# etheriqa/amber

Measured on AMD Instinct MI355X. Metric: Mrays/sec + wall-clock, Cornell 1024^2 @1024spp; 1/2/4/8 GPU, higher is better.
Workload: dtype f32

## Files before the change

amber_amd/api.py:

```python
from __future__ import annotations

import ctypes as C
import os
import subprocess
from pathlib import Path

import numpy as np

_ROOT = Path(__file__).resolve().parent
_LIB_PATH = _ROOT / "lib" / os.environ.get("AMBER_AMD_LIB", "libamber_hip.so")
_lib = None


class AmberError(RuntimeError):
    """Raised for every non-zero return code of the C ABI (message = amber_hip_last_error())."""


class FlatObject(C.Structure):
    _fields_ = [("kind", C.c_uint32), ("material", C.c_uint32), ("p", C.c_float * 12)]


class FlatMaterial(C.Structure):
    _fields_ = [("kind", C.c_uint32), ("rho", C.c_float * 3), ("param", C.c_float), ("r0", C.c_float)]


class FlatThinLens(C.Structure):
    _fields_ = [("origin", C.c_float * 3), ("global_", C.c_float * 9), ("local_", C.c_float * 9),
                ("focus_distance", C.c_float), ("sensor_distance", C.c_float), ("p_area", C.c_float),
                ("n_blades", C.c_uint32), ("first_blade_object", C.c_uint32), ("kind", C.c_uint32)]


class FlatLight(C.Structure):
    _fields_ = [("object", C.c_uint32), ("cum_power", C.c_float), ("pdf_area", C.c_float), ("irradiance", C.c_float * 3)]


class FlatSceneC(C.Structure):
    _fields_ = [("objects", C.POINTER(FlatObject)), ("n_objects", C.c_uint32),
                ("materials", C.POINTER(FlatMaterial)), ("n_materials", C.c_uint32), ("lens", FlatThinLens),
                ("lights", C.POINTER(FlatLight)), ("n_lights", C.c_uint32)]


class Splat(C.Structure):
    _fields_ = [("path", C.c_uint32), ("sample", C.c_uint32), ("bounce", C.c_uint32), ("pixel", C.c_uint32),
                ("rgb", C.c_float * 3), ("pad", C.c_uint32)]


class Sensor(C.Structure):
    _fields_ = [("width", C.c_uint32), ("height", C.c_uint32), ("scene_width", C.c_float), ("scene_height", C.c_float)]

    @classmethod
    def default(cls, width: int, height: int) -> "Sensor":
        return cls(width, height, np.float32(0.036), np.float32(0.036 / width * height))


class PtParams(C.Structure):
    _fields_ = [("seed", C.c_uint64), ("max_depth", C.c_uint32), ("device", C.c_int32), ("row_begin", C.c_uint32),
                ("row_end", C.c_uint32), ("stream", C.c_void_p), ("engine", C.c_uint32), ("stripe_rows", C.c_uint32),
                ("stripe_period", C.c_uint32), ("reserved", C.c_uint32)]


class BuildInfo(C.Structure):
    _fields_ = [("where", C.c_uint32), ("fallback_reason", C.c_uint32), ("n_nodes", C.c_uint32), ("n_leaves", C.c_uint32), ("depth", C.c_uint32),
                ("pad", C.c_uint32), ("tree_ms", C.c_double), ("create_ms", C.c_double)]


class UpdateInfo(C.Structure):
    _fields_ = [("mode_used", C.c_uint32), ("fallback_reason", C.c_uint32), ("n_nodes", C.c_uint32), ("depth", C.c_uint32),
                ("area_before", C.c_float), ("area_after", C.c_float), ("update_ms", C.c_double)]


class LtPassInfo(C.Structure):
    _fields_ = [("n_splats", C.c_uint64), ("n_rays", C.c_uint64), ("n_launches", C.c_uint32), ("n_repeats", C.c_uint32),
                ("longest_run", C.c_uint32), ("pad", C.c_uint32)]


class Photon(C.Structure):
    _fields_ = [("pos", C.c_float * 3), ("object", C.c_int32), ("dir_out", C.c_float * 3), ("path", C.c_uint32),
                ("weight", C.c_float * 3), ("sample", C.c_uint32), ("normal", C.c_float * 3), ("bounce", C.c_uint32)]


class PhotonInfo(C.Structure):
    _fields_ = [("n_photons", C.c_uint64), ("n_written", C.c_uint64), ("n_rays", C.c_uint64), ("n_launches", C.c_uint32), ("n_repeats", C.c_uint32)]


class AccumulateInfo(C.Structure):
    _fields_ = [("n_launches", C.c_uint32), ("n_repeats", C.c_uint32), ("rec_count", C.c_uint32), ("flag_words_set", C.c_uint32),
                ("flags_dirty", C.c_uint32)]


LT_SPLAT_CAPACITY0 = 65536
SPLAT_DTYPE = np.dtype([("path", np.uint32), ("sample", np.uint32), ("bounce", np.uint32), ("pixel", np.uint32), ("rgb", np.float32, (3,)), ("pad", np.uint32)])
PHOTON_DIFFUSE, PHOTON_SPECULAR, PHOTON_LIGHT, PHOTON_EYE, PHOTON_ALL = 1, 2, 4, 8, 15
PHOTONS_HOST = 1
PHOTON_CAPACITY0 = 65536
PHOTON_DTYPE = np.dtype([("pos", np.float32, (3,)), ("object", np.int32), ("dir_out", np.float32, (3,)), ("path", np.uint32),
                         ("weight", np.float32, (3,)), ("sample", np.uint32), ("normal", np.float32, (3,)), ("bounce", np.uint32)])


class Ray(C.Structure):
    _fields_ = [("origin", C.c_float * 3), ("t_max", C.c_float), ("dir", C.c_float * 3), ("pad", C.c_uint32)]


class RayHit(C.Structure):
    _fields_ = [("t", C.c_float), ("object", C.c_int32), ("pos", C.c_float * 3), ("normal", C.c_float * 3)]


class PathRay(C.Structure):
    _fields_ = [("origin", C.c_float * 3), ("pad0", C.c_uint32), ("dir", C.c_float * 3), ("pad1", C.c_uint32),
                ("weight", C.c_float * 3), ("pad2", C.c_uint32), ("rng_state", C.c_uint64), ("pad3", C.c_uint64)]


class PathResult(C.Structure):
    _fields_ = [("rgb", C.c_float * 3), ("casts", C.c_uint32), ("rng_state", C.c_uint64), ("pad", C.c_uint32 * 2)]


class AovPixel(C.Structure):
    _fields_ = [("albedo", C.c_float * 3), ("depth", C.c_float), ("normal", C.c_float * 3), ("coverage", C.c_float)]


class DenoiseParams(C.Structure):
    _fields_ = [("levels", C.c_uint32), ("k_normal", C.c_float), ("k_albedo", C.c_float), ("k_depth", C.c_float), ("k_color", C.c_float),
                ("reserved", C.c_uint32 * 3)]


class MomentsPixel(C.Structure):
    _fields_ = [("m1", C.c_float), ("m2", C.c_float), ("batches", C.c_float), ("pad", C.c_float)]


class DenoiseVarianceParams(C.Structure):
    _fields_ = [("levels", C.c_uint32), ("k_normal", C.c_float), ("k_albedo", C.c_float), ("k_depth", C.c_float), ("k_lum", C.c_float),
                ("var_radius", C.c_uint32), ("reserved", C.c_uint32 * 2)]


class TemporalParams(C.Structure):
    _fields_ = [("levels", C.c_uint32), ("max_history", C.c_uint32), ("k_normal", C.c_float), ("k_albedo", C.c_float), ("k_depth", C.c_float),
                ("k_color", C.c_float), ("reserved", C.c_uint32 * 2)]


class HistoryPixel(C.Structure):
    _fields_ = [("color", C.c_float * 3), ("length", C.c_float), ("m1", C.c_float), ("m2", C.c_float), ("pad", C.c_float * 2)]


class BvhDumpInfo(C.Structure):
    _fields_ = [("n_nodes", C.c_uint32), ("n_prims", C.c_uint32), ("root", C.c_int32), ("depth", C.c_uint32),
                ("gmin", C.c_float * 3), ("step", C.c_float * 3), ("reach", C.c_float * 3)]


class HostStats(C.Structure):
    _fields_ = [("rays", C.c_uint64), ("passes", C.c_uint64), ("launches", C.c_uint32), ("pad", C.c_uint32), ("kernel_ms", C.c_double)]


PRIM_TRIANGLE, PRIM_SPHERE, PRIM_DISK, PRIM_CYLINDER = 0, 1, 2, 3
_RECORD = np.dtype([("kind", np.uint32), ("material", np.uint32), ("p", np.float32, (12,))])
MAT_LAMBERTIAN, MAT_PHONG, MAT_SPECULAR, MAT_REFRACTION, MAT_DIFFUSE_LIGHT, MAT_EYE = 0, 1, 2, 3, 4, 5
ENGINE_AUTO, ENGINE_LIST, ENGINE_TWO_PHASE, ENGINE_BVH, ENGINE_WAVEFRONT = 0, 1, 2, 3, 4
ENGINE_REFERENCE_BVH = 6
PT_FLAG_NULL_STREAM, PT_FLAG_BVH_POOL, PT_FLAG_BVH_ITEMS = 1, 2, 4
PT_FLAG_DEVICE_BUILD = 8
BUILD_NONE, BUILD_HOST, BUILD_DEVICE, BUILD_HOST_FALLBACK = 0, 1, 2, 3
BUILD_REASON_NONE, BUILD_REASON_DEPTH, BUILD_REASON_WIDE, BUILD_REASON_BOUNDS = 0, 1, 2, 3
RAYS_HOST = 1
_RAY = np.dtype([("origin", np.float32, (3,)), ("t_max", np.float32), ("dir", np.float32, (3,)), ("pad", np.uint32)])
_RAY_HIT = np.dtype([("t", np.float32), ("object", np.int32), ("pos", np.float32, (3,)), ("normal", np.float32, (3,))])
_PATH_RAY = np.dtype([("origin", np.float32, (3,)), ("pad0", np.uint32), ("dir", np.float32, (3,)), ("pad1", np.uint32),
                      ("weight", np.float32, (3,)), ("pad2", np.uint32), ("rng_state", np.uint64), ("pad3", np.uint64)])
_PATH_RESULT = np.dtype([("rgb", np.float32, (3,)), ("casts", np.uint32), ("rng_state", np.uint64), ("pad", np.uint32, (2,))])
RESOLVE_MEAN_F32, RESOLVE_RGB8, RESOLVE_RGBA8 = 0, 1, 2
RESOLVE_HOST, RESOLVE_MIRROR_X = 1, 2
UPDATE_REFIT, UPDATE_REBUILD = 0, 1

ABI_SYMBOLS = [
    "amber_hip_pt_create", "amber_hip_pt_render_pass", "amber_hip_pt_clear", "amber_hip_pt_sync",
    "amber_hip_pt_download", "amber_hip_pt_device_framebuffer", "amber_hip_pt_stream", "amber_hip_pt_local_rows", "amber_hip_pt_kernel_time", "amber_hip_pt_build_info", "amber_hip_pt_update_objects", "amber_hip_pt_update_lens",
    "amber_hip_pt_cast_rays", "amber_hip_pt_occluded", "amber_hip_pt_resolve", "amber_hip_pt_destroy",
    "amber_hip_pt_trace_paths", "amber_hip_sampler_state",
    "amber_hip_pt_aov_pass", "amber_hip_pt_aov_clear", "amber_hip_pt_aov_download", "amber_hip_pt_device_aov", "amber_hip_pt_denoise",
    "amber_hip_pt_render_batch", "amber_hip_pt_moments_clear", "amber_hip_pt_moments_download", "amber_hip_pt_device_moments", "amber_hip_pt_denoise_variance",
    "amber_hip_pt_temporal", "amber_hip_pt_temporal_reset", "amber_hip_pt_history_download", "amber_hip_pt_device_history",
    "amber_hip_last_error", "amber_hip_abi_version", "amber_hip_math_mode", "amber_hip_device_count", "amber_hip_lt_trace", "amber_hip_lt_trace_range", "amber_hip_lt_render_pass",
    "amber_hip_lt_trace_photons",
    "amber_host_cornell_box", "amber_host_scene_import", "amber_host_scene_create", "amber_host_scene_destroy", "amber_host_scene_flatten",
    "amber_host_pt_create", "amber_host_render", "amber_host_render_devices", "amber_host_last_error", "amber_host_tonemap", "amber_host_export",
]
LAB_SYMBOLS = [
    "amber_hip_kat_cast", "amber_hip_kat_sample", "amber_hip_kat_eye", "amber_hip_kat_trace", "amber_hip_kat_math", "amber_hip_kat_signatures", "amber_hip_pt_signatures",
    "amber_hip_kat_traversal_rate", "amber_hip_kat_pixel_masks", "amber_hip_kat_bvh_dump", "amber_hip_kat_division",
    "amber_hip_kat_sqrt", "amber_hip_kat_sqrt_sweep", "amber_hip_kat_lt_accumulate", "amber_hip_kat_lt_stage_ms",
    "amber_hip_kat_photon_stage_ms",
    "amber_hip_kat_light_ray", "amber_hip_kat_lens_response", "amber_hip_kat_radiance", "amber_host_kat_scene_lights",
    "amber_hip_kat_accumulate",
]
PRODUCT_LIB, LAB_LIB = "libamber_hip.so", "libamber_hip_lab.so"


def library_path() -> Path:
    return _LIB_PATH


def build_library(force: bool = False) -> Path:
    import shutil
    if shutil.which(os.environ.get("HIPCC", "hipcc")) or not _LIB_PATH.exists():
        subprocess.run(["make", "-C", str(_ROOT / "csrc")] + (["-B"] if force else []), check=True)
    return _LIB_PATH


def is_lab() -> bool:
    return hasattr(load_library(), "amber_hip_kat_cast")


def load_library() -> C.CDLL:
    global _lib
    if _lib is not None:
        return _lib
    if not _LIB_PATH.exists():
        raise AmberError(f"{_LIB_PATH} is missing: build it with `make -C amber_amd/csrc` "
                         "(or __graft_entry__.build()); amber_amd has no CPU fallback")
    lib = C.CDLL(str(_LIB_PATH))
    vp, u32, u64, i32 = C.c_void_p, C.c_uint32, C.c_uint64, C.c_int32
    lib.amber_hip_last_error.restype = C.c_char_p
    lib.amber_host_last_error.restype = C.c_char_p
    lib.amber_hip_pt_create.argtypes = [C.POINTER(FlatSceneC), C.POINTER(Sensor), C.POINTER(PtParams), C.POINTER(vp)]
    lib.amber_hip_pt_render_pass.argtypes = [vp, u32, u32]
    lib.amber_hip_pt_clear.argtypes = [vp]
    lib.amber_hip_pt_sync.argtypes = [vp]
    lib.amber_hip_pt_download.argtypes = [vp, vp, C.POINTER(u64)]
    lib.amber_hip_pt_device_framebuffer.argtypes = [vp, C.POINTER(vp), C.POINTER(u64)]
    lib.amber_hip_pt_local_rows.argtypes = [vp, C.POINTER(u32)]
    lib.amber_hip_pt_stream.argtypes = [vp, C.POINTER(vp)]
    lib.amber_hip_pt_kernel_time.argtypes = [vp, C.POINTER(u32), C.POINTER(C.c_double)]
    lib.amber_hip_pt_destroy.argtypes = [vp]
    lib.amber_hip_pt_destroy.restype = None
    if hasattr(lib, "amber_hip_pt_build_info"):
        lib.amber_hip_pt_build_info.argtypes = [vp, C.POINTER(BuildInfo)]
    if hasattr(lib, "amber_hip_pt_update_objects"):
        lib.amber_hip_pt_update_objects.argtypes = [vp, u32, u32, vp, u32, C.POINTER(UpdateInfo)]
    if hasattr(lib, "amber_hip_pt_update_lens"):
        lib.amber_hip_pt_update_lens.argtypes = [vp, C.POINTER(FlatThinLens), vp, u32, C.POINTER(UpdateInfo)]
    if hasattr(lib, "amber_hip_pt_cast_rays"):
        lib.amber_hip_pt_cast_rays.argtypes = [vp, u64, vp, vp, u32]
        lib.amber_hip_pt_occluded.argtypes = [vp, u64, vp, vp, u32]
    if hasattr(lib, "amber_hip_pt_trace_paths"):
        lib.amber_hip_pt_trace_paths.argtypes = [vp, u64, vp, vp, u32, u32, u32]
        lib.amber_hip_sampler_state.argtypes = [u64, u32, u32]
        lib.amber_hip_sampler_state.restype = u64
    if hasattr(lib, "amber_hip_pt_resolve"):
        lib.amber_hip_pt_resolve.argtypes = [vp, u32, u32, vp, u64, u32]
    if hasattr(lib, "amber_hip_pt_aov_pass"):
        lib.amber_hip_pt_aov_pass.argtypes = [vp, u32, u32]
        lib.amber_hip_pt_aov_clear.argtypes = [vp]
        lib.amber_hip_pt_aov_download.argtypes = [vp, vp]
        lib.amber_hip_pt_device_aov.argtypes = [vp, C.POINTER(vp), C.POINTER(u64)]
    if hasattr(lib, "amber_hip_pt_denoise"):
        lib.amber_hip_pt_denoise.argtypes = [vp, u32, C.POINTER(DenoiseParams), u32, vp, u64, u32]
    if hasattr(lib, "amber_hip_pt_render_batch"):
        lib.amber_hip_pt_render_batch.argtypes = [vp, u32, u32]
        lib.amber_hip_pt_moments_clear.argtypes = [vp]
        lib.amber_hip_pt_moments_download.argtypes = [vp, vp]
        lib.amber_hip_pt_device_moments.argtypes = [vp, C.POINTER(vp), C.POINTER(u64)]
        lib.amber_hip_pt_denoise_variance.argtypes = [vp, u32, C.POINTER(DenoiseVarianceParams), u32, vp, u64, u32]
    if hasattr(lib, "amber_hip_pt_temporal"):
        lib.amber_hip_pt_temporal.argtypes = [vp, u32, C.POINTER(TemporalParams), u32, vp, u64, u32]
        lib.amber_hip_pt_temporal_reset.argtypes = [vp]
        lib.amber_hip_pt_history_download.argtypes = [vp, vp]
        lib.amber_hip_pt_device_history.argtypes = [vp, C.POINTER(vp), C.POINTER(u64)]
    if hasattr(lib, "amber_hip_lt_trace"):
        lib.amber_hip_lt_trace.argtypes = [vp, u32, u32, vp, u32, C.POINTER(u32), C.POINTER(u64)]
    if hasattr(lib, "amber_hip_lt_trace_range"):
        lib.amber_hip_lt_trace_range.argtypes = [vp, u32, u32, u32, u32, vp, u32, C.POINTER(u32), C.POINTER(u64)]
    if hasattr(lib, "amber_hip_lt_render_pass"):
        lib.amber_hip_lt_render_pass.argtypes = [vp, u32, u32, C.POINTER(LtPassInfo)]
        if hasattr(lib, "amber_hip_lt_trace_photons"):
            lib.amber_hip_lt_trace_photons.argtypes = [vp, u32, u32, u32, u32, u32, vp, u64, C.POINTER(PhotonInfo), u32]
        if hasattr(lib, "amber_hip_kat_photon_stage_ms"):
            lib.amber_hip_kat_photon_stage_ms.argtypes = [vp, C.POINTER(C.c_double), C.POINTER(C.c_double), C.POINTER(C.c_double)]
    if hasattr(lib, "amber_hip_kat_cast"):
        lib.amber_hip_kat_cast.argtypes = [vp, u32, vp, vp, vp, vp, vp, vp]
        lib.amber_hip_kat_sample.argtypes = [vp, u32, vp, vp, vp, vp, vp, vp]
        lib.amber_hip_kat_eye.argtypes = [vp, u32, vp, vp, vp]
        lib.amber_hip_kat_trace.argtypes = [vp, u32, vp, vp, u32, vp, vp]
        lib.amber_hip_kat_math.argtypes = [i32, i32, u32, vp, vp]
        lib.amber_hip_kat_signatures.argtypes = [vp, u32, u32, vp]
        lib.amber_hip_kat_pixel_masks.argtypes = [vp, vp, vp, C.POINTER(C.c_uint32), C.POINTER(C.c_double)]
        lib.amber_hip_kat_traversal_rate.argtypes = [vp, u32, vp, vp, u32, u32, u32, vp, vp, C.POINTER(C.c_double), vp]
        lib.amber_hip_pt_signatures.argtypes = [vp, u32, u32, vp]
        lib.amber_hip_kat_bvh_dump.argtypes = [vp, vp, u32, vp, u32, C.POINTER(BvhDumpInfo)]
        if hasattr(lib, "amber_hip_kat_division"):
            lib.amber_hip_kat_division.argtypes = [i32, i32, u32, vp, vp]
        if hasattr(lib, "amber_hip_kat_sqrt"):
            lib.amber_hip_kat_sqrt.argtypes = [i32, i32, u32, vp, vp]
            lib.amber_hip_kat_sqrt_sweep.argtypes = [i32, u32, u64, C.POINTER(SqrtSweep)]
        if hasattr(lib, "amber_hip_kat_lt_accumulate"):
            lib.amber_hip_kat_lt_accumulate.argtypes = [vp, vp, u32]
            lib.amber_hip_kat_lt_stage_ms.argtypes = [vp, C.POINTER(C.c_double), C.POINTER(C.c_double)]
        if hasattr(lib, "amber_hip_kat_light_ray"):
            lib.amber_hip_kat_light_ray.argtypes = [vp, u32, vp, vp, vp, vp, vp]
            lib.amber_hip_kat_lens_response.argtypes = [vp, u32, vp, vp, vp, vp, vp]
            lib.amber_hip_kat_radiance.argtypes = [vp, u32, vp, vp, vp, vp]
            lib.amber_host_kat_scene_lights.argtypes = [vp, C.POINTER(FlatLight), C.POINTER(u32)]
        if hasattr(lib, "amber_hip_kat_accumulate"):
            lib.amber_hip_kat_accumulate.argtypes = [vp, u32, vp, vp, u32, u32, u32, u64, C.POINTER(AccumulateInfo)]
    lib.amber_host_cornell_box.restype = vp
    lib.amber_host_cornell_box.argtypes = [C.c_float, C.c_float, u32]
    lib.amber_host_scene_import.restype = vp
    lib.amber_host_scene_import.argtypes = [C.c_char_p]
    lib.amber_host_scene_create.restype = vp
    lib.amber_host_scene_create.argtypes = [C.POINTER(FlatObject), u32, C.POINTER(FlatMaterial), u32, C.POINTER(C.c_float),
                                            C.c_float, C.c_float, C.c_float, u32, C.c_int]
    lib.amber_host_scene_destroy.argtypes = [vp]
    lib.amber_host_scene_destroy.restype = None
    lib.amber_host_scene_flatten.argtypes = [vp, C.POINTER(FlatObject), C.POINTER(u32), C.POINTER(FlatMaterial), C.POINTER(u32),
                                             C.POINTER(FlatThinLens)]
    lib.amber_host_pt_create.argtypes = [vp, C.POINTER(Sensor), C.POINTER(PtParams), C.POINTER(vp)]
    lib.amber_host_render.argtypes = [vp, C.c_char_p, C.POINTER(Sensor), u32, u64, u32, C.c_int, u32, vp, C.POINTER(HostStats)]
    lib.amber_host_render_devices.argtypes = [vp, C.c_char_p, C.POINTER(Sensor), u32, u64, u32, C.POINTER(C.c_int), u32, u32, vp, C.POINTER(HostStats)]
    lib.amber_host_tonemap.argtypes = [vp, u32, u32, vp]
    lib.amber_host_export.argtypes = [vp, u32, u32, C.c_char_p, C.c_char_p]
    _lib = lib
    return lib


def _check(rc: int, host: bool = False) -> None:
    if rc != 0:
        lib = load_library()
        msg = (lib.amber_host_last_error() if host else lib.amber_hip_last_error()) or b""
        if host and not msg:
            msg = lib.amber_hip_last_error() or b""
        raise AmberError(f"amber error {rc}: {msg.decode(errors='replace')}")


def device_count() -> int:
    return int(load_library().amber_hip_device_count())


def _f32(a) -> np.ndarray:
    return np.ascontiguousarray(a, dtype=np.float32)


class HostScene:

    def __init__(self, handle):
        if not handle:
            raise AmberError("scene creation failed: " + (load_library().amber_host_last_error() or b"").decode())
        self._h = C.c_void_p(handle)

    @classmethod
    def cornell_box(cls, focal_length: float = 0.050, aperture_radius: float = 0.050, n_blades: int = 6) -> "HostScene":
        return cls(load_library().amber_host_cornell_box(focal_length, aperture_radius, n_blades))

    @classmethod
    def import_file(cls, filename) -> "HostScene":
        return cls(load_library().amber_host_scene_import(str(filename).encode()))

    @classmethod
    def create(cls, objects, materials, transform, focal_length, focus_distance, radius, n_blades, accel: int = 0) -> "HostScene":
        objs = (FlatObject * max(1, len(objects)))()
        for i, (kind, mat, params) in enumerate(objects):
            objs[i].kind, objs[i].material = kind, mat
            for j, v in enumerate(params):
                objs[i].p[j] = v
        mats = (FlatMaterial * max(1, len(materials)))()
        for i, (kind, rho, param) in enumerate(materials):
            mats[i].kind, mats[i].param = kind, param
            for j in range(3):
                mats[i].rho[j] = rho[j]
        t = (C.c_float * 16)(*[float(x) for x in transform])
        return cls(load_library().amber_host_scene_create(objs, len(objects), mats, len(materials), t, focal_length,
                                                          focus_distance, radius, n_blades, accel))

    @classmethod
    def create_arrays(cls, kinds, material_index, params, materials, transform, focal_length, focus_distance, radius, n_blades,
                      accel: int = 0) -> "HostScene":
        n = len(kinds)
        dt = np.dtype([("kind", np.uint32), ("material", np.uint32), ("p", np.float32, (12,))])
        arr = np.zeros(n, dt)
        arr["kind"], arr["material"] = kinds, material_index
        arr["p"][:, : np.asarray(params).shape[1]] = params
        assert arr.itemsize == C.sizeof(FlatObject)
        mats = (FlatMaterial * max(1, len(materials)))()
        for i, (kind, rho, param) in enumerate(materials):
            mats[i].kind, mats[i].param = kind, param
            for j in range(3):
                mats[i].rho[j] = rho[j]
        t = (C.c_float * 16)(*[float(x) for x in transform])
        return cls(load_library().amber_host_scene_create(arr.ctypes.data_as(C.POINTER(FlatObject)), n, mats, len(materials), t,
                                                          focal_length, focus_distance, radius, n_blades, accel))

    def flatten(self):
        lib = load_library()
        no, nm = C.c_uint32(0), C.c_uint32(0)
        _check(lib.amber_host_scene_flatten(self._h, None, C.byref(no), None, C.byref(nm), None), host=True)
        objs, mats, lens = (FlatObject * no.value)(), (FlatMaterial * nm.value)(), FlatThinLens()
        _check(lib.amber_host_scene_flatten(self._h, objs, C.byref(no), mats, C.byref(nm), C.byref(lens)), host=True)
        return objs, mats, lens

    def lights(self):
        lib = load_library()
        n = C.c_uint32(0)
        _check(lib.amber_host_kat_scene_lights(self._h, None, C.byref(n)), host=True)
        out = (FlatLight * max(1, n.value))()
        _check(lib.amber_host_kat_scene_lights(self._h, out, C.byref(n)), host=True)
        return list(out[:n.value])

    def render(self, sensor: Sensor, spp: int, seed: int = 12345, max_depth: int = 0, device: int = 0,
               samples_per_launch: int = 0, algorithm: str = "pt", devices=None):
        out = np.empty((sensor.height, sensor.width, 3), np.float32)
        st = HostStats()
        devs = list(devices) if devices else [device]
        arr = (C.c_int * len(devs))(*devs)
        _check(load_library().amber_host_render_devices(self._h, algorithm.encode(), C.byref(sensor), spp, seed, max_depth, arr, len(devs),
                                                        samples_per_launch, out.ctypes.data, C.byref(st)), host=True)
        return out, {"rays": st.rays, "passes": st.passes, "launches": st.launches, "kernel_ms": st.kernel_ms}

    def close(self):
        if self._h:
            load_library().amber_host_scene_destroy(self._h)
            self._h = None

    def __del__(self):
        try:
            self.close()
        except Exception:
            pass


def sampler_state(seed: int, pixel: int, sample: int) -> int:
    return int(load_library().amber_hip_sampler_state(seed & 0xffffffffffffffff, pixel, sample))


def _splitmix64(z):
    with np.errstate(over="ignore"):
        z = z + np.uint64(0x9E3779B97F4A7C15)
        z = (z ^ (z >> np.uint64(30))) * np.uint64(0xBF58476D1CE4E5B9)
        z = (z ^ (z >> np.uint64(27))) * np.uint64(0x94D049BB133111EB)
        return z ^ (z >> np.uint64(31))


def sampler_states(seed: int, pixels, samples) -> np.ndarray:
    pixels, samples = np.asarray(pixels, np.uint64), np.asarray(samples, np.uint64)
    hashed = _splitmix64(np.array([seed & 0xffffffffffffffff], np.uint64))[0]
    s = _splitmix64(hashed ^ ((pixels << np.uint64(32)) | samples))
    return np.where(s == 0, np.uint64(0x9E3779B97F4A7C15), s).astype(np.uint64)


class PathTracer:

    def __init__(self, scene: HostScene, sensor: Sensor, seed: int = 12345, max_depth: int = 0, device: int = 0,
                 rows=None, stream: int | None = None, engine: int = ENGINE_AUTO, stripe=None, flags: int = 0):
        self.sensor, self.seed = sensor, seed
        self._scene, self._resident = scene, None
        rb, re = rows if rows is not None else (0, sensor.height)
        s_rows, s_period = stripe if stripe else (0, 0)
        p = PtParams(seed, max_depth, device, rb, re, stream, engine, s_rows, s_period, flags)
        h = C.c_void_p()
        _check(load_library().amber_host_pt_create(scene._h, C.byref(sensor), C.byref(p), C.byref(h)), host=True)
        self._h = h
        ys = np.arange(rb, re)
        self.row_index = ys[(ys - rb) % s_period < s_rows] if s_rows else ys
        n = C.c_uint32()
        _check(load_library().amber_hip_pt_local_rows(self._h, C.byref(n)))
        assert n.value == len(self.row_index)
        self.rows = (rb, re)

    @property
    def band_shape(self):
        return (len(self.row_index), self.sensor.width, 3)

    def render_pass(self, first_sample: int, n_samples: int) -> None:
        _check(load_library().amber_hip_pt_render_pass(self._h, first_sample, n_samples))

    def clear(self) -> None:
        _check(load_library().amber_hip_pt_clear(self._h))

    def sync(self) -> None:
        _check(load_library().amber_hip_pt_sync(self._h))

    def download(self):
        out = np.empty(self.band_shape, np.float32)
        rays = C.c_uint64()
        _check(load_library().amber_hip_pt_download(self._h, out.ctypes.data, C.byref(rays)))
        return out, rays.value

    def ray_count(self) -> int:
        rays = C.c_uint64()
        _check(load_library().amber_hip_pt_download(self._h, None, C.byref(rays)))
        return rays.value

    def stream(self) -> int:
        p = C.c_void_p()
        _check(load_library().amber_hip_pt_stream(self._h, C.byref(p)))
        return p.value or 0

    def device_framebuffer(self):
        p, n = C.c_void_p(), C.c_uint64()
        _check(load_library().amber_hip_pt_device_framebuffer(self._h, C.byref(p), C.byref(n)))
        return p.value, n.value

    def kernel_time(self):
        n, ms = C.c_uint32(), C.c_double()
        _check(load_library().amber_hip_pt_kernel_time(self._h, C.byref(n), C.byref(ms)))
        return n.value, ms.value

    def build_info(self) -> dict:
        b = BuildInfo()
        _check(load_library().amber_hip_pt_build_info(self._h, C.byref(b)))
        return {k: getattr(b, k) for k, _ in BuildInfo._fields_ if k != "pad"}

    def update_objects(self, first: int, kinds, material_index, params, mode: int = UPDATE_REFIT) -> dict:
        kinds, material_index = np.ascontiguousarray(kinds, np.uint32), np.ascontiguousarray(material_index, np.uint32)
        n = len(kinds)
        if n == 0:
            return self.update_flat(first, np.zeros(0, _RECORD), mode)
        if self._resident is None:
            objs, _, _ = self._scene.flatten()
            self._resident = np.frombuffer(objs, dtype=_RECORD)[["kind", "material"]].copy()
        if first < 0 or first + n > len(self._resident):
            raise AmberError(f"update_objects: objects [{first}, {first + n}) are not all in the scene ({len(self._resident)} objects)")
        resident = self._resident[first:first + n]
        if not np.array_equal(resident["kind"], kinds):
            raise AmberError(f"update_objects: object {first + int(np.argmax(resident['kind'] != kinds))}: the kind differs from the resident record's (an update moves geometry only)")
        pairs = np.unique(np.stack([material_index, resident["material"]], 1), axis=0)
        if len(np.unique(pairs[:, 0])) != len(pairs) or len(np.unique(pairs[:, 1])) != len(pairs):
            raise AmberError("update_objects: material_index is not the resident objects' material assignment (an update moves geometry only)")
        tmp = HostScene.create_arrays(kinds, np.zeros(n, np.uint32), params, [(MAT_LAMBERTIAN, (0.5, 0.5, 0.5), 0.0)],
                                      [1, 0, 0, 0, 0, 1, 0, 0, 0, 0, 1, 0, 0, 0, 0, 1], 0.05, 1.0, 0.01, 0)
        objs, _, lens = tmp.flatten()
        flat = np.frombuffer(objs, dtype=_RECORD)
        keep = np.ones(len(flat), bool)
        keep[lens.first_blade_object:lens.first_blade_object + lens.n_blades] = False
        records = flat[keep].copy()
        tmp.close()
        assert len(records) == n and np.array_equal(records["kind"], kinds)
        records["material"] = resident["material"]
        return self.update_flat(first, records, mode)

    def update_flat(self, first: int, records, mode: int = UPDATE_REFIT, count=None) -> dict:
        info = UpdateInfo()
        ptr, n = None, count or 0
        if records is not None:
            records = np.ascontiguousarray(records)
            assert records.itemsize == C.sizeof(FlatObject)
            ptr, n = records.ctypes.data, len(records) if count is None else count
        _check(load_library().amber_hip_pt_update_objects(self._h, first, n, ptr, mode, C.byref(info)))
        return {k: getattr(info, k) for k, _ in UpdateInfo._fields_}

    def update_lens(self, scene_or_lens, mode: int = UPDATE_REFIT) -> dict:
        if isinstance(scene_or_lens, HostScene):
            objs, _, lens = scene_or_lens.flatten()
            records = np.frombuffer(objs, dtype=_RECORD)[lens.first_blade_object:lens.first_blade_object + lens.n_blades].copy()
        else:
            lens, records = scene_or_lens
        ptr = None
        if records is not None:
            records = np.ascontiguousarray(records)
            assert records.itemsize == C.sizeof(FlatObject)
            if lens is not None and len(records) < lens.n_blades:
                raise AmberError(f"update_lens: {len(records)} blade records for a lens of {lens.n_blades} blades")
            ptr = records.ctypes.data
        info = UpdateInfo()
        _check(load_library().amber_hip_pt_update_lens(self._h, C.byref(lens) if lens is not None else None, ptr, mode, C.byref(info)))
        return {k: getattr(info, k) for k, _ in UpdateInfo._fields_}

    @staticmethod
    def _is_torch(a) -> bool:
        return type(a).__module__.split(".")[0] == "torch"

    def _pack_rays(self, origins, dirs, t_max):
        if self._is_torch(origins) or self._is_torch(dirs):
            import torch
            if not (self._is_torch(origins) and self._is_torch(dirs)) or not origins.is_cuda or origins.device != dirs.device:
                raise AmberError("cast_rays / occluded: origins and dirs must both be numpy arrays or both be torch tensors on the handle's device")
            o, d = origins.reshape(-1, 3).to(torch.float32), dirs.reshape(-1, 3).to(torch.float32)
            if len(o) != len(d):
                raise AmberError("cast_rays / occluded: origins and dirs differ in length")
            packed = torch.zeros((len(o), 8), dtype=torch.float32, device=o.device)
            packed[:, 0:3], packed[:, 4:7] = o, d
            if t_max is None:
                packed[:, 3] = float("inf")
            else:
                packed[:, 3] = t_max if not self._is_torch(t_max) else t_max.to(device=o.device, dtype=torch.float32).reshape(-1)
            return packed, len(o), torch
        o, d = _f32(origins).reshape(-1, 3), _f32(dirs).reshape(-1, 3)
        if len(o) != len(d):
            raise AmberError("cast_rays / occluded: origins and dirs differ in length")
        packed = np.zeros(len(o), _RAY)
        packed["origin"], packed["dir"] = o, d
        packed["t_max"] = np.inf if t_max is None else np.asarray(t_max, np.float32)
        return packed, len(o), None

    def cast_rays(self, origins, dirs, t_max=None):
        packed, n, torch = self._pack_rays(origins, dirs, t_max)
        lib = load_library()
        if torch is None:
            hits = np.zeros(n, _RAY_HIT)
            _check(lib.amber_hip_pt_cast_rays(self._h, n, packed.ctypes.data, hits.ctypes.data, RAYS_HOST))
            return hits["object"].copy(), hits["t"].copy(), hits["pos"].copy(), hits["normal"].copy()
        out = torch.empty((n, 8), dtype=torch.float32, device=packed.device)
        same = self._torch_enter(torch, packed.device)
        _check(lib.amber_hip_pt_cast_rays(self._h, n, packed.data_ptr(), out.data_ptr(), 0))
        self._torch_leave(same)
        return out[:, 1].contiguous().view(torch.int32), out[:, 0].contiguous(), out[:, 2:5].contiguous(), out[:, 5:8].contiguous()

    def occluded(self, origins, dirs, t_max=None):
        packed, n, torch = self._pack_rays(origins, dirs, t_max)
        lib = load_library()
        if torch is None:
            occ = np.zeros(n, np.uint8)
            _check(lib.amber_hip_pt_occluded(self._h, n, packed.ctypes.data, occ.ctypes.data, RAYS_HOST))
            return occ.astype(bool)
        out = torch.empty(n, dtype=torch.uint8, device=packed.device)
        same = self._torch_enter(torch, packed.device)
        _check(lib.amber_hip_pt_occluded(self._h, n, packed.data_ptr(), out.data_ptr(), 0))
        self._torch_leave(same)
        return out.to(torch.bool)

    def trace_paths(self, origins, dirs, weights=None, states=None, n_samples: int = 1, max_depth: int = 0):
        lib = load_library()
        if self._is_torch(origins) or self._is_torch(dirs):
            import torch
            if not (self._is_torch(origins) and self._is_torch(dirs)) or not origins.is_cuda or origins.device != dirs.device:
                raise AmberError("trace_paths: origins and dirs must both be numpy arrays or both be torch tensors on the handle's device")
            o, d = origins.reshape(-1, 3).to(torch.float32), dirs.reshape(-1, 3).to(torch.float32)
            n = len(o)
            if len(d) != n:
                raise AmberError("trace_paths: origins and dirs differ in length")
            packed = torch.zeros((n, 16), dtype=torch.float32, device=o.device)
            packed[:, 0:3], packed[:, 4:7] = o, d
            if weights is None:
                packed[:, 8:11] = 1.0
            else:
                packed[:, 8:11] = torch.as_tensor(weights, device=o.device).to(torch.float32).reshape(-1, 3)
            if states is None:
                states = sampler_states(self.seed, np.arange(n), np.zeros(n))
            if not self._is_torch(states):
                states = torch.from_numpy(np.ascontiguousarray(states, np.uint64).view(np.int64))
            packed.view(torch.int64)[:, 6] = states.to(device=o.device, dtype=torch.int64).reshape(-1)
            out = torch.empty((n, 8), dtype=torch.float32, device=o.device)
            same = self._torch_enter(torch, o.device)
            _check(lib.amber_hip_pt_trace_paths(self._h, n, packed.data_ptr(), out.data_ptr(), n_samples, max_depth, 0))
            self._torch_leave(same)
            return out[:, 0:3].contiguous(), out[:, 3].contiguous().view(torch.int32), out.view(torch.int64)[:, 2].contiguous()
        o, d = _f32(origins).reshape(-1, 3), _f32(dirs).reshape(-1, 3)
        n = len(o)
        if len(d) != n:
            raise AmberError("trace_paths: origins and dirs differ in length")
        packed = np.zeros(n, _PATH_RAY)
        packed["origin"], packed["dir"] = o, d
        packed["weight"] = 1.0 if weights is None else _f32(weights).reshape(-1, 3)
        packed["rng_state"] = sampler_states(self.seed, np.arange(n), np.zeros(n)) if states is None else np.asarray(states, np.uint64).reshape(-1)
        res = np.zeros(n, _PATH_RESULT)
        _check(lib.amber_hip_pt_trace_paths(self._h, n, packed.ctypes.data, res.ctypes.data, n_samples, max_depth, RAYS_HOST))
        return res["rgb"].copy(), res["casts"].copy(), res["rng_state"].copy()

    def _torch_enter(self, torch, device) -> bool:
        same = torch.cuda.current_stream(device).cuda_stream == self.stream()
        if not same:
            torch.cuda.current_stream(device).synchronize()
        return same

    def _torch_leave(self, same: bool) -> None:
        if not same:
            self.sync()

    def resolve(self, n_samples: int, format: int = RESOLVE_RGB8, mirror: bool = False, out=None):
        return self._filter("resolve", load_library().amber_hip_pt_resolve, n_samples, None, format, mirror, out)

    def _band_download(self, entry, channels: int) -> np.ndarray:
        rows, width, _ = self.band_shape
        out = np.zeros((rows, width, channels), np.float32)
        _check(entry(self._h, out.ctypes.data))
        return out

    def _band_pointer(self, entry):
        p, n = C.c_void_p(), C.c_uint64()
        _check(entry(self._h, C.byref(p), C.byref(n)))
        return p.value, n.value

    def aov_pass(self, first_sample: int, n_samples: int) -> None:
        _check(load_library().amber_hip_pt_aov_pass(self._h, first_sample, n_samples))

    def aov_clear(self) -> None:
        _check(load_library().amber_hip_pt_aov_clear(self._h))

    def aov_download(self) -> np.ndarray:
        return self._band_download(load_library().amber_hip_pt_aov_download, 8)

    def device_aov(self):
        return self._band_pointer(load_library().amber_hip_pt_device_aov)

    def denoise(self, n_samples: int, levels: int = 5, k_normal: float = 4.0, k_albedo: float = 100.0, k_depth: float = 10.0, k_color: float = 0.25,
                format: int = RESOLVE_RGB8, mirror: bool = False, out=None):
        params = DenoiseParams(levels=levels, k_normal=k_normal, k_albedo=k_albedo, k_depth=k_depth, k_color=k_color)
        return self._filter("denoise", load_library().amber_hip_pt_denoise, n_samples, params, format, mirror, out)

    def _filter(self, what: str, entry, n_samples: int, params, format: int, mirror: bool, out):
        if format not in (RESOLVE_MEAN_F32, RESOLVE_RGB8, RESOLVE_RGBA8):
            raise AmberError(f"{what}: unknown format {format}")
        rows, width, _ = self.band_shape
        channels, flags = (4 if format == RESOLVE_RGBA8 else 3), (RESOLVE_MIRROR_X if mirror else 0)
        head = (self._h, n_samples) if params is None else (self._h, n_samples, C.byref(params))
        if out is None:
            res = np.empty((rows, width, channels), np.float32 if format == RESOLVE_MEAN_F32 else np.uint8)
            _check(entry(*head, format, res.ctypes.data, res.nbytes, flags | RESOLVE_HOST))
            return res
        if not self._is_torch(out):
            raise AmberError(f"{what}: out must be None or a torch tensor on the handle's device")
        import torch
        dtype = torch.float32 if format == RESOLVE_MEAN_F32 else torch.uint8
        if not out.is_cuda or out.dtype != dtype or not out.is_contiguous() or out.numel() != rows * width * channels:
            raise AmberError(f"{what}: out must be a contiguous {dtype} tensor of {rows} x {width} x {channels} elements on the handle's device")
        same = self._torch_enter(torch, out.device)
        _check(entry(*head, format, out.data_ptr(), out.numel() * out.element_size(), flags))
        self._torch_leave(same)
        return out

    def render_batch(self, first_sample: int, n_samples: int) -> None:
        _check(load_library().amber_hip_pt_render_batch(self._h, first_sample, n_samples))

    def moments_clear(self) -> None:
        _check(load_library().amber_hip_pt_moments_clear(self._h))

    def moments_download(self) -> np.ndarray:
        return self._band_download(load_library().amber_hip_pt_moments_download, 4)

    def device_moments(self):
        return self._band_pointer(load_library().amber_hip_pt_device_moments)

    def denoise_variance(self, n_samples: int, levels: int = 5, k_normal: float = 4.0, k_albedo: float = 100.0, k_depth: float = 10.0, k_lum: float = 16.0,
                         var_radius: int = 3, format: int = RESOLVE_RGB8, mirror: bool = False, out=None):
        params = DenoiseVarianceParams(levels=levels, k_normal=k_normal, k_albedo=k_albedo, k_depth=k_depth, k_lum=k_lum, var_radius=var_radius)
        return self._filter("denoise_variance", load_library().amber_hip_pt_denoise_variance, n_samples, params, format, mirror, out)

    def temporal(self, n_samples: int, levels: int = 5, max_history: int = 32, k_normal: float = 4.0, k_albedo: float = 100.0, k_depth: float = 10.0,
                 k_color: float = 0.25, format: int = RESOLVE_RGB8, mirror: bool = False, out=None):
        params = TemporalParams(levels=levels, max_history=max_history, k_normal=k_normal, k_albedo=k_albedo, k_depth=k_depth, k_color=k_color)
        return self._filter("temporal", load_library().amber_hip_pt_temporal, n_samples, params, format, mirror, out)

    def temporal_reset(self) -> None:
        _check(load_library().amber_hip_pt_temporal_reset(self._h))

    def history_download(self) -> np.ndarray:
        return self._band_download(load_library().amber_hip_pt_history_download, 8)

    def device_history(self):
        return self._band_pointer(load_library().amber_hip_pt_device_history)

    def lt_trace(self, first_sample: int, n_samples: int, capacity: int = 1 << 16, paths=None):
        dt = SPLAT_DTYPE
        while True:
            out = np.zeros(capacity, dt)
            n, rays = C.c_uint32(), C.c_uint64()
            if paths is None:
                rc = load_library().amber_hip_lt_trace(self._h, first_sample, n_samples, out.ctypes.data, capacity, C.byref(n), C.byref(rays))
            else:
                rc = load_library().amber_hip_lt_trace_range(self._h, first_sample, n_samples, paths[0], paths[1], out.ctypes.data, capacity,
                                                             C.byref(n), C.byref(rays))
            if rc == -4 and n.value > capacity:
                capacity = n.value
                continue
            _check(rc)
            return out[: n.value], rays.value

    def lt_render_pass(self, first_sample: int, n_samples: int) -> dict:
        info = LtPassInfo()
        _check(load_library().amber_hip_lt_render_pass(self._h, first_sample, n_samples, C.byref(info)))
        return {k: int(getattr(info, k)) for k, _ in LtPassInfo._fields_ if k != "pad"}

    def lt_trace_photons(self, first_sample: int, n_samples: int, surfaces: int = PHOTON_DIFFUSE, paths=None, out=None):
        lib = load_library()
        begin, end = (0, self.sensor.width * self.sensor.height) if paths is None else (int(paths[0]), int(paths[1]))
        info = PhotonInfo()

        def call(ptr, capacity, flags):
            rc = lib.amber_hip_lt_trace_photons(self._h, first_sample, n_samples, begin, end, surfaces, ptr, capacity, C.byref(info), flags)
            d = {k: int(getattr(info, k)) for k, _ in PhotonInfo._fields_}
            if rc != 0:
                try:
                    _check(rc)
                except AmberError as e:
                    e.code, e.info = rc, d
                    raise
            return d

        if out is None:
            need = call(None, 0, PHOTONS_HOST)["n_photons"]
            out = np.zeros(need, PHOTON_DTYPE)
            d = call(out.ctypes.data if need else None, need, PHOTONS_HOST)
            return out, d
        if isinstance(out, np.ndarray):
            if out.dtype != PHOTON_DTYPE or not out.flags.c_contiguous or out.ndim != 1:
                raise AmberError("lt_trace_photons: out must be a contiguous one-dimensional numpy array of PHOTON_DTYPE")
            d = call(out.ctypes.data if len(out) else None, len(out), PHOTONS_HOST)
            return out[: d["n_written"]], d
        if self._is_torch(out):
            import torch
            if not out.is_cuda or not out.is_contiguous() or out.dim() != 2 or out.shape[1] * out.element_size() != 64:
                raise AmberError("lt_trace_photons: out must be a contiguous torch tensor on the handle's device with rows of 64 bytes")
            same = self._torch_enter(torch, out.device)
            try:
                d = call(out.data_ptr() if out.shape[0] else None, out.shape[0], 0)
            finally:
                self._torch_leave(same)
            return out[: d["n_written"]], d
        ptr, capacity = out
        d = call(ptr, capacity, 0)
        return d["n_written"], d

    def kat_photon_stage_ms(self):
        a, b, c = C.c_double(), C.c_double(), C.c_double()
        _check(load_library().amber_hip_kat_photon_stage_ms(self._h, C.byref(a), C.byref(b), C.byref(c)))
        return a.value, b.value, c.value

    def kat_lt_accumulate(self, records) -> None:
        rec = np.ascontiguousarray(records, SPLAT_DTYPE)
        _check(load_library().amber_hip_kat_lt_accumulate(self._h, rec.ctypes.data if len(rec) else None, len(rec)))

    def kat_accumulate(self, n_samples: int, q, rgb, n_waves: int = 4, rec_capacity: int = 0, rays: int = 0) -> dict:
        qq = np.ascontiguousarray(q, np.uint32).reshape(-1)
        cc = _f32(rgb).reshape(-1, 3)
        assert len(qq) == len(cc)
        info = AccumulateInfo()
        _check(load_library().amber_hip_kat_accumulate(self._h, n_samples, qq.ctypes.data if len(qq) else None, cc.ctypes.data if len(qq) else None,
                                                       len(qq), n_waves, rec_capacity, rays, C.byref(info)))
        return {k: int(getattr(info, k)) for k, _ in AccumulateInfo._fields_}

    def kat_lt_stage_ms(self):
        a, b = C.c_double(), C.c_double()
        _check(load_library().amber_hip_kat_lt_stage_ms(self._h, C.byref(a), C.byref(b)))
        return a.value, b.value

    def kat_cast(self, origins, dirs):
        o, d = _f32(origins).reshape(-1, 3), _f32(dirs).reshape(-1, 3)
        n = len(o)
        obj, t = np.empty(n, np.int32), np.empty(n, np.float32)
        pos, nrm = np.empty((n, 3), np.float32), np.empty((n, 3), np.float32)
        _check(load_library().amber_hip_kat_cast(self._h, n, o.ctypes.data, d.ctypes.data, obj.ctypes.data, t.ctypes.data,
                                                 pos.ctypes.data, nrm.ctypes.data))
        return obj, t, pos, nrm

    def kat_sample(self, material, normals, dirs_out, rng_state, importance: bool = False):
        m = np.ascontiguousarray(material, np.uint32) | np.uint32(0x80000000 if importance else 0)
        nn, dd = _f32(normals).reshape(-1, 3), _f32(dirs_out).reshape(-1, 3)
        st = np.ascontiguousarray(rng_state, np.uint64).copy()
        n = len(m)
        di, w = np.empty((n, 3), np.float32), np.empty((n, 3), np.float32)
        _check(load_library().amber_hip_kat_sample(self._h, n, m.ctypes.data, nn.ctypes.data, dd.ctypes.data, st.ctypes.data,
                                                   di.ctypes.data, w.ctypes.data))
        return di, w, st

    def kat_eye(self, pixel, sample):
        p, s = np.ascontiguousarray(pixel, np.uint32), np.ascontiguousarray(sample, np.uint32)
        out = np.empty((len(p), 7), np.float32)
        _check(load_library().amber_hip_kat_eye(self._h, len(p), p.ctypes.data, s.ctypes.data, out.ctypes.data))
        return out

    def kat_light_ray(self, rng_state):
        st = np.ascontiguousarray(rng_state, np.uint64).copy()
        n = len(st)
        o, d, w = np.empty((n, 3), np.float32), np.empty((n, 3), np.float32), np.empty((n, 3), np.float32)
        light = np.empty(n, np.uint32)
        _check(load_library().amber_hip_kat_light_ray(self._h, n, st.ctypes.data, o.ctypes.data, d.ctypes.data, w.ctypes.data, light.ctypes.data))
        return o, d, w, light, st

    def kat_lens_response(self, position, direction_out):
        p, d = _f32(position).reshape(-1, 3), _f32(direction_out).reshape(-1, 3)
        n = len(p)
        reached, pixel, value = np.empty(n, np.uint32), np.empty(n, np.uint32), np.empty(n, np.float32)
        _check(load_library().amber_hip_kat_lens_response(self._h, n, p.ctypes.data, d.ctypes.data, reached.ctypes.data, pixel.ctypes.data,
                                                          value.ctypes.data))
        return reached, pixel, value

    def kat_radiance(self, material, normals, dirs_out):
        m = np.ascontiguousarray(material, np.uint32)
        nn, dd = _f32(normals).reshape(-1, 3), _f32(dirs_out).reshape(-1, 3)
        out = np.empty((len(m), 3), np.float32)
        _check(load_library().amber_hip_kat_radiance(self._h, len(m), m.ctypes.data, nn.ctypes.data, dd.ctypes.data, out.ctypes.data))
        return out

    def kat_trace(self, pixel, sample, max_bounces: int = 16):
        p, s = np.ascontiguousarray(pixel, np.uint32), np.ascontiguousarray(sample, np.uint32)
        rec = np.zeros((len(p), max_bounces, 11), np.uint32)
        casts = np.zeros(len(p), np.uint32)
        _check(load_library().amber_hip_kat_trace(self._h, len(p), p.ctypes.data, s.ctypes.data, max_bounces, rec.ctypes.data,
                                                  casts.ctypes.data))
        return rec, casts

    def kat_traversal_rate(self, origins, dirs, waves: int = 5, refill_min: int = 16, repeats: int = 3, rounds=None):
        o, d = _f32(origins).reshape(-1, 3), _f32(dirs).reshape(-1, 3)
        n = len(o)
        obj, t, ms = np.empty(n, np.int32), np.empty(n, np.float32), C.c_double()
        _check(load_library().amber_hip_kat_traversal_rate(self._h, n, o.ctypes.data, d.ctypes.data, waves, refill_min, repeats, t.ctypes.data,
                                                           obj.ctypes.data, C.byref(ms), rounds.ctypes.data if rounds is not None else None))
        return obj, t, ms.value

    def kat_signatures(self, first_sample: int, n_samples: int) -> np.ndarray:
        rows, width, _ = self.band_shape
        out = np.zeros((rows, width, n_samples), np.uint64)
        _check(load_library().amber_hip_kat_signatures(self._h, first_sample, n_samples, out.ctypes.data))
        return out

    def pixel_masks(self):
        rows, width, _ = self.band_shape
        masks = np.zeros((rows, width), np.uint32)
        ms = C.c_double()
        _check(load_library().amber_hip_kat_pixel_masks(self._h, masks.ctypes.data, None, None, C.byref(ms)))
        return masks, ms.value

    def object_slots(self, n_objects: int):
        slots = np.zeros(n_objects, np.uint32)
        always = C.c_uint32()
        _check(load_library().amber_hip_kat_pixel_masks(self._h, None, slots.ctypes.data, C.byref(always), None))
        return slots, always.value

    def bvh_dump(self) -> dict:
        info = BvhDumpInfo()
        _check(load_library().amber_hip_kat_bvh_dump(self._h, None, 0, None, 0, C.byref(info)))
        nodes, prims = np.zeros((info.n_nodes, 8), np.uint32), np.zeros(info.n_prims, np.uint32)
        _check(load_library().amber_hip_kat_bvh_dump(self._h, nodes.ctypes.data, info.n_nodes, prims.ctypes.data, info.n_prims, C.byref(info)))
        return dict(nodes=nodes, prims=prims, root=int(info.root), depth=int(info.depth), gmin=np.array(info.gmin[:], np.float32),
                    step=np.array(info.step[:], np.float32), reach=np.array(info.reach[:], np.float32))

    def render_signatures(self, first_sample: int, n_samples: int) -> np.ndarray:
        rows, width, _ = self.band_shape
        out = np.zeros((rows, width, n_samples), np.uint64)
        _check(load_library().amber_hip_pt_signatures(self._h, first_sample, n_samples, out.ctypes.data))
        return out

    def close(self):
        if getattr(self, "_h", None):
            load_library().amber_hip_pt_destroy(self._h)
            self._h = None

    def __del__(self):
        try:
            self.close()
        except Exception:
            pass


def kat_math(mode: int, x, device: int = 0) -> np.ndarray:
    x = _f32(x)
    n = len(x)
    out = np.empty((n,) if mode == 1 else (n, 2), np.float32)
    _check(load_library().amber_hip_kat_math(device, mode, n, x.ctypes.data, out.ctypes.data))
    return out.view(np.float64).reshape(n) if mode >= 2 else out


def kat_division(mode: int, x, device: int = 0) -> np.ndarray:
    x = np.ascontiguousarray(x, np.float32).reshape(-1, 4)
    n = len(x)
    out = np.empty((n, 3), np.float32)
    _check(load_library().amber_hip_kat_division(device, mode, n, x.ctypes.data, out.ctypes.data))
    return out


class SqrtSweep(C.Structure):
    _fields_ = [("mismatches", C.c_uint64), ("in_range", C.c_uint64), ("n_offenders", C.c_uint32), ("offenders", C.c_uint32 * 8),
                ("seed_low", C.c_int32), ("seed_high", C.c_int32)]


def kat_sqrt(mode: int, x, device: int = 0) -> np.ndarray:
    width = 1 if mode <= 1 else (3 if mode <= 3 else 2)
    x = np.ascontiguousarray(x, np.float32).reshape(-1, width)
    out = np.empty_like(x)
    _check(load_library().amber_hip_kat_sqrt(device, mode, len(x), x.ctypes.data, out.ctypes.data))
    return out.reshape(-1) if width == 1 else out


def kat_sqrt_sweep(first_bits: int, count: int, device: int = 0) -> dict:
    r = SqrtSweep()
    _check(load_library().amber_hip_kat_sqrt_sweep(device, first_bits, count, C.byref(r)))
    return {"mismatches": int(r.mismatches), "in_range": int(r.in_range), "offenders": [int(b) for b in r.offenders[:min(int(r.n_offenders), 8)]],
            "seed_low": int(r.seed_low), "seed_high": int(r.seed_high)}


MATH_PORTABLE, MATH_GLIBC = 1, 2


def math_mode() -> int:
    return int(load_library().amber_hip_math_mode())


def tonemap(image) -> np.ndarray:
    img = _f32(image)
    h, w, _ = img.shape
    out = np.empty((h, w, 3), np.uint8)
    _check(load_library().amber_host_tonemap(img.ctypes.data, w, h, out.ctypes.data), host=True)
    return out


def export(image, png_path=None, exr_path=None) -> None:
    img = _f32(image)
    h, w, _ = img.shape
    _check(load_library().amber_host_export(img.ctypes.data, w, h, png_path.encode() if png_path else None,
                                            exr_path.encode() if exr_path else None), host=True)
```

amber_amd/csrc/hip/dev_scene.h:

```cpp
#pragma once

namespace amber_dev {

#ifdef AMBER_STAMPS
struct StampCtx { unsigned long long last; unsigned long long acc[8]; };
__device__ __forceinline__ void StampAt(StampCtx* c, int k) {
  __builtin_amdgcn_sched_barrier(0);
  const unsigned long long t = __builtin_amdgcn_s_memtime();
  __builtin_amdgcn_s_waitcnt(0xC07F);
  c->acc[k] += t - c->last;
  c->last = t;
  __builtin_amdgcn_sched_barrier(0);
}
#define AMBER_STAMP_PARAM , StampCtx* stamp_ctx
#define AMBER_STAMP_ARG , stamp_ctx
#define AMBER_STAMP(k) StampAt(stamp_ctx, k)
__device__ __forceinline__ void CountAt(StampCtx* c, int k) {
  if (!c) return;
  const unsigned long long m = __ballot(true);
  c->acc[2 * k] += 1ull;
  if (__builtin_amdgcn_mbcnt_hi(static_cast<uint32_t>(m >> 32), __builtin_amdgcn_mbcnt_lo(static_cast<uint32_t>(m), 0u)) == 0u) c->acc[2 * k + 1] += 1ull;
}
#ifdef AMBER_BVH_CLOCKS
#define AMBER_COUNT(k)
#define AMBER_CLK(k) do { if (stamp_ctx) StampAt(stamp_ctx, k); } while (0)
#else
#define AMBER_COUNT(k) CountAt(stamp_ctx, k)
#define AMBER_CLK(k)
#endif
#ifdef AMBER_COUNT_ALT
#define AMBER_COUNT_ROUNDS(k)
#define AMBER_COUNT_LEAVES(k) AMBER_COUNT(k)
#else
#define AMBER_COUNT_ROUNDS(k) AMBER_COUNT(k)
#define AMBER_COUNT_LEAVES(k)
#endif
#define AMBER_STAMP_PARAM_OPT , StampCtx* stamp_ctx = nullptr
#else
#define AMBER_COUNT(k)
#define AMBER_COUNT_ROUNDS(k)
#define AMBER_COUNT_LEAVES(k)
#define AMBER_CLK(k)
#define AMBER_STAMP_PARAM_OPT
#define AMBER_STAMP_PARAM
#define AMBER_STAMP_ARG
#define AMBER_STAMP(k)
#endif

struct alignas(16) DevObject {
  float a[3];   uint32_t kind;
  float e1[3];  float radius;
  float e2[3];  float height;
  float n[3];   uint32_t material;
};
struct alignas(16) DevMaterial {
  uint32_t kind; float rho[3];
  float param; float r0;
  float aux0, aux1;
};
struct alignas(16) DevBlade {
  float v0[3], v1[3], v2[3], n[3];
  int32_t slot;
  int32_t pad[3];
};
struct alignas(16) DevPlane {
  float n[3]; float d0;
  float kt;
  float ktol;
  uint32_t n_tris;
  uint32_t n_pairs;
};
struct alignas(16) DevTriFilter {
  float c[4][2];
};
struct alignas(16) DevSphereFilter {
  float c[3]; float r2;
  float ktol; uint32_t pad[3];
};
struct alignas(16) DevFilterGroup {
  uint32_t plane_first, n_planes, n_simple_planes, tri_first;
  uint32_t sphere_first, n_sphere_filters, always_mask, n_prog_tris;
  uint32_t n_objects, pad[3];
};
struct alignas(16) DevBvhNode {
  float lxy[4];
  float rxy[4];
  float z[4];
  int32_t left, right, pad0, pad1;
};
struct alignas(16) DevBvhNodeQ {
  uint32_t w[6];
  int32_t left, right;
};
struct alignas(16) DevBvhNodeQ4 {
  uint32_t w[12];
  int32_t child[4];
};
#ifndef AMBER_BVH_WIDE
#define AMBER_BVH_WIDE 0
#endif
struct alignas(16) DevLight {
  uint32_t kind; int32_t slot;
  float cum_power; float pdf_area;
  float irr[3]; float pad0;
  float p[12];
  float pad1[4];
};
struct DevSplat { uint32_t path, sample, bounce, pixel; float rgb[3]; uint32_t pad; };
struct DevLens {
  float origin[3];
  float global_[9];
  float local_[9];
  float focus_distance, sensor_distance, p_area;
  float neg_fd_over_sd;
  float neg_sd_over_fd;
  float size_over_area;
  double sd2;
  uint32_t n_blades;
  float n_blades_f;
  uint32_t kind;
  float inv_scene_area;
  float edge_tol;
};
struct alignas(16) DevRefNode { float lmin[3], lmax[3], rmin[3], rmax[3]; int32_t left, right; uint32_t pad[2]; };
struct DevRefLeaf { uint32_t first, count; };
struct DevSensor {
  uint32_t w, h;
  float wf, hf, sw, sh;
  float size_f;
};
struct DevScene {
  const DevObject* __restrict__ objects;
  const DevMaterial* __restrict__ materials;
  const DevBlade* __restrict__ blades;
  const DevPlane* __restrict__ planes;
  const DevTriFilter* __restrict__ tri_filters;
  const DevSphereFilter* __restrict__ sphere_filters;
  uint32_t n_planes, n_sphere_filters;
  uint32_t n_simple_planes;
  uint32_t always_mask;
  uint32_t blade_mask;
  uint32_t n_prog_tris;
  const DevObject* __restrict__ prog_objects;
  const DevFilterGroup* __restrict__ groups;
  uint32_t n_groups;
  uint32_t n_lds_objects;
  const DevBvhNodeQ* __restrict__ bvh_nodes;
  const DevBvhNodeQ4* __restrict__ bvh_nodes4;
  float bvh_gmin[3], bvh_step[3];
  float bvh_reach[3];
  const float4* __restrict__ bvh_spheres;
  const float4* __restrict__ bvh_tris;
  const uint32_t* __restrict__ bvh_prims;
  const DevObject* __restrict__ bvh_objects;
  int32_t bvh_root;
  float fp_center[3];
  float fp_reach;
  float fp_tmax;
  float bvh_center[3];
  float bvh_half_diag;
  float bvh_inv_rmin;
  const DevLight* __restrict__ lights;
  uint32_t n_lights;
  float total_power;
  uint32_t n_objects;
  uint32_t max_depth;
  const DevLens* __restrict__ lens;
  DevSensor sensor;
  const DevRefNode* __restrict__ ref_nodes;
  const DevRefLeaf* __restrict__ ref_leaves;
  uint2* ref_stack;
  uint32_t ref_stack_stride;
};

#define AMBER_PHONG_MAX_TRIES 1024
enum { PRIM_TRIANGLE = 0, PRIM_SPHERE = 1, PRIM_DISK = 2, PRIM_CYLINDER = 3 };
enum { MAT_LAMBERTIAN = 0, MAT_PHONG = 1, MAT_SPECULAR = 2, MAT_REFRACTION = 3, MAT_DIFFUSE_LIGHT = 4, MAT_EYE = 5 };

}
```

amber_amd/csrc/hip/dev_two_phase.h:

```cpp
#pragma once

namespace amber_dev {

#define AMBER_GRAZING 1e-3f
#ifndef AMBER_SHARED_WEIGHT_QUOTIENT
#define AMBER_SHARED_WEIGHT_QUOTIENT 1
#endif
struct FilterView {
  ConstWords planes, tris, spheres;
  int n_planes, n_simple_planes, n_sphere_filters;
  uint32_t always_mask, n_prog_tris, n_objects;
  int slot_base;
};
__device__ __forceinline__ FilterView SceneView(const DevScene& sc) {
  return FilterView{(ConstWords)(sc.planes), (ConstWords)(sc.tri_filters), (ConstWords)(sc.sphere_filters), static_cast<int>(sc.n_planes), static_cast<int>(sc.n_simple_planes),
                    static_cast<int>(sc.n_sphere_filters), sc.always_mask, sc.n_prog_tris, sc.n_objects, 0};
}
template <bool kMulti, bool kFirst, int kSqrt = SQRT_PLAIN>
__device__ __forceinline__ void ClosestHitTwoPhaseView(const DevScene& sc, const FilterView fv, const DevObject* lds_objects, V3 o_world, V3 d, int origin_slot, HitRec& best AMBER_STAMP_PARAM,
                                                       const bool use_premask, const uint32_t premask);
template <int kSqrt = SQRT_PLAIN>
__device__ __forceinline__ void ClosestHitTwoPhase(const DevScene& sc, const DevObject* lds_objects, V3 o_world, V3 d, int origin_slot, HitRec& best AMBER_STAMP_PARAM,
                                                   const bool use_premask = false, const uint32_t premask = 0u) {
  ClosestHitTwoPhaseView<false, true, kSqrt>(sc, SceneView(sc), lds_objects, o_world, d, origin_slot, best AMBER_STAMP_ARG, use_premask, premask);
}
template <int kSqrt = SQRT_PLAIN>
__device__ __forceinline__ void ClosestHitTwoPhaseGroups(const DevScene& sc, const DevObject* lds_objects, V3 o_world, V3 d, int origin_slot, HitRec& best AMBER_STAMP_PARAM,
                                                         const bool use_premask = false, const uint32_t premask = 0u) {
  ClosestHitTwoPhaseView<true, true, kSqrt>(sc, SceneView(sc), lds_objects, o_world, d, origin_slot < 32 ? origin_slot : -1, best AMBER_STAMP_ARG, use_premask, premask);
  const int n_groups = static_cast<int>(sc.n_groups);
  ConstWords gw = (ConstWords)(sc.groups);
  for (int g = 1; g < n_groups; ++g) {
    ConstWords w = gw + g * 12;
    const FilterView fv{(ConstWords)(sc.planes) + w[0] * 8u, (ConstWords)(sc.tri_filters) + w[3] * 8u, (ConstWords)(sc.sphere_filters) + w[4] * 8u,
                        static_cast<int>(w[1]), static_cast<int>(w[2]), static_cast<int>(w[5]), w[6], w[7], w[8], g * 32};
    ClosestHitTwoPhaseView<true, false, kSqrt>(sc, fv, lds_objects, o_world, d, origin_slot, best AMBER_STAMP_ARG, false, 0u);
  }
}
template <bool kGrouped> constexpr uint32_t kLdsKindMask = kGrouped ? 0x7fu : 0xffu;
template <bool kMulti, bool kFirst, int kSqrt>
__device__ __forceinline__ void ClosestHitTwoPhaseView(const DevScene& sc, const FilterView fv, const DevObject* lds_objects_all, V3 o_world, V3 d, int origin_slot_all, HitRec& best AMBER_STAMP_PARAM,
                                                       const bool use_premask, const uint32_t premask) {
  if (kFirst) { best.t = 3.402823466e+38f; best.u = 0.f; best.v = 0.f; best.idx = -1; best.slot = -1; }
  const int slot_base = kMulti ? fv.slot_base : 0;
  const DevObject* lds_objects = kMulti ? lds_objects_all + slot_base : lds_objects_all;
  const int origin_slot = kFirst ? origin_slot_all : ((origin_slot_all >= slot_base && origin_slot_all < slot_base + 32) ? origin_slot_all - slot_base : -1);
  constexpr uint32_t kKindMask = kLdsKindMask<kMulti>;
  uint32_t cand = kMulti ? fv.always_mask : sc.always_mask;
  if (use_premask) cand |= premask;
  else {
    const V3 o = v3(o_world.x - sc.fp_center[0], o_world.y - sc.fp_center[1], o_world.z - sc.fp_center[2]);
    float t_upper = sc.fp_tmax * __builtin_amdgcn_rsqf(d.x * d.x + d.y * d.y + d.z * d.z);
    if (!(t_upper == t_upper)) t_upper = 3.402823466e+38f;
    ConstWords pl = kMulti ? fv.planes : (ConstWords)(sc.planes);
    ConstWords tr = kMulti ? fv.tris : (ConstWords)(sc.tri_filters);
    const int n_planes = kMulti ? fv.n_planes : static_cast<int>(sc.n_planes);
    uint32_t bit = 1u;
    float nd = 0.f, no = 0.f, rc = 0.f;
#define AMBER_PLANE_NORMAL() \
        nd = __builtin_fmaf(cw_f(pl, 0), d.x, __builtin_fmaf(cw_f(pl, 1), d.y, cw_f(pl, 2) * d.z)); \
        no = __builtin_fmaf(cw_f(pl, 0), o.x, __builtin_fmaf(cw_f(pl, 1), o.y, cw_f(pl, 2) * o.z)); \
        rc = __builtin_amdgcn_rcpf(nd);
#define AMBER_PLANE_SETUP() \
      const float tp = (cw_f(pl, 3) - no) * rc; \
      const float rho = Abs(rc); \
      const float Px = __builtin_fmaf(tp, d.x, o.x), Py = __builtin_fmaf(tp, d.y, o.y), Pz = __builtin_fmaf(tp, d.z, o.z); \
      const float kr = cw_f(pl, 4) * rho;                    \
      const bool t_ok = (tp >= AMBER_KEPS - kr) && !(tp - kr > t_upper);                   \
       \
       \
      const bool degenerate = !(Abs(nd) >= 1e-6f); \
      const bool grazing = !(Abs(nd) >= AMBER_GRAZING); \
      const bool t_sure = (tp - kr > AMBER_KEPS) && !grazing; \
      const float ptol = cw_f(pl, 5) * rho; \
      const float mtol = grazing ? -3.402823466e+38f : -ptol;                              \
      bool plane_hit = false;
#ifndef AMBER_NO_CERTAIN_HITS
#define AMBER_PLANE_HIT(m_) plane_hit |= (m_) >= ptol
#else
#define AMBER_PLANE_HIT(m_)
#endif
#define AMBER_PAIR_RECORD() { \
        const float b = __builtin_fmaf(cw_f(tr, 0), Px, __builtin_fmaf(cw_f(tr, 2), Py, __builtin_fmaf(cw_f(tr, 4), Pz, cw_f(tr, 6)))); \
        const float a = __builtin_fmaf(cw_f(tr, 1), Px, __builtin_fmaf(cw_f(tr, 3), Py, __builtin_fmaf(cw_f(tr, 5), Pz, cw_f(tr, 7)))); \
        const float ba = b + a;                              \
        const float g = 1.0f - ba; \
        const float m1 = __builtin_fminf(__builtin_fminf(b, a), g); \
        const float m2 = __builtin_fminf(__builtin_fminf(-b, 1.0f - a), ba); \
        const bool keep1 = (!(m1 < mtol) && t_ok) || degenerate;                           \
        const bool keep2 = (!(m2 < mtol) && t_ok) || degenerate; \
        cand |= keep1 ? bit : 0u; \
        cand |= keep2 ? (bit << 1) : 0u; \
        AMBER_PLANE_HIT(__builtin_fmaxf(m1, m2)); }
    const int n_simple = kMulti ? fv.n_simple_planes : static_cast<int>(sc.n_simple_planes);
    int p = 0;
    for (; p < n_simple; p += 2) {
      AMBER_PLANE_NORMAL();
      { AMBER_PLANE_SETUP(); AMBER_PAIR_RECORD(); if (plane_hit && t_sure) t_upper = __builtin_fminf(t_upper, tp + kr); }
      pl += 8; tr += 8; bit <<= 2;
      { AMBER_PLANE_SETUP(); AMBER_PAIR_RECORD(); if (plane_hit && t_sure) t_upper = __builtin_fminf(t_upper, tp + kr); }
      pl += 8; tr += 8; bit <<= 2;
    }
    for (; p < n_planes; ++p, pl += 8) {
      if (!(pl[6] & 0x80000000u)) { AMBER_PLANE_NORMAL(); }
      AMBER_PLANE_SETUP();
      const int nt = static_cast<int>(pl[6] & 0x7fffffffu), np = static_cast<int>(pl[7]);
      for (int k = 0; k < np; ++k, tr += 8, bit <<= 2) {
        AMBER_PAIR_RECORD();
      }
      for (int k = 0; k < nt; ++k, tr += 8, bit <<= 1) {
        const float u = __builtin_fmaf(cw_f(tr, 0), Px, __builtin_fmaf(cw_f(tr, 2), Py, __builtin_fmaf(cw_f(tr, 4), Pz, cw_f(tr, 6))));
        const float v = __builtin_fmaf(cw_f(tr, 1), Px, __builtin_fmaf(cw_f(tr, 3), Py, __builtin_fmaf(cw_f(tr, 5), Pz, cw_f(tr, 7))));
        const float w = 1.0f - u - v;
        const float m = __builtin_fminf(__builtin_fminf(u, v), w);
        const bool keep = (!(m < mtol) && t_ok) || degenerate;
        cand |= keep ? bit : 0u;
        AMBER_PLANE_HIT(m);
      }
      if (plane_hit && t_sure) t_upper = __builtin_fminf(t_upper, tp + kr);
    }
#undef AMBER_PLANE_SETUP
#undef AMBER_PLANE_NORMAL
#undef AMBER_PAIR_RECORD
#undef AMBER_PLANE_HIT
    ConstWords sp = kMulti ? fv.spheres : (ConstWords)(sc.sphere_filters);
    const int ns = kMulti ? fv.n_sphere_filters : static_cast<int>(sc.n_sphere_filters);
    for (int k = 0; k < ns; ++k, sp += 8, bit <<= 1) {
      const float cx = cw_f(sp, 0) - o.x, cy = cw_f(sp, 1) - o.y, cz = cw_f(sp, 2) - o.z;
      const float bb = __builtin_fmaf(cx, d.x, __builtin_fmaf(cy, d.y, cz * d.z));
      const float c2 = __builtin_fmaf(cx, cx, __builtin_fmaf(cy, cy, cz * cz));
      const float r2 = cw_f(sp, 3);
      const float cc = c2 - r2;
      const float tol = cw_f(sp, 4) * (c2 + r2);
      const bool miss = (__builtin_fmaf(bb, bb, -cc) < -tol) || (bb < 0.0f && cc > tol);
      cand |= miss ? 0u : bit;
    }
  }
  if (!use_premask) {
    const float ex = Abs(o_world.x - sc.fp_center[0]), ey = Abs(o_world.y - sc.fp_center[1]), ez = Abs(o_world.z - sc.fp_center[2]);
    const bool in_model = __builtin_fmaxf(__builtin_fmaxf(ex, ey), ez) <= sc.fp_reach && (d.x * d.x + d.y * d.y + d.z * d.z) <= 4.0f;
    if (!in_model) { const uint32_t n_here = kMulti ? fv.n_objects : sc.n_objects; cand = n_here >= 32u ? 0xffffffffu : ((1u << n_here) - 1u); }
  }
  AMBER_STAMP(2);
  {
    const bool has_self = origin_slot >= 0 && ((cand >> (origin_slot & 31)) & 1u) != 0u;
    if (has_self) {
      const DevObject& ob = lds_objects[origin_slot];
      const V3 A = ld3(ob.a), E1 = ld3(ob.e1), E2 = ld3(ob.e2);
      const float det = Dot(Cross(d, E2), E1);
      const float t = Dot(Cross(o_world - A, E1), E2) / det;
      if (t <= AMBER_KEPS) cand &= ~(1u << origin_slot);
    }
  }
  const uint32_t n_tris_here = kMulti ? fv.n_prog_tris : sc.n_prog_tris;
  const uint32_t tri_bits = n_tris_here >= 32u ? 0xffffffffu : ((1u << n_tris_here) - 1u);
  uint32_t mt = cand & tri_bits;
#ifdef AMBER_STAMPS
  while (__any(mt != 0u)) {
    stamp_ctx->acc[7] += 1ull + (static_cast<unsigned long long>(__popcll(__ballot(mt != 0u))) << 32);
    if (mt != 0u) {
#else
  while (mt != 0u) {
    {
#endif
      const int slot = __builtin_ctz(mt);
      mt &= mt - 1u;
      const DevObject& ob = lds_objects[slot];
      IntersectTriangle<true>(ld3(ob.a), ld3(ob.e1), ld3(ob.e2), static_cast<int>(ob.kind >> 8), slot_base + slot, o_world, d, best);
    }
  }
  uint32_t mo = cand & ~tri_bits;
  while (mo != 0u) {
    const int slot = __builtin_ctz(mo);
    mo &= mo - 1u;
    const DevObject& ob = lds_objects[slot];
    IntersectObject<true, kSqrt>(ob, ob.kind & kKindMask, static_cast<int>(ob.kind >> 8), slot_base + slot, o_world, d, best);
  }
}

}
```

amber_amd/csrc/hip/filter_build.h:

```cpp
#pragma once

#include <algorithm>
#include <cmath>
#include <cstdint>
#include <cstring>
#include <vector>

#include "../../../include/amber_hip.h"
#include "pt_device.h"

namespace amber_filter {

using amber_dev::DevObject;
using amber_dev::DevPlane;
using amber_dev::DevSphereFilter;
using amber_dev::DevTriFilter;

struct FilterProgram {
  std::vector<DevPlane> planes;
  std::vector<DevTriFilter> tris;
  std::vector<DevSphereFilter> spheres;
  std::vector<uint32_t> order;
  uint32_t n_prog_tris = 0, always_mask = 0;
  uint32_t n_simple_planes = 0;
};

inline void BuildFilterProgram(const std::vector<DevObject>& objs, const float center[3], FilterProgram& fp, const std::vector<uint32_t>* subset = nullptr) {
  double lo[3] = {1e300, 1e300, 1e300}, hi[3] = {-1e300, -1e300, -1e300}, e_max = 0;
  auto grow = [&](double x, double y, double z) {
    const double p[3] = {x, y, z};
    for (int c = 0; c < 3; c++) { if (p[c] < lo[c]) lo[c] = p[c]; if (p[c] > hi[c]) hi[c] = p[c]; }
  };
  auto len3 = [](const double* v) { return std::sqrt(v[0] * v[0] + v[1] * v[1] + v[2] * v[2]); };
  for (const DevObject& o : objs) {
    if (o.kind == AMBER_PRIM_TRIANGLE) {
      grow(o.a[0], o.a[1], o.a[2]);
      grow(double(o.a[0]) + o.e1[0], double(o.a[1]) + o.e1[1], double(o.a[2]) + o.e1[2]);
      grow(double(o.a[0]) + o.e2[0], double(o.a[1]) + o.e2[1], double(o.a[2]) + o.e2[2]);
      const double E1[3] = {o.e1[0], o.e1[1], o.e1[2]}, E2[3] = {o.e2[0], o.e2[1], o.e2[2]};
      e_max = std::max(e_max, std::max(len3(E1), len3(E2)));
    } else {
      const double r = std::fabs(double(o.radius)) + std::fabs(double(o.height));
      grow(o.a[0] - r, o.a[1] - r, o.a[2] - r); grow(o.a[0] + r, o.a[1] + r, o.a[2] + r);
    }
  }
  const double diam = std::sqrt((hi[0] - lo[0]) * (hi[0] - lo[0]) + (hi[1] - lo[1]) * (hi[1] - lo[1]) + (hi[2] - lo[2]) * (hi[2] - lo[2]));
  const double eps = 5.9604644775390625e-08;
  const double c = 32.0 * eps * (diam + 1.5 * e_max);
  struct Tri { uint32_t index; double v[3][3]; double coef[3][4]; double g; };
  struct Group { double n[3], d0, kt, ktol; std::vector<Tri> tris; bool flip = false, same_normal = false; };
  std::vector<Group> groups;
  std::vector<uint32_t> sphere_index, always_index;
  const size_t n_members = subset ? std::min<size_t>(subset->size(), 32) : std::min<size_t>(objs.size(), 32);
  for (size_t member = 0; member < n_members; member++) {
    const uint32_t idx = subset ? (*subset)[member] : static_cast<uint32_t>(member);
    const DevObject& o = objs[idx];
    if (o.kind == AMBER_PRIM_TRIANGLE) {
      const double v0[3] = {double(o.a[0]) - center[0], double(o.a[1]) - center[1], double(o.a[2]) - center[2]};
      const double E1[3] = {o.e1[0], o.e1[1], o.e1[2]}, E2[3] = {o.e2[0], o.e2[1], o.e2[2]};
      const double nr[3] = {E1[1] * E2[2] - E1[2] * E2[1], E1[2] * E2[0] - E1[0] * E2[2], E1[0] * E2[1] - E1[1] * E2[0]};
      const double n2 = nr[0] * nr[0] + nr[1] * nr[1] + nr[2] * nr[2];
      if (!(n2 > 1e-60) || !std::isfinite(n2)) { always_index.push_back(idx); continue; }
      const double nl = std::sqrt(n2);
      const double n[3] = {nr[0] / nl, nr[1] / nl, nr[2] / nl};
      const double d0 = n[0] * v0[0] + n[1] * v0[1] + n[2] * v0[2];
      const double A[3] = {(E2[1] * nr[2] - E2[2] * nr[1]) / n2, (E2[2] * nr[0] - E2[0] * nr[2]) / n2, (E2[0] * nr[1] - E2[1] * nr[0]) / n2};
      const double B[3] = {(nr[1] * E1[2] - nr[2] * E1[1]) / n2, (nr[2] * E1[0] - nr[0] * E1[2]) / n2, (nr[0] * E1[1] - nr[1] * E1[0]) / n2};
      const double AB[3] = {A[0] + B[0], A[1] + B[1], A[2] + B[2]};
      const double g = std::max(len3(A), std::max(len3(B), len3(AB)));
      const double inv_sin = len3(E1) * len3(E2) / nl;
      const double verts[3][3] = {{v0[0], v0[1], v0[2]}, {v0[0] + E1[0], v0[1] + E1[1], v0[2] + E1[2]}, {v0[0] + E2[0], v0[1] + E2[1], v0[2] + E2[2]}};
      Group* grp = nullptr; double dist = 0;
      for (Group& gq : groups) {
        double dmax = 0;
        for (const auto& vtx : verts) dmax = std::max(dmax, std::fabs(gq.n[0] * vtx[0] + gq.n[1] * vtx[1] + gq.n[2] * vtx[2] - gq.d0));
        if (dmax <= 4.0 * eps * diam) { grp = &gq; dist = dmax; break; }
      }
      Tri t;
      t.index = idx; t.g = g;
      for (int k = 0; k < 3; k++) for (int c2 = 0; c2 < 3; c2++) t.v[k][c2] = verts[k][c2];
      const double a0 = -(A[0] * v0[0] + A[1] * v0[1] + A[2] * v0[2]), b0 = -(B[0] * v0[0] + B[1] * v0[1] + B[2] * v0[2]);
      for (int k = 0; k < 3; k++) { t.coef[1][k] = A[k]; t.coef[2][k] = B[k]; t.coef[0][k] = -(A[k] + B[k]); }
      t.coef[1][3] = a0; t.coef[2][3] = b0; t.coef[0][3] = 1.0 - a0 - b0;
      const double ktol = (c + dist) * g * 1.0001 + 1e-7;
      const double kt = 2.0 * (c + dist) * std::max(1.0, inv_sin) + 1e-7;
      if (!std::isfinite(ktol) || !std::isfinite(static_cast<float>(a0)) || !std::isfinite(static_cast<float>(b0)) || !std::isfinite(kt)) { always_index.push_back(idx); continue; }
      if (!grp) { groups.push_back(Group{{n[0], n[1], n[2]}, d0, 0.0, 0.0, {}, false, false}); grp = &groups.back(); }
      grp->kt = std::max(grp->kt, kt);
      grp->ktol = std::max(grp->ktol, ktol);
      grp->tris.push_back(t);
    } else if (o.kind == AMBER_PRIM_SPHERE) {
      DevSphereFilter f;
      std::memset(&f, 0, sizeof f);
      for (int k = 0; k < 3; k++) f.c[k] = static_cast<float>(double(o.a[k]) - center[k]);
      f.r2 = static_cast<float>(double(o.radius) * double(o.radius));
      f.ktol = 1e-5f;
      if (!std::isfinite(f.r2)) { always_index.push_back(idx); continue; }
      fp.spheres.push_back(f);
      sphere_index.push_back(idx);
    } else {
      always_index.push_back(idx);
    }
  }
  auto record = [](const Tri& t, int row_a, int row_b) {
    DevTriFilter f;
    std::memset(&f, 0, sizeof f);
    for (int k = 0; k < 4; k++) { f.c[k][0] = static_cast<float>(t.coef[row_a][k]); f.c[k][1] = static_cast<float>(t.coef[row_b][k]); }
    return f;
  };
  {
    double cw[3] = {0, 0, 0}, wsum = 0;
    std::vector<double> gc(groups.size() * 3, 0.0);
    for (size_t gi = 0; gi < groups.size(); gi++) {
      double gw = 0;
      for (const Tri& t : groups[gi].tris) {
        const double e1[3] = {t.v[1][0] - t.v[0][0], t.v[1][1] - t.v[0][1], t.v[1][2] - t.v[0][2]};
        const double e2[3] = {t.v[2][0] - t.v[0][0], t.v[2][1] - t.v[0][1], t.v[2][2] - t.v[0][2]};
        const double cr[3] = {e1[1] * e2[2] - e1[2] * e2[1], e1[2] * e2[0] - e1[0] * e2[2], e1[0] * e2[1] - e1[1] * e2[0]};
        const double area = 0.5 * len3(cr);
        for (int k = 0; k < 3; k++) gc[gi * 3 + k] += area * (t.v[0][k] + t.v[1][k] + t.v[2][k]) / 3.0;
        gw += area;
      }
      for (int k = 0; k < 3; k++) { cw[k] += gc[gi * 3 + k]; if (gw > 0) gc[gi * 3 + k] /= gw; }
      wsum += gw;
    }
    if (wsum > 0) for (int k = 0; k < 3; k++) cw[k] /= wsum;
    std::vector<int> cls(groups.size(), -1);
    std::vector<size_t> cls_first;
    for (size_t gi = 0; gi < groups.size(); gi++) {
      for (size_t c = 0; c < cls_first.size() && cls[gi] < 0; c++) {
        const Group& f = groups[cls_first[c]];
        const double dot = f.n[0] * groups[gi].n[0] + f.n[1] * groups[gi].n[1] + f.n[2] * groups[gi].n[2];
        const double sgn = dot < 0 ? -1.0 : 1.0;
        bool same = true;
        for (int k = 0; k < 3; k++) same = same && static_cast<float>(groups[gi].n[k]) == static_cast<float>(sgn * f.n[k]);
        if (same) {
          cls[gi] = static_cast<int>(c);
          for (int k = 0; k < 3; k++) groups[gi].n[k] = sgn * f.n[k];
          groups[gi].flip = dot < 0;
        }
      }
      if (cls[gi] < 0) { cls[gi] = static_cast<int>(cls_first.size()); cls_first.push_back(gi); }
    }
    auto dist2 = [&](size_t gi) { double d2 = 0; for (int k = 0; k < 3; k++) d2 += (gc[gi * 3 + k] - cw[k]) * (gc[gi * 3 + k] - cw[k]); return d2; };
    std::vector<double> cls_min(cls_first.size(), 1e300);
    for (size_t gi = 0; gi < groups.size(); gi++) cls_min[cls[gi]] = std::min(cls_min[cls[gi]], dist2(gi));
    std::vector<size_t> perm(groups.size());
    for (size_t gi = 0; gi < perm.size(); gi++) perm[gi] = gi;
    std::stable_sort(perm.begin(), perm.end(), [&](size_t x, size_t y) {
      if (cls[x] != cls[y]) return cls_min[cls[x]] != cls_min[cls[y]] ? cls_min[cls[x]] < cls_min[cls[y]] : cls[x] < cls[y];
      return dist2(x) < dist2(y);
    });
    std::vector<Group> sorted;
    int prev_cls = -1;
    for (size_t gi : perm) {
      sorted.push_back(groups[gi]);
      sorted.back().same_normal = cls[gi] == prev_cls;
      prev_cls = cls[gi];
    }
    groups.swap(sorted);
  }
  for (const Group& g : groups) {
    const size_t nt = g.tris.size();
    std::vector<int> partner(nt, -1), unshared(nt, -1);
    double pair_slack = 0;
    auto apart = [](const double* p, const double* r) { return std::max(std::fabs(p[0] - r[0]), std::max(std::fabs(p[1] - r[1]), std::fabs(p[2] - r[2]))); };
    for (size_t i = 0; i < nt; i++) {
      if (partner[i] >= 0) continue;
      for (size_t j = i + 1; j < nt && partner[i] < 0; j++) {
        if (partner[j] >= 0) continue;
        int match_i[3] = {-1, -1, -1}, n_shared = 0;
        bool used_j[3] = {false, false, false};
        double err = 0;
        for (int k = 0; k < 3; k++)
          for (int l = 0; l < 3; l++)
            if (!used_j[l] && match_i[k] < 0 && apart(g.tris[i].v[k], g.tris[j].v[l]) <= 1e-6 * diam) {
              match_i[k] = l; used_j[l] = true; n_shared++;
              err = std::max(err, apart(g.tris[i].v[k], g.tris[j].v[l]));
            }
        if (n_shared != 2) continue;
        int bi = -1, dj = -1;
        for (int k = 0; k < 3; k++) if (match_i[k] < 0) bi = k;
        for (int l = 0; l < 3; l++) if (!used_j[l]) dj = l;
        double expect[3];
        for (int c2 = 0; c2 < 3; c2++) {
          expect[c2] = -g.tris[i].v[bi][c2];
          for (int k = 0; k < 3; k++) if (k != bi) expect[c2] += g.tris[i].v[k][c2];
        }
        err = std::max(err, apart(expect, g.tris[j].v[dj]));
        if (err <= 1e-6 * diam) {
          partner[i] = static_cast<int>(j); partner[j] = static_cast<int>(i); unshared[i] = bi;
          pair_slack = std::max(pair_slack, 4.0 * err * std::max(g.tris[i].g, g.tris[j].g));
        }
      }
    }
    DevPlane p;
    std::memset(&p, 0, sizeof p);
    for (int k = 0; k < 3; k++) p.n[k] = static_cast<float>(g.flip ? -g.n[k] : g.n[k]);
    p.d0 = static_cast<float>(g.flip ? -g.d0 : g.d0); p.kt = static_cast<float>(g.kt * 1.0001); p.ktol = static_cast<float>((g.ktol + 4e-7 + pair_slack) * 1.0001);
    for (size_t i = 0; i < nt; i++) {
      if (partner[i] < 0 || static_cast<size_t>(partner[i]) < i) continue;
      const int bi = unshared[i], ai = (bi + 1) % 3;
      fp.tris.push_back(record(g.tris[i], bi, ai));
      fp.order.push_back(g.tris[i].index); fp.order.push_back(g.tris[static_cast<size_t>(partner[i])].index);
      p.n_pairs++;
    }
    for (size_t i = 0; i < nt; i++) {
      if (partner[i] >= 0) continue;
      fp.tris.push_back(record(g.tris[i], 1, 2));
      fp.order.push_back(g.tris[i].index);
      p.n_tris++;
    }
    if (g.same_normal) p.n_tris |= 0x80000000u;
    fp.planes.push_back(p);
  }
  {
    struct Span { size_t rec, slot; };
    std::vector<Span> span(fp.planes.size());
    { size_t rec = 0, slot = 0;
      for (size_t i = 0; i < fp.planes.size(); i++) {
        span[i] = Span{rec, slot};
        const uint32_t nt = fp.planes[i].n_tris & 0x7fffffffu, np = fp.planes[i].n_pairs;
        rec += np + nt; slot += 2 * np + nt;
      } }
    auto simple = [&](size_t i) { return fp.planes[i].n_pairs == 1 && (fp.planes[i].n_tris & 0x7fffffffu) == 0; };
    std::vector<char> in_slab(fp.planes.size(), 0);
    for (size_t i = 0; i + 1 < fp.planes.size(); i++)
      if (!in_slab[i] && simple(i) && simple(i + 1) && std::memcmp(fp.planes[i].n, fp.planes[i + 1].n, sizeof fp.planes[i].n) == 0) { in_slab[i] = in_slab[i + 1] = 1; i++; }
    std::vector<DevPlane> planes; std::vector<DevTriFilter> tris; std::vector<uint32_t> order;
    for (int pass = 0; pass < 2; pass++)
      for (size_t i = 0; i < fp.planes.size(); i++) {
        if ((in_slab[i] != 0) != (pass == 0)) continue;
        DevPlane q = fp.planes[i];
        const uint32_t nt = q.n_tris & 0x7fffffffu, np = q.n_pairs;
        q.n_tris = nt;
        if (!planes.empty() && std::memcmp(planes.back().n, q.n, sizeof q.n) == 0) q.n_tris |= 0x80000000u;
        planes.push_back(q);
        for (uint32_t k = 0; k < np + nt; k++) tris.push_back(fp.tris[span[i].rec + k]);
        for (uint32_t k = 0; k < 2 * np + nt; k++) order.push_back(fp.order[span[i].slot + k]);
        if (pass == 0) fp.n_simple_planes++;
      }
    fp.planes.swap(planes); fp.tris.swap(tris); fp.order.swap(order);
  }
  fp.n_prog_tris = static_cast<uint32_t>(fp.order.size());
  fp.order.insert(fp.order.end(), sphere_index.begin(), sphere_index.end());
  for (uint32_t idx : always_index) { fp.always_mask |= 1u << fp.order.size(); fp.order.push_back(idx); }
}

}
```

amber_amd/csrc/hip/lab_api.inc:

```

namespace {
constexpr const char* kKatNoRefBvh = "the known-answer kernels have no instantiation for AMBER_ENGINE_REFERENCE_BVH (its traversal stack belongs to the render kernels' grid): compare amber_hip_pt_signatures instead";
template <typename F>
void WithKatEngine(const amber_hip_pt* h, F&& f) {
  WithHitEngine(h->hit_engine, [&](auto engine) -> int { if constexpr (decltype(engine)::value != ENGINE_REF_BVH) f(engine); return AMBER_OK; });
}

int RenderPassWavefront(amber_hip_pt* h, uint32_t first_sample, uint32_t n_samples) {
  const uint32_t n_pixels = static_cast<uint32_t>(BandPixels(h));
  const uint64_t kMaxPaths = 1ull << 28;
  uint64_t max_chunks = kMaxPaths / (static_cast<uint64_t>(n_pixels) * AMBER_ACCUM_CHUNK);
  if (max_chunks == 0) return Fail(AMBER_EINVAL, "band too large for the wavefront engine");
  const uint32_t kMaxBounces = 4096;
  const uint64_t cap = max_chunks * AMBER_ACCUM_CHUNK;
  return SplitSamples(first_sample, n_samples, "band too large for the wavefront engine", [&](uint32_t left, amber_plan::Launch* l) -> int {
    *l = {left > cap ? static_cast<uint32_t>(cap) : left, 0};
    return AMBER_OK;
  }, [&](uint32_t first, const amber_plan::Launch& l, bool*) -> int {
    const uint32_t n = l.n;
    const uint32_t n_chunks = (n + AMBER_ACCUM_CHUNK - 1) / AMBER_ACCUM_CHUNK;
    const size_t n_paths = static_cast<size_t>(n_chunks) * n_pixels * AMBER_ACCUM_CHUNK;
    const size_t shard_capacity = ((n_paths + AMBER_WF_SHARDS - 1) / AMBER_WF_SHARDS + 63) / 64 * 64 + 64;
    const size_t q_len = shard_capacity * AMBER_WF_SHARDS;
    const size_t n_counts = static_cast<size_t>(kMaxBounces + 2) * AMBER_WF_SHARDS;
    const size_t bytes = (26 * q_len + 3 * n_paths) * 4 + n_counts * sizeof(unsigned int);
    AMBER_TRY(Grow(h, h->d_wf, bytes / sizeof(float), "wavefront queues"));
    float* base = h->d_wf;
    WfQueue q[2];
    for (int k = 0; k < 2; k++) {
      for (int c = 0; c < 9; c++) q[k].f[c] = base + (static_cast<size_t>(k) * 13 + c) * q_len;
      for (int c = 0; c < 4; c++) q[k].u[c] = reinterpret_cast<uint32_t*>(base + (static_cast<size_t>(k) * 13 + 9 + c) * q_len);
    }
    float* meas = base + 26 * q_len;
    unsigned int* counts = reinterpret_cast<unsigned int*>(meas + 3 * n_paths);
    HIP_TRY(hipMemsetAsync(counts, 0, n_counts * sizeof(unsigned int), h->stream));
    WfArgs a;
    a.scene = h->scene; a.meas = meas; a.counts = counts; a.ray_count = h->d_rays; a.hashed_seed = h->hashed_seed;
    a.SetBand(h->row_begin, h->stripe_rows, h->stripe_period); a.n_pixels = n_pixels;
    a.first_sample = first; a.n_samples = n; a.n_paths = static_cast<uint32_t>(n_paths); a.bounce = 0; a.shard_capacity = static_cast<uint32_t>(shard_capacity);
    const uint32_t n_blocks = 2048u;
    AMBER_TRY(TimedLaunch(h, true, [&]() -> int {
      a.out = q[0]; a.in = q[1];
      hipLaunchKernelGGL(wf_generate_kernel, dim3(n_blocks), dim3(256), 0, h->stream, a);
      HIP_TRY(hipGetLastError());
      uint32_t bounce = 0;
      for (;;) {
        const uint32_t burst = bounce < 16 ? 8 : 16;
        for (uint32_t k = 0; k < burst && bounce < kMaxBounces; k++, bounce++) {
          a.bounce = bounce; a.in = q[bounce & 1]; a.out = q[(bounce + 1) & 1];
          WithHitEngine(h->hit_engine, [&](auto engine) -> int {
            constexpr int kEngine = decltype(engine)::value == ENGINE_TWO_PHASE || decltype(engine)::value == ENGINE_BVH ? decltype(engine)::value : ENGINE_LIST;
            hipLaunchKernelGGL(wf_bounce_kernel<kEngine>, dim3(n_blocks), dim3(256), 0, h->stream, a);
            return AMBER_OK;
          });
          HIP_TRY(hipGetLastError());
        }
        unsigned int shard_live[AMBER_WF_SHARDS];
        HIP_TRY(hipMemcpyAsync(shard_live, counts + static_cast<size_t>(bounce) * AMBER_WF_SHARDS, sizeof shard_live, hipMemcpyDeviceToHost, h->stream));
        HIP_TRY(hipStreamSynchronize(h->stream));
        unsigned long long live = 0;
        for (unsigned int v : shard_live) live += v;
        if (live == 0) break;
        if (bounce >= kMaxBounces) return Fail(AMBER_EHIP, "wavefront engine: path longer than 4096 bounces");
      }
      return AMBER_OK;
    }));
    const uint32_t n_elems = n_pixels * 3u;
    hipLaunchKernelGGL(wf_reduce_kernel, dim3((n_elems + 255u) / 256u), dim3(256), 0, h->stream, h->d_fb, meas, n_pixels, n_chunks);
    HIP_TRY(hipGetLastError());
    return AMBER_OK;
  });
}

int LaunchLabRecords(amber_hip_pt* h, uint32_t n, uint32_t n_pixels, float* target, const RecordProducer& producer) {
  AMBER_TRY(BeginPathLaunch(h, n, n_pixels, false));
  RenderArgs a = MakeRenderArgs(h, h->hashed_seed, n_pixels, 0u, n);
  SetRecordArgs(h, a);
  a.n_items = n_pixels * n;
  AMBER_TRY(TimedLaunch(h, false, [&]() -> int {
    hipLaunchKernelGGL(kat_accumulate_kernel, dim3((producer.n_waves + 3u) / 4u), dim3(256), 0, h->stream, a, producer.q, producer.rgb, producer.n_items,
                       producer.n_waves, producer.rays);
    return AMBER_OK;
  }));
  return FinishPathLaunch(h, 0u, n, n_pixels, target, producer, false);
}

}

extern "C" {

int amber_hip_kat_cast(amber_hip_pt* h, uint32_t n, const float* origins, const float* dirs,
                       int32_t* out_object, float* out_t, float* out_pos, float* out_normal) { return Guarded("amber_hip_kat_cast", [&]() -> int {
  if (h && h->hit_engine == AMBER_ENGINE_REFERENCE_BVH) return Fail(AMBER_EINVAL, kKatNoRefBvh);
  if (!h || !origins || !dirs || !out_object || !out_t || !out_pos || !out_normal) return Fail(AMBER_EINVAL, "null argument");
  if (n == 0) return AMBER_OK;
  HIP_TRY(hipSetDevice(h->device));
  DevBuf<float> d_o, d_d, d_t, d_p, d_n; DevBuf<int32_t> d_i;
  HIP_TRY(d_o.alloc(3 * n)); HIP_TRY(d_d.alloc(3 * n)); HIP_TRY(d_t.alloc(n)); HIP_TRY(d_p.alloc(3 * n)); HIP_TRY(d_n.alloc(3 * n)); HIP_TRY(d_i.alloc(n));
  HIP_TRY(hipMemcpy(d_o.p, origins, 3ull * n * 4, hipMemcpyHostToDevice));
  HIP_TRY(hipMemcpy(d_d.p, dirs, 3ull * n * 4, hipMemcpyHostToDevice));
  WithKatEngine(h, [&](auto engine) { hipLaunchKernelGGL(kat_cast_kernel<decltype(engine)::value>, dim3((n + 255) / 256), dim3(256), 0, h->stream, h->scene, n, d_o.p, d_d.p, d_i.p, d_t.p, d_p.p, d_n.p); });
  HIP_TRY(hipGetLastError());
  HIP_TRY(hipStreamSynchronize(h->stream));
  HIP_TRY(hipMemcpy(out_object, d_i.p, 4ull * n, hipMemcpyDeviceToHost));
  HIP_TRY(hipMemcpy(out_t, d_t.p, 4ull * n, hipMemcpyDeviceToHost));
  HIP_TRY(hipMemcpy(out_pos, d_p.p, 12ull * n, hipMemcpyDeviceToHost));
  HIP_TRY(hipMemcpy(out_normal, d_n.p, 12ull * n, hipMemcpyDeviceToHost));
  return AMBER_OK;
}); }

int amber_hip_kat_sample(amber_hip_pt* h, uint32_t n, const uint32_t* material, const float* normals,
                         const float* dirs_out, uint64_t* rng_state, float* out_dir_in, float* out_weight) { return Guarded("amber_hip_kat_sample", [&]() -> int {
  if (!h || !material || !normals || !dirs_out || !rng_state || !out_dir_in || !out_weight) return Fail(AMBER_EINVAL, "null argument");
  if (n == 0) return AMBER_OK;
  for (uint32_t i = 0; i < n; i++)
    if ((material[i] & 0x7fffffffu) >= h->n_materials) return Fail(AMBER_EINVAL, "material index out of range");
  HIP_TRY(hipSetDevice(h->device));
  DevBuf<uint32_t> d_m; DevBuf<float> d_n, d_d, d_o, d_w; DevBuf<uint64_t> d_r;
  HIP_TRY(d_m.alloc(n)); HIP_TRY(d_n.alloc(3 * n)); HIP_TRY(d_d.alloc(3 * n)); HIP_TRY(d_o.alloc(3 * n)); HIP_TRY(d_w.alloc(3 * n)); HIP_TRY(d_r.alloc(n));
  HIP_TRY(hipMemcpy(d_m.p, material, 4ull * n, hipMemcpyHostToDevice));
  HIP_TRY(hipMemcpy(d_n.p, normals, 12ull * n, hipMemcpyHostToDevice));
  HIP_TRY(hipMemcpy(d_d.p, dirs_out, 12ull * n, hipMemcpyHostToDevice));
  HIP_TRY(hipMemcpy(d_r.p, rng_state, 8ull * n, hipMemcpyHostToDevice));
  hipLaunchKernelGGL(kat_sample_kernel, dim3((n + 255) / 256), dim3(256), 0, h->stream, h->scene, n, d_m.p, d_n.p, d_d.p, d_r.p, d_o.p, d_w.p);
  HIP_TRY(hipGetLastError());
  HIP_TRY(hipStreamSynchronize(h->stream));
  HIP_TRY(hipMemcpy(rng_state, d_r.p, 8ull * n, hipMemcpyDeviceToHost));
  HIP_TRY(hipMemcpy(out_dir_in, d_o.p, 12ull * n, hipMemcpyDeviceToHost));
  HIP_TRY(hipMemcpy(out_weight, d_w.p, 12ull * n, hipMemcpyDeviceToHost));
  return AMBER_OK;
}); }

int amber_hip_kat_eye(amber_hip_pt* h, uint32_t n, const uint32_t* pixel, const uint32_t* sample, float* out7) { return Guarded("amber_hip_kat_eye", [&]() -> int {
  if (!h || !pixel || !sample || !out7) return Fail(AMBER_EINVAL, "null argument");
  if (n == 0) return AMBER_OK;
  const uint32_t npx = h->scene.sensor.w * h->scene.sensor.h;
  for (uint32_t i = 0; i < n; i++) if (pixel[i] >= npx) return Fail(AMBER_EINVAL, "pixel index out of range");
  HIP_TRY(hipSetDevice(h->device));
  DevBuf<uint32_t> d_p, d_s; DevBuf<float> d_o;
  HIP_TRY(d_p.alloc(n)); HIP_TRY(d_s.alloc(n)); HIP_TRY(d_o.alloc(7 * n));
  HIP_TRY(hipMemcpy(d_p.p, pixel, 4ull * n, hipMemcpyHostToDevice));
  HIP_TRY(hipMemcpy(d_s.p, sample, 4ull * n, hipMemcpyHostToDevice));
  hipLaunchKernelGGL(kat_eye_kernel, dim3((n + 255) / 256), dim3(256), 0, h->stream, h->scene, h->hashed_seed, n, d_p.p, d_s.p, d_o.p);
  HIP_TRY(hipGetLastError());
  HIP_TRY(hipStreamSynchronize(h->stream));
  HIP_TRY(hipMemcpy(out7, d_o.p, 28ull * n, hipMemcpyDeviceToHost));
  return AMBER_OK;
}); }

int amber_hip_kat_light_ray(amber_hip_pt* h, uint32_t n, uint64_t* rng_state, float* out_origin, float* out_dir, float* out_weight,
                            uint32_t* out_light) { return Guarded("amber_hip_kat_light_ray", [&]() -> int {
  if (!h || !rng_state || !out_origin || !out_dir || !out_weight || !out_light) return Fail(AMBER_EINVAL, "null argument");
  if (h->scene.n_lights == 0) return Fail(AMBER_EINVAL, "amber_hip_kat_light_ray: the handle's scene has no lights");
  if (h->lights_stale) return Fail(AMBER_EINVAL, "lights are stale after amber_hip_pt_update_objects: re-create the handle");
  if (n == 0) return AMBER_OK;
  if (n > 0x3fffffffu) return Fail(AMBER_EINVAL, "too many items for one call");
  HIP_TRY(hipSetDevice(h->device));
  DevBuf<uint64_t> d_r; DevBuf<float> d_o, d_d, d_w; DevBuf<uint32_t> d_l;
  HIP_TRY(d_r.alloc(n)); HIP_TRY(d_o.alloc(3ull * n)); HIP_TRY(d_d.alloc(3ull * n)); HIP_TRY(d_w.alloc(3ull * n)); HIP_TRY(d_l.alloc(n));
  HIP_TRY(hipMemcpy(d_r.p, rng_state, 8ull * n, hipMemcpyHostToDevice));
  hipLaunchKernelGGL(kat_light_ray_kernel, dim3((n + 255) / 256), dim3(256), 0, h->stream, h->scene, n, d_r.p, d_o.p, d_d.p, d_w.p, d_l.p);
  HIP_TRY(hipGetLastError());
  HIP_TRY(hipStreamSynchronize(h->stream));
  HIP_TRY(hipMemcpy(rng_state, d_r.p, 8ull * n, hipMemcpyDeviceToHost));
  HIP_TRY(hipMemcpy(out_origin, d_o.p, 12ull * n, hipMemcpyDeviceToHost));
  HIP_TRY(hipMemcpy(out_dir, d_d.p, 12ull * n, hipMemcpyDeviceToHost));
  HIP_TRY(hipMemcpy(out_weight, d_w.p, 12ull * n, hipMemcpyDeviceToHost));
  HIP_TRY(hipMemcpy(out_light, d_l.p, 4ull * n, hipMemcpyDeviceToHost));
  return AMBER_OK;
}); }

int amber_hip_kat_lens_response(amber_hip_pt* h, uint32_t n, const float* position, const float* direction_out, uint32_t* out_reached,
                                uint32_t* out_pixel, float* out_value) { return Guarded("amber_hip_kat_lens_response", [&]() -> int {
  if (!h || !position || !direction_out || !out_reached || !out_pixel || !out_value) return Fail(AMBER_EINVAL, "null argument");
  if (n == 0) return AMBER_OK;
  if (n > 0x3fffffffu) return Fail(AMBER_EINVAL, "too many items for one call");
  HIP_TRY(hipSetDevice(h->device));
  DevBuf<float> d_p, d_d, d_v; DevBuf<uint32_t> d_r, d_x;
  HIP_TRY(d_p.alloc(3ull * n)); HIP_TRY(d_d.alloc(3ull * n)); HIP_TRY(d_v.alloc(n)); HIP_TRY(d_r.alloc(n)); HIP_TRY(d_x.alloc(n));
  HIP_TRY(hipMemcpy(d_p.p, position, 12ull * n, hipMemcpyHostToDevice));
  HIP_TRY(hipMemcpy(d_d.p, direction_out, 12ull * n, hipMemcpyHostToDevice));
  hipLaunchKernelGGL(kat_lens_response_kernel, dim3((n + 255) / 256), dim3(256), 0, h->stream, h->scene, n, d_p.p, d_d.p, d_r.p, d_x.p, d_v.p);
  HIP_TRY(hipGetLastError());
  HIP_TRY(hipStreamSynchronize(h->stream));
  HIP_TRY(hipMemcpy(out_reached, d_r.p, 4ull * n, hipMemcpyDeviceToHost));
  HIP_TRY(hipMemcpy(out_pixel, d_x.p, 4ull * n, hipMemcpyDeviceToHost));
  HIP_TRY(hipMemcpy(out_value, d_v.p, 4ull * n, hipMemcpyDeviceToHost));
  return AMBER_OK;
}); }

int amber_hip_kat_radiance(amber_hip_pt* h, uint32_t n, const uint32_t* material, const float* normals, const float* dirs_out,
                           float* out) { return Guarded("amber_hip_kat_radiance", [&]() -> int {
  if (!h || !material || !normals || !dirs_out || !out) return Fail(AMBER_EINVAL, "null argument");
  if (n == 0) return AMBER_OK;
  if (n > 0x3fffffffu) return Fail(AMBER_EINVAL, "too many items for one call");
  for (uint32_t i = 0; i < n; i++) if (material[i] >= h->n_materials) return Fail(AMBER_EINVAL, "material index out of range");
  HIP_TRY(hipSetDevice(h->device));
  DevBuf<uint32_t> d_m; DevBuf<float> d_n, d_d, d_o;
  HIP_TRY(d_m.alloc(n)); HIP_TRY(d_n.alloc(3ull * n)); HIP_TRY(d_d.alloc(3ull * n)); HIP_TRY(d_o.alloc(3ull * n));
  HIP_TRY(hipMemcpy(d_m.p, material, 4ull * n, hipMemcpyHostToDevice));
  HIP_TRY(hipMemcpy(d_n.p, normals, 12ull * n, hipMemcpyHostToDevice));
  HIP_TRY(hipMemcpy(d_d.p, dirs_out, 12ull * n, hipMemcpyHostToDevice));
  hipLaunchKernelGGL(kat_radiance_kernel, dim3((n + 255) / 256), dim3(256), 0, h->stream, h->scene, n, d_m.p, d_n.p, d_d.p, d_o.p);
  HIP_TRY(hipGetLastError());
  HIP_TRY(hipStreamSynchronize(h->stream));
  HIP_TRY(hipMemcpy(out, d_o.p, 12ull * n, hipMemcpyDeviceToHost));
  return AMBER_OK;
}); }

int amber_hip_kat_trace(amber_hip_pt* h, uint32_t n, const uint32_t* pixel, const uint32_t* sample,
                        uint32_t max_bounces, uint32_t* out_records, uint32_t* out_casts) { return Guarded("amber_hip_kat_trace", [&]() -> int {
  if (h && h->hit_engine == AMBER_ENGINE_REFERENCE_BVH) return Fail(AMBER_EINVAL, kKatNoRefBvh);
  if (!h || !pixel || !sample || !out_records || !out_casts || max_bounces == 0) return Fail(AMBER_EINVAL, "bad argument");
  if (n == 0) return AMBER_OK;
  const uint32_t npx = h->scene.sensor.w * h->scene.sensor.h;
  for (uint32_t i = 0; i < n; i++) if (pixel[i] >= npx) return Fail(AMBER_EINVAL, "pixel index out of range");
  HIP_TRY(hipSetDevice(h->device));
  DevBuf<uint32_t> d_p, d_s, d_r, d_c;
  const size_t nrec = static_cast<size_t>(n) * max_bounces * 11;
  HIP_TRY(d_p.alloc(n)); HIP_TRY(d_s.alloc(n)); HIP_TRY(d_r.alloc(nrec)); HIP_TRY(d_c.alloc(n));
  HIP_TRY(hipMemcpy(d_p.p, pixel, 4ull * n, hipMemcpyHostToDevice));
  HIP_TRY(hipMemcpy(d_s.p, sample, 4ull * n, hipMemcpyHostToDevice));
  HIP_TRY(hipMemsetAsync(d_r.p, 0, nrec * 4, h->stream));
  WithKatEngine(h, [&](auto engine) { hipLaunchKernelGGL(kat_trace_kernel<decltype(engine)::value>, dim3((n + 255) / 256), dim3(256), 0, h->stream, h->scene, h->hashed_seed, n, d_p.p, d_s.p, max_bounces, d_r.p, d_c.p); });
  HIP_TRY(hipGetLastError());
  HIP_TRY(hipStreamSynchronize(h->stream));
  HIP_TRY(hipMemcpy(out_records, d_r.p, nrec * 4, hipMemcpyDeviceToHost));
  HIP_TRY(hipMemcpy(out_casts, d_c.p, 4ull * n, hipMemcpyDeviceToHost));
  return AMBER_OK;
}); }

int amber_hip_kat_signatures(amber_hip_pt* h, uint32_t first_sample, uint32_t n_samples, uint64_t* out) { return Guarded("amber_hip_kat_signatures", [&]() -> int {
  if (h && h->hit_engine == AMBER_ENGINE_REFERENCE_BVH) return Fail(AMBER_EINVAL, kKatNoRefBvh);
  if (!h || !out || n_samples == 0) return Fail(AMBER_EINVAL, "bad argument");
  if (static_cast<uint64_t>(first_sample) + n_samples > 0xffffffffull) return Fail(AMBER_EINVAL, "sample index overflow");
  const uint64_t n = BandPixels(h) * n_samples;
  if (n == 0) return AMBER_OK;
  if ((n + 255) / 256 > 0x7fffffffull) return Fail(AMBER_EINVAL, "too many paths for one call");
  HIP_TRY(hipSetDevice(h->device));
  DevBuf<unsigned long long> d_out;
  HIP_TRY(d_out.alloc(n));
  const dim3 grid(static_cast<uint32_t>((n + 255) / 256));
  WithKatEngine(h, [&](auto engine) { hipLaunchKernelGGL(kat_signature_kernel<decltype(engine)::value>, grid, dim3(256), 0, h->stream, h->scene, h->hashed_seed, n, first_sample, n_samples, h->row_begin, h->stripe_rows, h->stripe_period, MakeExactDiv(h->stripe_rows), d_out.p); });
  HIP_TRY(hipGetLastError());
  HIP_TRY(hipStreamSynchronize(h->stream));
  HIP_TRY(hipMemcpy(out, d_out.p, n * sizeof(uint64_t), hipMemcpyDeviceToHost));
  return AMBER_OK;
}); }

int amber_hip_kat_traversal_rate(amber_hip_pt* h, uint32_t n, const float* origins, const float* dirs, uint32_t waves, uint32_t refill_min, uint32_t repeats,
                                 float* out_t, int32_t* out_object, double* best_ms, uint32_t* out_rounds) { return Guarded("amber_hip_kat_traversal_rate", [&]() -> int {
  if (!h || !origins || !dirs || !out_t || !out_object || n == 0) return Fail(AMBER_EINVAL, "bad argument");
  if (h->hit_engine != AMBER_ENGINE_BVH) return Fail(AMBER_EINVAL, "the handle's engine is not BVH");
  if (refill_min == 0 || refill_min > 64) return Fail(AMBER_EINVAL, "refill_min must be in [1, 64]");
  const uint64_t n_virtual = static_cast<uint64_t>(n) * (repeats ? repeats : 1u);
  if (n_virtual > 0xfffffeffull) return Fail(AMBER_EINVAL, "n * repeats must stay below 2^32");
  HIP_TRY(hipSetDevice(h->device));
  AMBER_TRY(ResolvePending(h));
  std::vector<float4> packed(2ull * n);
  for (uint32_t i = 0; i < n; i++) {
    packed[2ull * i] = make_float4(origins[3ull * i], origins[3ull * i + 1], origins[3ull * i + 2], 0.f);
    packed[2ull * i + 1] = make_float4(dirs[3ull * i], dirs[3ull * i + 1], dirs[3ull * i + 2], 0.f);
  }
  DevBuf<float4> d_rays; DevBuf<float2> d_out; DevBuf<unsigned int> d_next; DevBuf<int32_t> d_stack; DevBuf<uint32_t> d_rounds;
  if (out_rounds) HIP_TRY(d_rounds.alloc(n));
  HIP_TRY(d_rays.alloc(2ull * n)); HIP_TRY(d_out.alloc(n)); HIP_TRY(d_next.alloc(1));
  const uint32_t n_blocks = static_cast<uint32_t>(h->n_cus) * (waves >= 4 && waves <= 8 ? waves : 5u);
  HIP_TRY(d_stack.alloc(static_cast<size_t>(n_blocks) * 256u * AMBER_BVH_STACK));
  HIP_TRY(hipMemcpy(d_rays.p, packed.data(), packed.size() * sizeof(float4), hipMemcpyHostToDevice));
  Event ev0, ev1;
  HIP_TRY(hipEventCreate(&ev0.v)); HIP_TRY(hipEventCreate(&ev1.v));
  const hipEvent_t e0 = ev0.v, e1 = ev1.v;
  double best = 1e300;
  const uint32_t nv = static_cast<uint32_t>(n_virtual);
  for (uint32_t rep = 0; rep < 2u; rep++) {
    HIP_TRY(hipMemsetAsync(d_next.p, 0, sizeof(unsigned int), h->stream));
    HIP_TRY(hipEventRecord(e0, h->stream));
    switch (waves) {
      case 4: hipLaunchKernelGGL((bvh_trace_rate_kernel<4, 24>), dim3(n_blocks), dim3(256), 0, h->stream, h->scene, nv, d_rays.p, d_out.p, d_next.p, d_stack.p, refill_min, n, d_rounds.p); break;
      case 6: hipLaunchKernelGGL((bvh_trace_rate_kernel<6, 24>), dim3(n_blocks), dim3(256), 0, h->stream, h->scene, nv, d_rays.p, d_out.p, d_next.p, d_stack.p, refill_min, n, d_rounds.p); break;
      case 8: hipLaunchKernelGGL((bvh_trace_rate_kernel<8, 16>), dim3(n_blocks), dim3(256), 0, h->stream, h->scene, nv, d_rays.p, d_out.p, d_next.p, d_stack.p, refill_min, n, d_rounds.p); break;
      default: hipLaunchKernelGGL((bvh_trace_rate_kernel<5, 24>), dim3(n_blocks), dim3(256), 0, h->stream, h->scene, nv, d_rays.p, d_out.p, d_next.p, d_stack.p, refill_min, n, d_rounds.p); break;
    }
    HIP_TRY(hipGetLastError());
    HIP_TRY(hipEventRecord(e1, h->stream));
    HIP_TRY(hipStreamSynchronize(h->stream));
    float ms = 0; HIP_TRY(hipEventElapsedTime(&ms, e0, e1));
    if (rep == 1u || ms < best) best = ms;
  }
  std::vector<float2> res(n);
  HIP_TRY(hipMemcpy(res.data(), d_out.p, n * sizeof(float2), hipMemcpyDeviceToHost));
  if (out_rounds) HIP_TRY(hipMemcpy(out_rounds, d_rounds.p, n * sizeof(uint32_t), hipMemcpyDeviceToHost));
  std::vector<uint32_t> prims(h->scene.n_objects);
  HIP_TRY(hipMemcpy(prims.data(), h->scene.bvh_prims, prims.size() * sizeof(uint32_t), hipMemcpyDeviceToHost));
  for (uint32_t i = 0; i < n; i++) {
    int32_t slot; std::memcpy(&slot, &res[i].y, 4);
    out_object[i] = slot < 0 ? -1 : static_cast<int32_t>(prims[slot]);
    out_t[i] = slot < 0 ? std::nanf("") : res[i].x;
  }
  if (best_ms) *best_ms = best;
  return AMBER_OK;
}); }

int amber_hip_kat_pixel_masks(amber_hip_pt* h, uint32_t* out_mask, uint32_t* out_slot_of_object, uint32_t* out_always_mask, double* kernel_ms) { return Guarded("amber_hip_kat_pixel_masks", [&]() -> int {
  if (!h) return Fail(AMBER_EINVAL, "null handle");
  if (!h->two_phase) return Fail(AMBER_EINVAL, "pixel masks belong to the two-phase engine");
  HIP_TRY(hipSetDevice(h->device));
  AMBER_TRY(ResolvePending(h));
  const uint32_t n_pixels = static_cast<uint32_t>(BandPixels(h));
  if (out_mask || kernel_ms) {
    float ms = 0;
    AMBER_TRY(StartPixelMasks(h, kernel_ms ? &ms : nullptr));
    if (!h->pixel_mask_ready) return Fail(AMBER_EINVAL, "pixel masks are switched off (AMBER_PIXEL_MASK=0) or the band is empty");
    HIP_TRY(hipStreamSynchronize(h->stream));
    if (out_mask) HIP_TRY(hipMemcpy(out_mask, h->d_pixel_mask, static_cast<size_t>(n_pixels) * sizeof(uint32_t), hipMemcpyDeviceToHost));
    if (kernel_ms) *kernel_ms = static_cast<double>(ms);
  }
  if (out_slot_of_object) {
    for (uint32_t i = 0; i < h->scene.n_objects; i++) out_slot_of_object[i] = 0xffffffffu;
    for (size_t k = 0; k < h->prog_order.size(); k++) if (h->prog_order[k] < h->scene.n_objects) out_slot_of_object[h->prog_order[k]] = static_cast<uint32_t>(k);
  }
  if (out_always_mask) *out_always_mask = h->scene.always_mask | h->scene.blade_mask;
  return AMBER_OK;
}); }

int amber_hip_kat_bvh_dump(amber_hip_pt* h, uint32_t* nodes, uint32_t node_capacity, uint32_t* prims, uint32_t prim_capacity, AmberBvhDump* info) { return Guarded("amber_hip_kat_bvh_dump", [&]() -> int {
  if (!h || !info) return Fail(AMBER_EINVAL, "null argument");
  if (h->hit_engine != AMBER_ENGINE_BVH) return Fail(AMBER_EINVAL, "the handle's engine is not BVH");
  HIP_TRY(hipSetDevice(h->device));
  AMBER_TRY(ResolvePending(h));
  HIP_TRY(hipStreamSynchronize(h->stream));
  static_assert(sizeof(DevBvhNodeQ) == 8 * sizeof(uint32_t), "a dumped node is 8 words");
  info->n_nodes = h->build.n_nodes; info->n_prims = h->scene.n_objects; info->root = h->scene.bvh_root; info->depth = h->build.depth;
  for (int c = 0; c < 3; c++) { info->gmin[c] = h->scene.bvh_gmin[c]; info->step[c] = h->scene.bvh_step[c]; info->reach[c] = h->scene.bvh_reach[c]; }
  const uint32_t n_nodes = std::min(node_capacity, info->n_nodes), n_prims = std::min(prim_capacity, info->n_prims);
  if (nodes && n_nodes) HIP_TRY(hipMemcpy(nodes, h->scene.bvh_nodes, static_cast<size_t>(n_nodes) * sizeof(DevBvhNodeQ), hipMemcpyDeviceToHost));
  if (prims && n_prims) HIP_TRY(hipMemcpy(prims, h->scene.bvh_prims, static_cast<size_t>(n_prims) * sizeof(uint32_t), hipMemcpyDeviceToHost));
  return AMBER_OK;
}); }

int amber_hip_pt_signatures(amber_hip_pt* h, uint32_t first_sample, uint32_t n_samples, uint64_t* out) { return Guarded("amber_hip_pt_signatures", [&]() -> int {
  if (!h || !out || n_samples == 0) return Fail(AMBER_EINVAL, "bad argument");
  if (static_cast<uint64_t>(first_sample) + n_samples > 0xffffffffull) return Fail(AMBER_EINVAL, "sample index overflow");
  if (h->engine == AMBER_ENGINE_WAVEFRONT) return Fail(AMBER_EINVAL, "signatures come from the work-queue kernels (engines list, two_phase, bvh)");
  const uint32_t n_pixels = static_cast<uint32_t>(BandPixels(h));
  const uint64_t n = static_cast<uint64_t>(n_pixels) * n_samples;
  if (n == 0) return AMBER_OK;
  if (n > kMaxPathsPerLaunch) return Fail(AMBER_EINVAL, "too many paths for one call");
  HIP_TRY(hipSetDevice(h->device));
  AMBER_TRY(ResolvePending(h));
  HIP_TRY(hipStreamSynchronize(h->stream));
  AMBER_TRY(Grow(h, h->d_sig, n, "signatures"));
  HIP_TRY(hipMemsetAsync(h->d_sig, 0, n * sizeof(unsigned long long), h->stream));
  AMBER_TRY(RenderSamples(h, first_sample, n_samples, n_pixels, h->d_fb, h->d_sig));
  HIP_TRY(hipStreamSynchronize(h->stream));
  HIP_TRY(hipMemcpy(out, h->d_sig, n * sizeof(uint64_t), hipMemcpyDeviceToHost));
  return AMBER_OK;
}); }

int amber_hip_kat_lt_accumulate(amber_hip_pt* h, const AmberSplat* records, uint32_t n) { return Guarded("amber_hip_kat_lt_accumulate", [&]() -> int {
  if (!h || (n && !records)) return Fail(AMBER_EINVAL, "null argument");
  if (!WholeFrame(h)) return Fail(AMBER_EINVAL, "amber_hip_kat_lt_accumulate: the handle renders a band or stripes of the frame");
  if (n > 0x7fffffffu) return Fail(AMBER_EINVAL, "too many records for one call");
  const uint32_t npx = h->scene.sensor.w * h->scene.sensor.h;
  for (uint32_t i = 0; i < n; i++) if (records[i].pixel >= npx) return Fail(AMBER_EINVAL, "pixel index out of range");
  if (n == 0) return AMBER_OK;
  HIP_TRY(hipSetDevice(h->device));
  AMBER_TRY(ResolvePending(h));
  AMBER_TRY(EnsureLtSplats(h, n));
  static_assert(sizeof(AmberSplat) == sizeof(DevSplat), "splat layouts must agree");
  HIP_TRY(hipMemcpyAsync(h->d_splats, records, static_cast<size_t>(n) * sizeof(DevSplat), hipMemcpyHostToDevice, h->stream));
  HIP_TRY(hipMemsetAsync(h->lt.longest.p, 0, sizeof(unsigned int), h->stream));
  AMBER_TRY(LtAccumulate(h, n, 32u));
  HIP_TRY(hipStreamSynchronize(h->stream));
  return AMBER_OK;
}); }

int amber_hip_kat_accumulate(amber_hip_pt* h, uint32_t n_samples, const uint32_t* q, const float* rgb, uint32_t n_items, uint32_t n_waves, uint32_t rec_capacity,
                             uint64_t rays, AmberAccumulateInfo* info) { return Guarded("amber_hip_kat_accumulate", [&]() -> int {
  if (info) *info = AmberAccumulateInfo{};
  if (!h || (n_items && (!q || !rgb))) return Fail(AMBER_EINVAL, "null argument");
  if (n_samples == 0 || n_waves == 0) return Fail(AMBER_EINVAL, "amber_hip_kat_accumulate: n_samples and n_waves must not be zero");
  if (n_waves > (1u << 20)) return Fail(AMBER_EINVAL, "amber_hip_kat_accumulate: more than 2^20 waves");
  const uint64_t n_paths = BandPixels(h) * n_samples;
  if (n_paths >= (1ull << 32)) return Fail(AMBER_EINVAL, "amber_hip_kat_accumulate: n_pixels * n_samples must stay below 2^32");
  {
    std::vector<uint32_t> seen;
    seen.reserve(n_items);
    for (uint32_t i = 0; i < n_items; i++) {
      if (q[i] == AMBER_REC_UNUSED) continue;
      if (q[i] >= n_paths) return Fail(AMBER_EINVAL, "amber_hip_kat_accumulate: item " + std::to_string(i) + ": path index out of range");
      seen.push_back(q[i]);
    }
    std::sort(seen.begin(), seen.end());
    if (std::adjacent_find(seen.begin(), seen.end()) != seen.end()) return Fail(AMBER_EINVAL, "amber_hip_kat_accumulate: a path index occurs twice");
  }
  HIP_TRY(hipSetDevice(h->device));
  AMBER_TRY(ResolvePending(h));
  PathLaunchBufs& p = h->paths;
  if (rec_capacity != 0 && rec_capacity < p.rec_capacity)
    return Fail(AMBER_EINVAL, "amber_hip_kat_accumulate: rec_capacity " + std::to_string(rec_capacity) + " is below the " + std::to_string(p.rec_capacity) + " slots the handle's record buffer has");
  const uint32_t n_pixels = static_cast<uint32_t>(BandPixels(h));
  if (n_pixels == 0) return AMBER_OK;
  AMBER_TRY(EnsureRecordCapacity(h, rec_capacity ? rec_capacity : static_cast<uint64_t>(n_items) + RecordSlack(h)));
  DevBuf<uint32_t> d_q; DevBuf<float> d_rgb;
  HIP_TRY(d_q.alloc(n_items ? n_items : 1u)); HIP_TRY(d_rgb.alloc(n_items ? 3ull * n_items : 1u));
  if (n_items) {
    HIP_TRY(hipMemcpy(d_q.p, q, 4ull * n_items, hipMemcpyHostToDevice));
    HIP_TRY(hipMemcpy(d_rgb.p, rgb, 12ull * n_items, hipMemcpyHostToDevice));
  }
  RecordProducer producer;
  producer.lab = true; producer.q = d_q.p; producer.rgb = d_rgb.p; producer.n_items = n_items; producer.n_waves = n_waves; producer.rays = rays;
  const uint64_t launches0 = p.n_launches, repeats0 = p.n_repeats;
  AMBER_TRY(LaunchLabRecords(h, n_samples, n_pixels, h->d_fb, producer));
  const int rc = ResolvePending(h);
  p.pending = false; p.pending_producer = RecordProducer{};
  AMBER_TRY(rc);
  const size_t used_words = static_cast<size_t>((n_paths + 31u) / 32u);
  std::vector<uint32_t> words(used_words);
  if (used_words) HIP_TRY(hipMemcpyAsync(words.data(), p.flags, used_words * sizeof(uint32_t), hipMemcpyDeviceToHost, h->stream));
  HIP_TRY(hipStreamSynchronize(h->stream));
  if (info) {
    info->n_launches = static_cast<uint32_t>(p.n_launches - launches0); info->n_repeats = static_cast<uint32_t>(p.n_repeats - repeats0);
    info->rec_count = *p.h_rec_count.v;
    info->flag_words_set = static_cast<uint32_t>(std::count_if(words.begin(), words.end(), [](uint32_t w) { return w != 0u; }));
    info->flags_dirty = p.flags_dirty ? 1u : 0u;
  }
  return AMBER_OK;
}); }

int amber_hip_kat_lt_stage_ms(amber_hip_pt* h, double* sort_ms, double* sum_ms) { return Guarded("amber_hip_kat_lt_stage_ms", [&]() -> int {
  if (!h) return Fail(AMBER_EINVAL, "null handle");
  h->lt.stage_timing = true;
  if (sort_ms) *sort_ms = h->lt.sort_ms;
  if (sum_ms) *sum_ms = h->lt.sum_ms;
  h->lt.sort_ms = h->lt.sum_ms = 0;
  return AMBER_OK;
}); }

int amber_hip_kat_photon_stage_ms(amber_hip_pt* h, double* trace_ms, double* sort_ms, double* gather_ms) { return Guarded("amber_hip_kat_photon_stage_ms", [&]() -> int {
  if (!h) return Fail(AMBER_EINVAL, "null handle");
  PhotonBufs& s = h->photons;
  s.stage_timing = true;
  if (trace_ms) *trace_ms = s.trace_ms;
  if (sort_ms) *sort_ms = s.sort_ms;
  if (gather_ms) *gather_ms = s.gather_ms;
  s.trace_ms = s.sort_ms = s.gather_ms = 0;
  return AMBER_OK;
}); }

int amber_hip_kat_math(int device, int mode, uint32_t n, const float* x, float* out) { return Guarded("amber_hip_kat_math", [&]() -> int {
  if (!x || !out || mode < 0 || mode > 3) return Fail(AMBER_EINVAL, "bad argument");
  if (n == 0) return AMBER_OK;
  int n_dev = 0;
  if (hipGetDeviceCount(&n_dev) != hipSuccess || device < 0 || device >= n_dev) return Fail(AMBER_ENODEVICE, "no such HIP device");
  HIP_TRY(hipSetDevice(device));
  const size_t n_in = mode == 1 ? 2ull * n : n, n_out = mode == 1 ? n : 2ull * n;
  DevBuf<float> d_x, d_o;
  HIP_TRY(d_x.alloc(n_in)); HIP_TRY(d_o.alloc(n_out));
  HIP_TRY(hipMemcpy(d_x.p, x, n_in * 4, hipMemcpyHostToDevice));
  hipLaunchKernelGGL(kat_math_kernel, dim3((n + 255) / 256), dim3(256), 0, 0, mode, n, d_x.p, d_o.p);
  HIP_TRY(hipGetLastError());
  HIP_TRY(hipDeviceSynchronize());
  HIP_TRY(hipMemcpy(out, d_o.p, n_out * 4, hipMemcpyDeviceToHost));
  return AMBER_OK;
}); }

int amber_hip_kat_division(int device, int mode, uint32_t n, const float* x, float* out) { return Guarded("amber_hip_kat_division", [&]() -> int {
  if (!x || !out || mode < 0 || mode > 3) return Fail(AMBER_EINVAL, "bad argument");
  if (n == 0) return AMBER_OK;
  if (n > 0x3fffffffu) return Fail(AMBER_EINVAL, "too many groups for one call");
  int n_dev = 0;
  if (hipGetDeviceCount(&n_dev) != hipSuccess || device < 0 || device >= n_dev) return Fail(AMBER_ENODEVICE, "no such HIP device");
  HIP_TRY(hipSetDevice(device));
  DevBuf<float> d_x, d_o;
  HIP_TRY(d_x.alloc(4ull * n)); HIP_TRY(d_o.alloc(3ull * n));
  HIP_TRY(hipMemcpy(d_x.p, x, 16ull * n, hipMemcpyHostToDevice));
  hipLaunchKernelGGL(kat_division_kernel, dim3((n + 255) / 256), dim3(256), 0, 0, mode, n, d_x.p, d_o.p);
  HIP_TRY(hipGetLastError());
  HIP_TRY(hipDeviceSynchronize());
  HIP_TRY(hipMemcpy(out, d_o.p, 12ull * n, hipMemcpyDeviceToHost));
  return AMBER_OK;
}); }

int amber_hip_kat_sqrt(int device, int mode, uint32_t n, const float* x, float* out) { return Guarded("amber_hip_kat_sqrt", [&]() -> int {
  if (!x || !out || mode < 0 || mode > 4) return Fail(AMBER_EINVAL, "bad argument");
  if (n == 0) return AMBER_OK;
  if (n > 0x3fffffffu) return Fail(AMBER_EINVAL, "too many items for one call");
  int n_dev = 0;
  if (hipGetDeviceCount(&n_dev) != hipSuccess || device < 0 || device >= n_dev) return Fail(AMBER_ENODEVICE, "no such HIP device");
  HIP_TRY(hipSetDevice(device));
  const size_t width = mode <= 1 ? 1u : (mode <= 3 ? 3u : 2u);
  DevBuf<float> d_x, d_o;
  HIP_TRY(d_x.alloc(width * n)); HIP_TRY(d_o.alloc(width * n));
  HIP_TRY(hipMemcpy(d_x.p, x, width * n * 4, hipMemcpyHostToDevice));
  hipLaunchKernelGGL(kat_sqrt_kernel, dim3((n + 255) / 256), dim3(256), 0, 0, mode, n, d_x.p, d_o.p);
  HIP_TRY(hipGetLastError());
  HIP_TRY(hipDeviceSynchronize());
  HIP_TRY(hipMemcpy(out, d_o.p, width * n * 4, hipMemcpyDeviceToHost));
  return AMBER_OK;
}); }

int amber_hip_kat_sqrt_sweep(int device, uint32_t first_bits, uint64_t count, AmberSqrtSweep* out) { return Guarded("amber_hip_kat_sqrt_sweep", [&]() -> int {
  if (!out || count == 0 || static_cast<uint64_t>(first_bits) + count > (1ull << 32)) return Fail(AMBER_EINVAL, "bad argument");
  int n_dev = 0;
  if (hipGetDeviceCount(&n_dev) != hipSuccess || device < 0 || device >= n_dev) return Fail(AMBER_ENODEVICE, "no such HIP device");
  HIP_TRY(hipSetDevice(device));
  static_assert(sizeof(SqrtSweepCounters) == sizeof(AmberSqrtSweep), "the kernel's counters are the C record");
  DevBuf<SqrtSweepCounters> d_c;
  HIP_TRY(d_c.alloc(1));
  HIP_TRY(hipMemset(d_c.p, 0, sizeof(SqrtSweepCounters)));
  const uint64_t blocks = (count + 255u) / 256u;
  hipLaunchKernelGGL(kat_sqrt_sweep_kernel, dim3(static_cast<uint32_t>(blocks < 8192u ? blocks : 8192u)), dim3(256), 0, 0, first_bits, static_cast<unsigned long long>(count), d_c.p);
  HIP_TRY(hipGetLastError());
  HIP_TRY(hipDeviceSynchronize());
  HIP_TRY(hipMemcpy(out, d_c.p, sizeof(SqrtSweepCounters), hipMemcpyDeviceToHost));
  return AMBER_OK;
}); }

}
```

amber_amd/csrc/hip/lab_kernels.inc:

```

template <int kEngine>
__global__ void kat_cast_kernel(const DevScene sc, uint32_t n, const float* org, const float* dir,
                                int32_t* out_obj, float* out_t, float* out_pos, float* out_n) {
  const uint32_t i = blockIdx.x * blockDim.x + threadIdx.x;
  const uint32_t k = ClampToLastItem(i, n);
  const EngineLds lds = StageEngineLds<kEngine, AMBER_BVH_STACK>(sc);
  const V3 o = ld3(org + 3 * k), d = ld3(dir + 3 * k);
  HitRec h;
#ifdef AMBER_STAMPS
  StampCtx stamp_store{}; StampCtx* stamp_ctx = &stamp_store;
#endif
  ClosestHit<kEngine>(sc, lds.objects, lds.stack, o, d, -1, h AMBER_STAMP_ARG);
  if (i >= n) return;
  out_obj[i] = h.idx;
  if (h.idx < 0) {
    out_t[i] = __builtin_nanf("");
    for (int c = 0; c < 3; c++) { out_pos[3 * i + c] = 0.f; out_n[3 * i + c] = 0.f; }
    return;
  }
  V3 pos, nrm; uint32_t mat;
  ResolveHit<kEngine>(sc, lds.objects, h, o, d, pos, nrm, mat);
  out_t[i] = h.t;
  out_pos[3 * i] = pos.x; out_pos[3 * i + 1] = pos.y; out_pos[3 * i + 2] = pos.z;
  out_n[3 * i] = nrm.x; out_n[3 * i + 1] = nrm.y; out_n[3 * i + 2] = nrm.z;
}

__global__ void kat_sample_kernel(const DevScene sc, uint32_t n, const uint32_t* material, const float* normals,
                                  const float* dirs_out, uint64_t* rng_state, float* out_dir, float* out_w) {
  const uint32_t i = blockIdx.x * blockDim.x + threadIdx.x;
  if (i >= n) return;
  const DevMaterial m = sc.materials[material[i] & 0x7fffffffu];
  uint64_t rng = rng_state[i];
  V3 di, w;
  if (material[i] >> 31) SampleImportance(m, ld3(normals + 3 * i), ld3(dirs_out + 3 * i), rng, di, w);
  else SampleLight(m, ld3(normals + 3 * i), ld3(dirs_out + 3 * i), rng, di, w);
  rng_state[i] = rng;
  out_dir[3 * i] = di.x; out_dir[3 * i + 1] = di.y; out_dir[3 * i + 2] = di.z;
  out_w[3 * i] = w.x; out_w[3 * i + 1] = w.y; out_w[3 * i + 2] = w.z;
}

__global__ void kat_eye_kernel(const DevScene sc, uint64_t hashed_seed, uint32_t n, const uint32_t* pixel,
                               const uint32_t* sample, float* out7) {
  const uint32_t i = blockIdx.x * blockDim.x + threadIdx.x;
  if (i >= n) return;
  uint64_t rng = XorShiftSeed(hashed_seed, pixel[i], sample[i]);
  V3 o, d; float w; int origin_slot;
  GenerateEyeRay(sc, pixel[i] % sc.sensor.w, pixel[i] / sc.sensor.w, rng, o, d, w, origin_slot);
  float* p = out7 + 7 * i;
  p[0] = o.x; p[1] = o.y; p[2] = o.z; p[3] = d.x; p[4] = d.y; p[5] = d.z; p[6] = w;
}

__global__ void kat_light_ray_kernel(const DevScene sc, uint32_t n, uint64_t* rng_state, float* out_org, float* out_dir, float* out_w, uint32_t* out_light) {
  const uint32_t i = blockIdx.x * blockDim.x + threadIdx.x;
  if (i >= n) return;
  uint64_t rng = rng_state[i];
  uint64_t first = rng;
  const float x = Uniform(first) * sc.total_power;
  uint32_t pos = 0;
  while (pos + 1u < sc.n_lights && sc.lights[pos].cum_power < x) ++pos;
  V3 o, d, w; int origin_slot;
  GenerateLightRay(sc, rng, o, d, w, origin_slot);
  rng_state[i] = rng;
  out_org[3 * i] = o.x; out_org[3 * i + 1] = o.y; out_org[3 * i + 2] = o.z;
  out_dir[3 * i] = d.x; out_dir[3 * i + 1] = d.y; out_dir[3 * i + 2] = d.z;
  out_w[3 * i] = w.x; out_w[3 * i + 1] = w.y; out_w[3 * i + 2] = w.z;
  out_light[i] = pos;
}

__global__ void kat_lens_response_kernel(const DevScene sc, uint32_t n, const float* position, const float* direction_out,
                                         uint32_t* out_reached, uint32_t* out_pixel, float* out_value) {
  const uint32_t i = blockIdx.x * blockDim.x + threadIdx.x;
  if (i >= n) return;
  uint32_t pixel = 0u; float value = 0.f;
  const bool reached = LensResponse(sc, ld3(position + 3 * i), ld3(direction_out + 3 * i), pixel, value);
  out_reached[i] = reached ? 1u : 0u;
  out_pixel[i] = reached ? pixel : 0u;
  out_value[i] = reached ? value : 0.f;
}

__global__ void kat_radiance_kernel(const DevScene sc, uint32_t n, const uint32_t* material, const float* normals, const float* dirs_out, float* out) {
  const uint32_t i = blockIdx.x * blockDim.x + threadIdx.x;
  if (i >= n) return;
  const V3 r = Radiance(sc.materials[material[i]], ld3(normals + 3 * i), ld3(dirs_out + 3 * i));
  out[3 * i] = r.x; out[3 * i + 1] = r.y; out[3 * i + 2] = r.z;
}

template <int kEngine>
__global__ void kat_trace_kernel(const DevScene sc, uint64_t hashed_seed, uint32_t n, const uint32_t* pixel,
                                 const uint32_t* sample, uint32_t max_bounces, uint32_t* out_records, uint32_t* out_casts) {
  const uint32_t i = blockIdx.x * blockDim.x + threadIdx.x;
  const uint32_t k = ClampToLastItem(i, n);
  const EngineLds lds = StageEngineLds<kEngine, AMBER_BVH_STACK>(sc);
  uint64_t rng = XorShiftSeed(hashed_seed, pixel[k], sample[k]);
  V3 o, d; float ew; int origin_slot;
  GenerateEyeRay(sc, pixel[k] % sc.sensor.w, pixel[k] / sc.sensor.w, rng, o, d, ew, origin_slot);
  V3 w = v3(ew, ew, ew), meas = v3(0.f, 0.f, 0.f);
  uint32_t casts = 0;
  bool alive = true;
  while (__any(alive)) {
    if (alive) {
      Bounce b;
#ifdef AMBER_STAMPS
      StampCtx stamp_store{}; StampCtx* stamp_ctx = &stamp_store;
#endif
      alive = PathStep<true, kEngine>(sc, lds.objects, lds.stack, o, d, w, meas, rng, casts, origin_slot, &b AMBER_STAMP_ARG);
      if (i < n && casts <= max_bounces) {
        uint32_t* r = out_records + (static_cast<size_t>(i) * max_bounces + (casts - 1)) * 11u;
        r[0] = static_cast<uint32_t>(b.object);
        r[1] = __float_as_uint(b.t);
        r[2] = __float_as_uint(b.pos.x); r[3] = __float_as_uint(b.pos.y); r[4] = __float_as_uint(b.pos.z);
        r[5] = __float_as_uint(b.weight_before.x); r[6] = __float_as_uint(b.weight_before.y); r[7] = __float_as_uint(b.weight_before.z);
        r[8] = __float_as_uint(meas.x); r[9] = __float_as_uint(meas.y); r[10] = __float_as_uint(meas.z);
      }
    }
  }
  if (i < n) out_casts[i] = casts;
}

template <int kEngine>
__global__ void kat_signature_kernel(const DevScene sc, uint64_t hashed_seed, uint64_t n, uint32_t first_sample, uint32_t n_samples,
                                     uint32_t row_begin, uint32_t stripe_rows, uint32_t stripe_period, ExactDiv div_stripe_rows, unsigned long long* out) {
  const uint64_t i = static_cast<uint64_t>(blockIdx.x) * blockDim.x + threadIdx.x;
  const uint64_t k = ClampToLastItem(i, n);
  const EngineLds lds = StageEngineLds<kEngine, AMBER_BVH_STACK>(sc);
  const uint32_t plocal = static_cast<uint32_t>(k / n_samples), smp = first_sample + static_cast<uint32_t>(k % n_samples);
  const uint32_t lrow = plocal / sc.sensor.w, px = plocal - lrow * sc.sensor.w;
  const uint32_t py = FrameRow(row_begin, stripe_rows, stripe_period, div_stripe_rows, lrow);
  uint64_t rng = XorShiftSeed(hashed_seed, px + py * sc.sensor.w, smp);
  V3 o, d; float ew; int origin_slot;
  GenerateEyeRay(sc, px, py, rng, o, d, ew, origin_slot);
  V3 w = v3(ew, ew, ew), meas = v3(0.f, 0.f, 0.f);
  uint32_t casts = 0, sig_obj = 2166136261u, sig_t = 2166136261u;
  bool alive = true;
  while (__any(alive)) {
    if (alive) {
      Bounce b;
#ifdef AMBER_STAMPS
      StampCtx stamp_store{}; StampCtx* stamp_ctx = &stamp_store;
#endif
      alive = PathStep<true, kEngine>(sc, lds.objects, lds.stack, o, d, w, meas, rng, casts, origin_slot, &b AMBER_STAMP_ARG);
      sig_obj = Fnv32(sig_obj, static_cast<uint32_t>(b.object));
      if (b.object >= 0) sig_t = Fnv32(sig_t, __float_as_uint(b.t));
    }
  }
  if (i < n) out[i] = static_cast<unsigned long long>(sig_obj) | (static_cast<unsigned long long>(sig_t) << 32);
}

__global__ void __launch_bounds__(256) kat_accumulate_kernel(const RenderArgs a, const uint32_t* __restrict__ q, const float* __restrict__ rgb, uint32_t n_items,
                                                             uint32_t n_waves, unsigned long long rays) {
  const uint32_t wave = (blockIdx.x * blockDim.x + threadIdx.x) >> 6, lane = threadIdx.x & 63u;
  if (wave >= n_waves) return;
  const uint32_t n_trips = n_items / 64u + (n_items % 64u != 0u);
  uint32_t rec_next = 0u, rec_end = 0u;
  for (uint32_t t = wave; t < n_trips; t += n_waves) {
    const uint64_t i = static_cast<uint64_t>(t) * 64u + lane;
    const uint32_t path = i < n_items ? q[i] : AMBER_REC_UNUSED;
    const bool emit = path != AMBER_REC_UNUSED;
    const V3 meas = emit ? ld3(rgb + 3u * i) : v3(0.f, 0.f, 0.f);
    EmitRecords(a, emit, path, meas, rec_next, rec_end);
  }
  CloseRecords(a, rec_next, rec_end);
  if (wave == 0u && lane == 0u) atomicAdd(a.ray_count, rays);
}

__global__ void kat_math_kernel(int mode, uint32_t n, const float* x, float* out) {
  const uint32_t i = blockIdx.x * blockDim.x + threadIdx.x;
  if (i >= n) return;
  if (mode == 0) { float s, c; SinCos(x[i], s, c); out[2 * i] = s; out[2 * i + 1] = c; }
  else if (mode == 1) out[i] = Pow(x[2 * i], x[2 * i + 1]);
  else {
    const double d = mode == 2 ? Pow4(x[i]) : Pow5(x[i]);
    const unsigned long long b = static_cast<unsigned long long>(__double_as_longlong(d));
    out[2 * i] = __uint_as_float(static_cast<uint32_t>(b)); out[2 * i + 1] = __uint_as_float(static_cast<uint32_t>(b >> 32));
  }
}

__global__ void kat_division_kernel(int mode, uint32_t n, const float* x, float* out) {
  const uint32_t i = blockIdx.x * blockDim.x + threadIdx.x;
  const uint32_t k = ClampToLastItem(i, n);
  const float a = x[4ull * k], b = x[4ull * k + 1], c = x[4ull * k + 2], d = x[4ull * k + 3];
  V3 q;
  if (mode == 0) shared_div::Div3(a, b, c, d, q.x, q.y, q.z);
  else if (mode == 1) q = v3(a / d, b / d, c / d);
  else if (mode == 2) q = Normalize<true>(v3(a, b, c));
  else q = Normalize<false>(v3(a, b, c));
  if (i >= n) return;
  out[3ull * i] = q.x; out[3ull * i + 1] = q.y; out[3ull * i + 2] = q.z;
}

__global__ void kat_sqrt_kernel(int mode, uint32_t n, const float* x, float* out) {
  const uint32_t i = blockIdx.x * blockDim.x + threadIdx.x;
  const size_t k = ClampToLastItem(i, n);
  if (mode <= 1) {
    const float v = x[k];
    const float s = mode == 0 ? exact_sqrt::Sqrt1(v) : __builtin_sqrtf(v);
    if (i < n) out[i] = s;
  } else if (mode <= 3) {
    const V3 v = v3(x[3 * k], x[3 * k + 1], x[3 * k + 2]);
    const V3 q = mode == 2 ? Normalize<true, SQRT_FUSED>(v) : Normalize<false>(v);
    if (i < n) { out[3ull * i] = q.x; out[3ull * i + 1] = q.y; out[3ull * i + 2] = q.z; }
  } else {
    float sa, sb;
    exact_sqrt::Sqrt2(x[2 * k], x[2 * k + 1], sa, sb);
    if (i < n) { out[2ull * i] = sa; out[2ull * i + 1] = sb; }
  }
}

struct SqrtSweepCounters { unsigned long long mismatches, in_range; uint32_t n_offenders, offenders[8]; int32_t seed_low, seed_high; };
__global__ void kat_sqrt_sweep_kernel(uint32_t first_bits, unsigned long long count, SqrtSweepCounters* counters) {
  const unsigned long long stride = static_cast<unsigned long long>(gridDim.x) * blockDim.x;
  uint32_t mismatches = 0, in_range = 0;
  int32_t low = 0, high = 0;
  for (unsigned long long i = static_cast<unsigned long long>(blockIdx.x) * blockDim.x + threadIdx.x; i < count; i += stride) {
    const uint32_t bits = first_bits + static_cast<uint32_t>(i);
    const float x = __uint_as_float(bits);
    const float fast = exact_sqrt::Sqrt1(x), plain = __builtin_sqrtf(x);
    if (__float_as_uint(fast) != __float_as_uint(plain)) {
      ++mismatches;
      const uint32_t slot = atomicAdd(&counters->n_offenders, 1u);
      if (slot < 8u) counters->offenders[slot] = bits;
    }
    if (exact_sqrt::ExactSqrtSafe(x)) {
      ++in_range;
      const float nearest = static_cast<float>(1.0 / __builtin_sqrt(static_cast<double>(x)));
      const int32_t distance = static_cast<int32_t>(__float_as_uint(__builtin_amdgcn_rsqf(x))) - static_cast<int32_t>(__float_as_uint(nearest));
      low = distance < low ? distance : low;
      high = distance > high ? distance : high;
    }
  }
  for (int step = 32; step > 0; step >>= 1) {
    const int32_t other_low = __shfl_xor(low, step), other_high = __shfl_xor(high, step);
    low = other_low < low ? other_low : low;
    high = other_high > high ? other_high : high;
    mismatches += __shfl_xor(mismatches, step);
    in_range += __shfl_xor(in_range, step);
  }
  if ((threadIdx.x & 63u) == 0u) {
    if (mismatches) atomicAdd(&counters->mismatches, static_cast<unsigned long long>(mismatches));
    if (in_range) atomicAdd(&counters->in_range, static_cast<unsigned long long>(in_range));
    if (low < 0) atomicMin(&counters->seed_low, low);
    if (high > 0) atomicMax(&counters->seed_high, high);
  }
}
```

amber_amd/csrc/hip/scene_prep.h:

```cpp
#pragma once

#include <algorithm>
#include <chrono>
#include <cmath>
#include <cstdio>
#include <cstdlib>
#include <cstring>
#include <string>
#include <vector>

#include "../../../include/amber_hip.h"
#include "bvh_build.h"
#include "filter_build.h"
#include "ref_bvh_build.h"

namespace amber_prep {

using namespace amber_dev;

constexpr uint32_t kHitTwoPhaseN = 5;
constexpr uint32_t kTwoPhaseAutoObjects = 80;

struct EnvSwitches {
  uint32_t two_phase_auto = kTwoPhaseAutoObjects;
  int bvh_pool = -1;
  uint32_t bvh_shade_batch = 0;
  bool bvh_paths_off = false;
  uint32_t bvh_paths_max_depth = 0xffffffffu;
  bool debug_bvh = false, debug_filter = false;
  bool pixel_mask = true;
  uint32_t pixel_mask_block = 0;
  double test_density_scale = 0;
  uint32_t test_device_build_max_depth = 0;
};

inline EnvSwitches ReadEnv() {
  EnvSwitches e;
  const char* ev;
  if ((ev = std::getenv("AMBER_TWO_PHASE_MAX_OBJECTS")) && std::atoi(ev) >= 0) e.two_phase_auto = std::min<uint32_t>(AMBER_MAX_GROUP_OBJECTS, static_cast<uint32_t>(std::atoi(ev)));
#ifdef AMBER_LAB
  if ((ev = std::getenv("AMBER_BVH_POOL")) && (ev[0] == '0' || ev[0] == '1')) e.bvh_pool = ev[0] == '1';
#endif
  if ((ev = std::getenv("AMBER_BVH_SHADE_BATCH")) && std::atoi(ev) >= 1 && std::atoi(ev) <= 64) e.bvh_shade_batch = static_cast<uint32_t>(std::atoi(ev));
  e.bvh_paths_off = (ev = std::getenv("AMBER_BVH_PATHS")) && ev[0] == '0';
  if ((ev = std::getenv("AMBER_BVH_PATHS_MAX_DEPTH"))) e.bvh_paths_max_depth = static_cast<uint32_t>(std::atoi(ev));
  e.debug_bvh = std::getenv("AMBER_DEBUG_BVH") != nullptr;
  e.debug_filter = std::getenv("AMBER_DEBUG_FILTER") != nullptr;
  e.pixel_mask = !((ev = std::getenv("AMBER_PIXEL_MASK")) && ev[0] == '0');
  if ((ev = std::getenv("AMBER_PIXEL_MASK_BLOCK")) && (ev[0] == '1' || ev[0] == '2' || ev[0] == '4') && ev[1] == 0) e.pixel_mask_block = static_cast<uint32_t>(ev[0] - '0');
  if ((ev = std::getenv("AMBER_TEST_RECORD_DENSITY_SCALE"))) e.test_density_scale = std::atof(ev);
  if ((ev = std::getenv("AMBER_TEST_DEVICE_BUILD_MAX_DEPTH")) && std::atoi(ev) > 0) e.test_device_build_max_depth = static_cast<uint32_t>(std::atoi(ev));
  return e;
}

struct SceneState {
  uint32_t engine = AMBER_ENGINE_LIST;
  uint32_t hit_engine = AMBER_ENGINE_LIST;
  bool two_phase = false;
  bool bvh_pool = false;
  bool bvh_paths = false;
  uint32_t bvh_shade_batch = 0;
  DevScene scene{};
  DevLens lens{};
  float aperture_rect[4][3] = {};
  std::vector<uint32_t> prog_order;
  std::vector<DevPlane> host_planes;
  AmberBuildInfo build{};
};

inline void ChooseBvhScheduler(SceneState& st, size_t n_objects, size_t n_triangles, uint32_t flags, const EnvSwitches& env,
                               size_t n_nodes, uint32_t depth, uint32_t path_bvh_stack, uint32_t shade_batch) {
  st.bvh_paths = !st.bvh_pool && !(flags & AMBER_PT_FLAG_BVH_ITEMS) && st.engine != AMBER_ENGINE_WAVEFRONT && depth <= path_bvh_stack;
  st.bvh_shade_batch = 2u * n_triangles > n_objects ? 40u : shade_batch;
  if (env.bvh_shade_batch) st.bvh_shade_batch = env.bvh_shade_batch;
  if (env.bvh_paths_off || env.bvh_paths_max_depth < depth) st.bvh_paths = false;
  if (env.debug_bvh) std::fprintf(stderr, "amber_hip: BVH of %zu objects: %zu nodes, depth %u; scheduler %s, shading batch %u\n", n_objects, n_nodes, depth,
                                  st.bvh_pool ? "pt_bvh_pool_kernel" : (st.bvh_paths ? "pt_megakernel<ENGINE_BVH>" : "pt_bvh_megakernel"), st.bvh_shade_batch);
}
inline size_t CountTriangles(const std::vector<DevObject>& objs) {
  size_t n_triangles = 0;
  for (const DevObject& ob : objs) n_triangles += (ob.kind & 0xffu) == AMBER_PRIM_TRIANGLE ? 1u : 0u;
  return n_triangles;
}
inline void ChooseBvhScheduler(SceneState& st, const std::vector<DevObject>& objs, const AmberPtParams* params, const EnvSwitches& env,
                               size_t n_nodes, uint32_t depth, uint32_t path_bvh_stack, uint32_t shade_batch) {
  ChooseBvhScheduler(st, objs.size(), CountTriangles(objs), params->reserved, env, n_nodes, depth, path_bvh_stack, shade_batch);
}

inline amber_bvh::FlatBvh BuildHostTree(SceneState& st, const std::vector<DevObject>& objs, const AmberPtParams* params, const EnvSwitches& env,
                                        uint32_t path_bvh_stack, uint32_t shade_batch) {
  const auto t0 = std::chrono::steady_clock::now();
  amber_bvh::FlatBvh bvh = amber_bvh::BuildBvh(objs);
  st.build.tree_ms += std::chrono::duration<double, std::milli>(std::chrono::steady_clock::now() - t0).count();
  if (env.debug_bvh) {
    const amber_bvh::BvhQuality q = amber_bvh::MeasureBvh(bvh.nodes, bvh.root_ref);
    std::fprintf(stderr, "amber_hip: BVH %s: SAH inner-node term %.3f, leaf term %.3f (x objects %.3f), leaf volume / scene volume %.3f; %u inner nodes, %u leaves, %u levels\n",
                 "as built", q.inner_area, q.leaf_area, q.leaf_object_area, q.leaf_volume, q.inner, q.leaves, q.depth);
  }
  ChooseBvhScheduler(st, objs, params, env, bvh.nodes.size(), bvh.depth, path_bvh_stack, shade_batch);
  st.build.where = st.build.fallback_reason ? AMBER_BUILD_HOST_FALLBACK : AMBER_BUILD_HOST;
  st.build.n_nodes = static_cast<uint32_t>(bvh.nodes.size()); st.build.n_leaves = st.build.n_nodes + 1u; st.build.depth = bvh.depth;
  return bvh;
}

inline void SetBvhRayMargin(DevScene& sc, const float bounds_min[3], const float bounds_max[3], bool has_spheres, float min_sphere_radius) {
  double d2 = 0;
  for (int c = 0; c < 3; c++) {
    sc.bvh_center[c] = 0.5f * (bounds_min[c] + bounds_max[c]);
    const double e = double(bounds_max[c]) - bounds_min[c];
    d2 += e * e;
  }
  sc.bvh_half_diag = static_cast<float>(0.5 * std::sqrt(d2) * 1.0001);
  sc.bvh_inv_rmin = !has_spheres ? 0.0f : (min_sphere_radius > 0 ? static_cast<float>(std::min(3.0e38, 1.0001 / min_sphere_radius)) : 3.0e38f);
}


inline void DeriveLens(const AmberFlatThinLens& L, const AmberFlatObject* blade_records, const AmberSensor& sensor, const float fp_center[3], float fp_reach,
                       DevLens& lens, std::vector<DevBlade>& blades, float aperture_rect[4][3]) {
  blades.resize(L.n_blades);
  for (uint32_t i = 0; i < L.n_blades; i++) {
    const AmberFlatObject& f = blade_records[i];
    for (int c = 0; c < 3; c++) { blades[i].v0[c] = f.p[c]; blades[i].v1[c] = f.p[3 + c]; blades[i].v2[c] = f.p[6 + c]; blades[i].n[c] = f.p[9 + c]; }
    blades[i].slot = -1; blades[i].pad[0] = blades[i].pad[1] = blades[i].pad[2] = 0;
  }
  {
    double lo[2] = {1e300, 1e300}, hi[2] = {-1e300, -1e300};
    for (const DevBlade& bl : blades)
      for (const float* v : {bl.v0, bl.v1, bl.v2}) {
        const double r[3] = {double(v[0]) - L.origin[0], double(v[1]) - L.origin[1], double(v[2]) - L.origin[2]};
        for (int c = 0; c < 2; c++) {
          const double x = L.local_[3 * c] * r[0] + L.local_[3 * c + 1] * r[1] + L.local_[3 * c + 2] * r[2];
          lo[c] = std::min(lo[c], x); hi[c] = std::max(hi[c], x);
        }
      }
    double world_mag = 0;
    for (int c = 0; c < 3; c++) world_mag = std::max({world_mag, std::fabs(double(fp_center[c])) + fp_reach, std::fabs(double(L.origin[c]))});
    for (int c = 0; c < 2; c++) { const double m = 1e-3 * (hi[c] - lo[c]) + 1e-6 + 1e-5 * fp_reach + 32.0 * 5.9604644775390625e-08 * world_mag; lo[c] -= m; hi[c] += m; }
    for (int i = 0; i < 4; i++) {
      const double x = (i & 1) ? hi[0] : lo[0], y = (i & 2) ? hi[1] : lo[1];
      for (int c = 0; c < 3; c++) aperture_rect[i][c] = static_cast<float>(L.origin[c] + (L.kind == AMBER_LENS_PINHOLE ? 0.0 : L.global_[3 * c] * x + L.global_[3 * c + 1] * y));
    }
  }
  std::memset(&lens, 0, sizeof lens);
  std::memcpy(lens.origin, L.origin, sizeof L.origin);
  std::memcpy(lens.global_, L.global_, sizeof L.global_);
  std::memcpy(lens.local_, L.local_, sizeof L.local_);
  lens.focus_distance = L.focus_distance; lens.sensor_distance = L.sensor_distance; lens.p_area = L.p_area;
  { volatile float q = -L.focus_distance / L.sensor_distance; lens.neg_fd_over_sd = q; }
  {
    volatile float size_f = static_cast<float>(static_cast<uint64_t>(sensor.width) * sensor.height);
    volatile float area = sensor.scene_width * sensor.scene_height;
    volatile float r = size_f / area;
    lens.size_over_area = r;
  }
  lens.sd2 = static_cast<double>(L.sensor_distance) * static_cast<double>(L.sensor_distance);
  lens.n_blades = L.n_blades; lens.n_blades_f = static_cast<float>(L.n_blades);
  lens.kind = L.kind;
  { volatile float area = sensor.scene_width * sensor.scene_height; volatile float inv = 1.0f / area; lens.inv_scene_area = inv; }
  { volatile float q = -L.sensor_distance / L.focus_distance; lens.neg_sd_over_fd = q; }
  {
    double world_mag = 0, min_edge = 1e300;
    for (int c = 0; c < 3; c++) world_mag = std::max(world_mag, std::fabs(double(L.origin[c])));
    for (const DevBlade& bl : blades) {
      const float* v[3] = {bl.v0, bl.v1, bl.v2};
      for (int k = 0; k < 3; k++) {
        double e2 = 0;
        for (int c = 0; c < 3; c++) { const double e = double(v[k][c]) - v[(k + 1) % 3][c]; e2 += e * e; world_mag = std::max(world_mag, std::fabs(double(v[k][c]))); }
        min_edge = std::min(min_edge, std::sqrt(e2));
      }
    }
    const double tol = min_edge > 0 ? std::max(1e-3, 64.0 * 5.9604644775390625e-08 * world_mag / min_edge) : 1.0;
    lens.edge_tol = static_cast<float>(std::min(1.0, tol));
  }
}

inline void DeriveLensOfState(const SceneState& st, const AmberFlatThinLens& L, const AmberFlatObject* blade_records,
                              DevLens& lens, std::vector<DevBlade>& blades, float aperture_rect[4][3]) {
  const AmberSensor sensor{st.scene.sensor.w, st.scene.sensor.h, st.scene.sensor.sw, st.scene.sensor.sh};
  DeriveLens(L, blade_records, sensor, st.scene.fp_center, st.scene.fp_reach, lens, blades, aperture_rect);
}

struct PreparedScene : SceneState {
  std::string error;
  bool bvh_pending = false;
  uint32_t ref_depth = 0;
  std::vector<DevObject> objects;
  std::vector<DevMaterial> materials;
  std::vector<DevBlade> blades;
  std::vector<DevPlane> planes;
  std::vector<DevTriFilter> tri_filters;
  std::vector<DevSphereFilter> sphere_filters;
  std::vector<DevObject> prog_objects;
  std::vector<DevFilterGroup> groups;
  std::vector<DevLight> lights;
  std::vector<DevBvhNodeQ> bvh_nodes;
  std::vector<DevBvhNodeQ4> bvh_nodes4;
  std::vector<uint32_t> bvh_prims;
  std::vector<DevObject> bvh_objects;
  std::vector<float4> bvh_spheres, bvh_tris;
  std::vector<DevRefNode> ref_nodes;
  std::vector<DevRefLeaf> ref_leaves;
};

inline void FillBvhArrays(SceneState& st, PreparedScene& p, const std::vector<DevObject>& objs, amber_bvh::FlatBvh& bvh) {
  const auto t0 = std::chrono::steady_clock::now();
  amber_bvh::QuantizedBvh qbvh = amber_bvh::QuantizeBvh(bvh.nodes, bvh.root_ref, [&](uint32_t slot) { return objs[bvh.prim_index[slot]].kind & 0xffu; });
#if AMBER_BVH_WIDE
  {
    amber_bvh::QuantizedBvh4 q4 = amber_bvh::CollapseBvh4(bvh.nodes, bvh.root_ref, qbvh, [&](uint32_t slot) { return objs[bvh.prim_index[slot]].kind & 0xffu; });
    p.bvh_nodes4 = std::move(q4.nodes);
    qbvh.root_ref = q4.root_ref;
  }
#endif
  p.bvh_nodes = std::move(qbvh.nodes);
  {
    std::vector<DevObject>& leaf_order = p.bvh_objects;
    std::vector<float4>& leaf_spheres = p.bvh_spheres;
    leaf_order.resize(bvh.prim_index.size());
    leaf_spheres.resize(bvh.prim_index.size());
    for (size_t k = 0; k < leaf_order.size(); k++) {
      const DevObject& ob = objs[bvh.prim_index[k]];
      leaf_order[k] = ob;
      leaf_spheres[k] = (ob.kind & 0xffu) == AMBER_PRIM_SPHERE ? make_float4(ob.a[0], ob.a[1], ob.a[2], ob.radius) : make_float4(0.f, 0.f, 0.f, 0.f);
    }
    bool any_tri = false;
    for (const DevObject& ob : leaf_order) any_tri = any_tri || (ob.kind & 0xffu) == AMBER_PRIM_TRIANGLE;
    std::vector<float4>& leaf_tris = p.bvh_tris;
    leaf_tris.resize(any_tri ? 3 * leaf_order.size() : 0);
    for (size_t k = 0; any_tri && k < leaf_order.size(); k++) {
      const DevObject& ob = leaf_order[k];
      if ((ob.kind & 0xffu) != AMBER_PRIM_TRIANGLE) { leaf_tris[3 * k] = leaf_tris[3 * k + 1] = leaf_tris[3 * k + 2] = make_float4(0.f, 0.f, 0.f, 0.f); continue; }
      float idx; const uint32_t scene_index = bvh.prim_index[k]; std::memcpy(&idx, &scene_index, 4);
      leaf_tris[3 * k] = make_float4(ob.a[0], ob.a[1], ob.a[2], ob.e1[0]);
      leaf_tris[3 * k + 1] = make_float4(ob.e1[1], ob.e1[2], ob.e2[0], ob.e2[1]);
      leaf_tris[3 * k + 2] = make_float4(ob.e2[2], idx, 0.f, 0.f);
    }
  }
  p.bvh_prims = std::move(bvh.prim_index);
  DevScene& sc = st.scene;
  sc.bvh_root = qbvh.root_ref;
  for (int c = 0; c < 3; c++) { sc.bvh_gmin[c] = qbvh.gmin[c]; sc.bvh_step[c] = qbvh.step[c]; sc.bvh_reach[c] = qbvh.reach[c]; }
  SetBvhRayMargin(sc, bvh.bounds_min, bvh.bounds_max, bvh.has_spheres, bvh.min_sphere_radius);
  if (st.hit_engine == AMBER_ENGINE_BVH) st.build.tree_ms += std::chrono::duration<double, std::milli>(std::chrono::steady_clock::now() - t0).count();
}

inline void HostBvhFallback(SceneState& st, PreparedScene& p, uint32_t reason, const AmberPtParams* params, const EnvSwitches& env, uint32_t path_bvh_stack, uint32_t shade_batch) {
  st.build.fallback_reason = reason;
  amber_bvh::FlatBvh bvh = BuildHostTree(st, p.objects, params, env, path_bvh_stack, shade_batch);
  FillBvhArrays(st, p, p.objects, bvh);
  p.bvh_pending = false;
}

inline PreparedScene PrepareScene(const AmberFlatScene* s, const AmberSensor* sensor, const AmberPtParams* params, const EnvSwitches& env,
                                  uint32_t path_bvh_stack, uint32_t shade_batch) {
  PreparedScene p;
  p.bvh_shade_batch = shade_batch;
  std::vector<DevObject>& objs = p.objects;
  objs.resize(s->n_objects);
  for (uint32_t i = 0; i < s->n_objects; i++) {
    const AmberFlatObject& f = s->objects[i];
    DevObject& o = objs[i];
    std::memset(&o, 0, sizeof o);
    o.kind = f.kind; o.material = f.material;
    o.a[0] = f.p[0]; o.a[1] = f.p[1]; o.a[2] = f.p[2];
    if (f.kind == AMBER_PRIM_TRIANGLE) {
      for (int c = 0; c < 3; c++) {
        volatile float e1 = f.p[3 + c] - f.p[c];
        volatile float e2 = f.p[6 + c] - f.p[c];
        o.e1[c] = e1; o.e2[c] = e2; o.n[c] = f.p[9 + c];
      }
    } else if (f.kind == AMBER_PRIM_SPHERE) {
      o.radius = f.p[3];
    } else {
      o.e1[0] = f.p[3]; o.e1[1] = f.p[4]; o.e1[2] = f.p[5]; o.radius = f.p[6]; o.height = f.p[7];
    }
  }
  p.materials.resize(s->n_materials);
  for (uint32_t i = 0; i < s->n_materials; i++) {
    const AmberFlatMaterial& f = s->materials[i];
    DevMaterial& m = p.materials[i];
    std::memset(&m, 0, sizeof m);
    m.kind = f.kind; m.rho[0] = f.rho[0]; m.rho[1] = f.rho[1]; m.rho[2] = f.rho[2]; m.param = f.param; m.r0 = f.r0;
    volatile float e1 = f.param + 1.0f, e2 = f.param + 2.0f;
    if (f.kind == AMBER_MAT_PHONG) { volatile float a = 1.0f / e1, b = e2 / e1; m.aux0 = a; m.aux1 = b; }
    else if (f.kind == AMBER_MAT_REFRACTION) { volatile float a = 1.0f / f.param; m.aux0 = a; }
  }
  const AmberFlatThinLens& L = s->lens;
  std::vector<DevBlade>& blades = p.blades;

  const uint32_t auto_hit = s->n_objects <= AMBER_MAX_LDS_OBJECTS ? AMBER_ENGINE_TWO_PHASE : (s->n_objects <= env.two_phase_auto ? kHitTwoPhaseN : AMBER_ENGINE_BVH);
  p.engine = params->engine != AMBER_ENGINE_AUTO ? params->engine : (auto_hit == kHitTwoPhaseN ? static_cast<uint32_t>(AMBER_ENGINE_TWO_PHASE) : auto_hit);
  p.hit_engine = p.engine == AMBER_ENGINE_WAVEFRONT ? (s->n_objects <= AMBER_MAX_LDS_OBJECTS ? AMBER_ENGINE_TWO_PHASE : AMBER_ENGINE_BVH) : p.engine;
  if (p.hit_engine == AMBER_ENGINE_TWO_PHASE && s->n_objects > AMBER_MAX_LDS_OBJECTS) p.hit_engine = kHitTwoPhaseN;
  p.two_phase = p.hit_engine == AMBER_ENGINE_TWO_PHASE || p.hit_engine == kHitTwoPhaseN;
#ifdef AMBER_LAB
  p.bvh_pool = env.bvh_pool >= 0 ? env.bvh_pool == 1 : (params->reserved & AMBER_PT_FLAG_BVH_POOL) != 0u;
#endif
  amber_bvh::FlatBvh bvh;
  if (p.hit_engine == AMBER_ENGINE_BVH) {
    const bool device_build = (params->reserved & AMBER_PT_FLAG_DEVICE_BUILD) != 0u;
#if AMBER_BVH_WIDE
    if (device_build) p.build.fallback_reason = AMBER_BUILD_REASON_WIDE;
    bvh = BuildHostTree(p, objs, params, env, path_bvh_stack, shade_batch);
#else
    if (device_build) p.bvh_pending = true;
    else bvh = BuildHostTree(p, objs, params, env, path_bvh_stack, shade_batch);
#endif
  }
  amber_refbvh::FlatTree ref_tree;
  if (p.hit_engine == AMBER_ENGINE_REFERENCE_BVH) {
    const amber_refbvh::Tree tree = amber_refbvh::Build(s->objects, s->n_objects);
    if (tree.too_deep) { p.error = "AMBER_ENGINE_REFERENCE_BVH: the reference's recursive build goes deeper than " + std::to_string(amber_refbvh::kMaxDepth) + " levels on this scene"; return p; }
    ref_tree = amber_refbvh::Flatten(tree, s->objects);
    p.ref_depth = tree.depth;
    bvh.prim_index = tree.order;
    if (env.debug_bvh)
      std::fprintf(stderr, "amber_hip: reference BVH of %u objects: %u inner nodes, %u leaves (largest %u objects), depth %u\n", s->n_objects, tree.n_inner, tree.n_leaves, tree.largest_leaf, tree.depth);
  }
  amber_filter::FilterProgram fprog;
  float fp_center[3] = {0, 0, 0}, fp_reach = 0;
  {
    double lo[3] = {L.origin[0], L.origin[1], L.origin[2]}, hi[3] = {L.origin[0], L.origin[1], L.origin[2]};
    for (const DevObject& ob : objs) {
      const amber_bvh::Box bx = amber_bvh::ObjectBox(ob);
      for (int c = 0; c < 3; c++) { lo[c] = std::min<double>(lo[c], bx.mn[c]); hi[c] = std::max<double>(hi[c], bx.mx[c]); }
    }
    double reach = 0;
    for (int c = 0; c < 3; c++) { fp_center[c] = static_cast<float>(0.5 * (lo[c] + hi[c])); reach = std::max(reach, 0.5 * (hi[c] - lo[c])); }
    fp_reach = static_cast<float>(std::min(3.0e38, 2.0 * reach + 1e-3));
  }
  DeriveLens(L, s->objects + L.first_blade_object, *sensor, fp_center, fp_reach, p.lens, blades, p.aperture_rect);
  std::vector<amber_filter::FilterProgram> more_progs;
  if (p.hit_engine == kHitTwoPhaseN) {
    std::vector<uint32_t> order;
    for (uint32_t i = 0; i < L.n_blades; i++) order.push_back(L.first_blade_object + i);
    for (uint32_t i = 0; i < s->n_objects; i++) if (i < L.first_blade_object || i >= L.first_blade_object + L.n_blades) order.push_back(i);
    for (size_t first = 0; first < order.size(); first += 32) {
      const std::vector<uint32_t> members(order.begin() + first, order.begin() + std::min(order.size(), first + 32));
      if (first == 0) amber_filter::BuildFilterProgram(objs, fp_center, fprog, &members);
      else { more_progs.emplace_back(); amber_filter::BuildFilterProgram(objs, fp_center, more_progs.back(), &members); }
    }
  } else if (p.two_phase) amber_filter::BuildFilterProgram(objs, fp_center, fprog);
  if (p.two_phase && env.debug_filter) {
    uint32_t pairs = 0, singles = 0;
    uint32_t shared = 0;
    for (const DevPlane& pl : fprog.planes) { pairs += pl.n_pairs; singles += pl.n_tris & 0x7fffffffu; shared += pl.n_tris >> 31; }
    std::fprintf(stderr, "amber_hip: filter program%s: %zu planes (%u share the previous plane's normal), %u pair records, %u single records, %zu spheres, always mask %#x; %zu group(s) of <= 32 objects\n",
                 more_progs.empty() ? "" : " of group 0", fprog.planes.size(), shared, pairs, singles, fprog.spheres.size(), fprog.always_mask, more_progs.size() + 1);
  }
  p.prog_order = fprog.order;
  p.host_planes = fprog.planes;
  for (uint32_t i = 0; i < L.n_blades; i++)
    for (uint32_t k = 0; k < fprog.n_prog_tris; k++)
      if (fprog.order[k] == L.first_blade_object + i) blades[i].slot = static_cast<int32_t>(k);
  p.lights.resize(s->n_lights);
  for (uint32_t i = 0; i < s->n_lights; i++) {
    const AmberFlatLight& fl = s->lights[i];
    const AmberFlatObject& fo = s->objects[fl.object];
    DevLight& dl = p.lights[i];
    std::memset(&dl, 0, sizeof dl);
    dl.kind = fo.kind; dl.slot = -1; dl.cum_power = fl.cum_power; dl.pdf_area = fl.pdf_area;
    for (int c = 0; c < 3; c++) dl.irr[c] = fl.irradiance[c];
    for (int c = 0; c < 12; c++) dl.p[c] = fo.p[c];
    for (uint32_t k = 0; k < fprog.n_prog_tris; k++)
      if (fprog.order[k] == fl.object) dl.slot = static_cast<int32_t>(k);
    for (size_t g = 0; g < more_progs.size(); g++)
      for (uint32_t k = 0; k < more_progs[g].n_prog_tris; k++)
        if (more_progs[g].order[k] == fl.object) dl.slot = static_cast<int32_t>(32u * (g + 1) + k);
  }
  p.planes = fprog.planes;
  p.tri_filters = fprog.tris;
  p.sphere_filters = fprog.spheres;
  std::vector<DevObject>& prog = p.prog_objects;
  prog.resize(more_progs.empty() ? fprog.order.size() : 32u * (more_progs.size() + 1));
  if (!prog.empty()) std::memset(prog.data(), 0, prog.size() * sizeof(DevObject));
  auto place = [&](const amber_filter::FilterProgram& fp, size_t base) {
    for (size_t k = 0; k < fp.order.size(); k++) { prog[base + k] = objs[fp.order[k]]; prog[base + k].kind |= fp.order[k] << 8 | (!more_progs.empty() && k < fp.n_prog_tris ? 0x80u : 0u); }
  };
  place(fprog, 0);
  if (!more_progs.empty()) {
    auto record = [&](const amber_filter::FilterProgram& fp, size_t plane_first, size_t tri_first, size_t sphere_first) {
      DevFilterGroup g{};
      g.plane_first = static_cast<uint32_t>(plane_first); g.n_planes = static_cast<uint32_t>(fp.planes.size()); g.n_simple_planes = fp.n_simple_planes;
      g.tri_first = static_cast<uint32_t>(tri_first); g.sphere_first = static_cast<uint32_t>(sphere_first); g.n_sphere_filters = static_cast<uint32_t>(fp.spheres.size());
      g.always_mask = fp.always_mask; g.n_prog_tris = fp.n_prog_tris; g.n_objects = static_cast<uint32_t>(fp.order.size());
      p.groups.push_back(g);
    };
    record(fprog, 0, 0, 0);
    for (size_t g = 0; g < more_progs.size(); g++) {
      const amber_filter::FilterProgram& fp = more_progs[g];
      record(fp, p.planes.size(), p.tri_filters.size(), p.sphere_filters.size());
      p.planes.insert(p.planes.end(), fp.planes.begin(), fp.planes.end());
      p.tri_filters.insert(p.tri_filters.end(), fp.tris.begin(), fp.tris.end());
      p.sphere_filters.insert(p.sphere_filters.end(), fp.spheres.begin(), fp.spheres.end());
      place(fp, 32u * (g + 1));
    }
  }

  if (!p.bvh_pending) FillBvhArrays(p, p, objs, bvh);
  p.ref_nodes = std::move(ref_tree.nodes);
  p.ref_leaves = std::move(ref_tree.leaves);

  DevScene& sc = p.scene;
  sc.n_planes = static_cast<uint32_t>(fprog.planes.size()); sc.n_simple_planes = fprog.n_simple_planes; sc.n_sphere_filters = static_cast<uint32_t>(fprog.spheres.size());
  if (p.hit_engine == AMBER_ENGINE_REFERENCE_BVH) sc.bvh_root = ref_tree.root;
  for (int c = 0; c < 3; c++) sc.fp_center[c] = fp_center[c];
  sc.fp_reach = fp_reach;
  sc.fp_tmax = static_cast<float>(std::min(3.0e38, 1.7320508 * 1.5 * 1.01 * static_cast<double>(fp_reach)));
  sc.n_lights = s->n_lights; sc.total_power = s->n_lights ? s->lights[s->n_lights - 1].cum_power : 0.0f;
  sc.n_prog_tris = fprog.n_prog_tris; sc.always_mask = fprog.always_mask;
  sc.n_groups = static_cast<uint32_t>(p.groups.empty() ? 1 : p.groups.size()); sc.n_lds_objects = static_cast<uint32_t>(prog.size());
  sc.blade_mask = 0u;
  for (const DevBlade& bl : blades) if (bl.slot >= 0 && bl.slot < 32) sc.blade_mask |= 1u << bl.slot;
  sc.n_objects = s->n_objects; sc.max_depth = params->max_depth;
  sc.sensor.w = sensor->width; sc.sensor.h = sensor->height;
  sc.sensor.wf = static_cast<float>(sensor->width); sc.sensor.hf = static_cast<float>(sensor->height);
  sc.sensor.sw = sensor->scene_width; sc.sensor.sh = sensor->scene_height;
  sc.sensor.size_f = static_cast<float>(static_cast<uint64_t>(sensor->width) * sensor->height);
  return p;
}

}
```

include/amber_hip_lab.h:

```cpp
#ifndef AMBER_HIP_LAB_H
#define AMBER_HIP_LAB_H

#include "amber_hip.h"

#ifdef __cplusplus
extern "C" {
#endif
#pragma GCC visibility push(default)

int amber_hip_kat_cast(amber_hip_pt*, uint32_t n, const float* origins , const float* dirs ,
                       int32_t* out_object, float* out_t, float* out_pos , float* out_normal );
int amber_hip_kat_sample(amber_hip_pt*, uint32_t n, const uint32_t* material , const float* normals,
                         const float* dirs_out, uint64_t* rng_state , float* out_dir_in, float* out_weight);
int amber_hip_kat_eye(amber_hip_pt*, uint32_t n, const uint32_t* pixel, const uint32_t* sample, float* out7);
int amber_hip_kat_light_ray(amber_hip_pt*, uint32_t n, uint64_t* rng_state , float* out_origin , float* out_dir ,
                            float* out_weight , uint32_t* out_light );
int amber_hip_kat_lens_response(amber_hip_pt*, uint32_t n, const float* position , const float* direction_out ,
                                uint32_t* out_reached , uint32_t* out_pixel , float* out_value );
int amber_hip_kat_radiance(amber_hip_pt*, uint32_t n, const uint32_t* material , const float* normals , const float* dirs_out ,
                           float* out );
struct amber_host_scene;
int amber_host_kat_scene_lights(const struct amber_host_scene*, AmberFlatLight* lights, uint32_t* n_lights);
int amber_hip_kat_trace(amber_hip_pt*, uint32_t n, const uint32_t* pixel, const uint32_t* sample,
                        uint32_t max_bounces, uint32_t* out_records , uint32_t* out_casts );
int amber_hip_kat_signatures(amber_hip_pt*, uint32_t first_sample, uint32_t n_samples, uint64_t* out);
int amber_hip_pt_signatures(amber_hip_pt*, uint32_t first_sample, uint32_t n_samples, uint64_t* out);
int amber_hip_kat_traversal_rate(amber_hip_pt*, uint32_t n, const float* origins, const float* dirs, uint32_t waves, uint32_t refill_min,
                                 uint32_t repeats, float* out_t, int32_t* out_object, double* best_ms, uint32_t* out_rounds);
int amber_hip_kat_pixel_masks(amber_hip_pt*, uint32_t* out_mask, uint32_t* out_slot_of_object, uint32_t* out_always_mask, double* kernel_ms);
typedef struct { uint32_t n_nodes, n_prims; int32_t root; uint32_t depth; float gmin[3], step[3], reach[3]; } AmberBvhDump;
int amber_hip_kat_bvh_dump(amber_hip_pt*, uint32_t* nodes, uint32_t node_capacity, uint32_t* prims, uint32_t prim_capacity, AmberBvhDump* info);
int amber_hip_kat_lt_accumulate(amber_hip_pt*, const AmberSplat* records , uint32_t n);
typedef struct { uint32_t n_launches, n_repeats, rec_count, flag_words_set, flags_dirty; } AmberAccumulateInfo;
int amber_hip_kat_accumulate(amber_hip_pt*, uint32_t n_samples, const uint32_t* q , const float* rgb , uint32_t n_items,
                             uint32_t n_waves, uint32_t rec_capacity, uint64_t rays, AmberAccumulateInfo* info);
int amber_hip_kat_lt_stage_ms(amber_hip_pt*, double* sort_ms, double* sum_ms);
int amber_hip_kat_photon_stage_ms(amber_hip_pt*, double* trace_ms, double* sort_ms, double* gather_ms);
int amber_hip_kat_math(int device, int mode, uint32_t n, const float* x, float* out);
int amber_hip_kat_division(int device, int mode, uint32_t n, const float* x, float* out);
int amber_hip_kat_sqrt(int device, int mode, uint32_t n, const float* x, float* out);
typedef struct { uint64_t mismatches, in_range; uint32_t n_offenders, offenders[8]; int32_t seed_low, seed_high; } AmberSqrtSweep;
int amber_hip_kat_sqrt_sweep(int device, uint32_t first_bits, uint64_t count, AmberSqrtSweep* out);

#pragma GCC visibility pop
#ifdef __cplusplus
}
#endif
#endif
```

Before: 47550.

## Specialize axis-aligned slab planes in Phase A candidate filtering

```diff
diff --git a/amber_amd/api.py b/amber_amd/api.py
--- a/amber_amd/api.py
+++ b/amber_amd/api.py
@@ -188,7 +188,7 @@
     "amber_hip_kat_sqrt", "amber_hip_kat_sqrt_sweep", "amber_hip_kat_lt_accumulate", "amber_hip_kat_lt_stage_ms",
     "amber_hip_kat_photon_stage_ms",
     "amber_hip_kat_light_ray", "amber_hip_kat_lens_response", "amber_hip_kat_radiance", "amber_host_kat_scene_lights",
-    "amber_hip_kat_accumulate",
+    "amber_hip_kat_accumulate", "amber_hip_kat_phase_a",
 ]
 PRODUCT_LIB, LAB_LIB = "libamber_hip.so", "libamber_hip_lab.so"
 
@@ -274,6 +274,8 @@
         if hasattr(lib, "amber_hip_kat_photon_stage_ms"):
             lib.amber_hip_kat_photon_stage_ms.argtypes = [vp, C.POINTER(C.c_double), C.POINTER(C.c_double), C.POINTER(C.c_double)]
     if hasattr(lib, "amber_hip_kat_cast"):
+        if hasattr(lib, "amber_hip_kat_phase_a"):
+            lib.amber_hip_kat_phase_a.argtypes = [vp, u32, vp, vp, i32, vp, u64, C.POINTER(C.c_uint32)]
         lib.amber_hip_kat_cast.argtypes = [vp, u32, vp, vp, vp, vp, vp, vp]
         lib.amber_hip_kat_sample.argtypes = [vp, u32, vp, vp, vp, vp, vp, vp]
         lib.amber_hip_kat_eye.argtypes = [vp, u32, vp, vp, vp]
@@ -837,6 +839,13 @@
                                                  pos.ctypes.data, nrm.ctypes.data))
         return obj, t, pos, nrm
 
+    def kat_phase_a(self, origins, dirs, axis_loops: bool = True):
+        o, d = _f32(origins).reshape(-1, 3), _f32(dirs).reshape(-1, 3)
+        n = len(o)
+        out, groups = np.zeros(4 * n, np.uint32), C.c_uint32()
+        _check(load_library().amber_hip_kat_phase_a(self._h, n, o.ctypes.data, d.ctypes.data, int(bool(axis_loops)), out.ctypes.data, out.size, C.byref(groups)))
+        return out[:n * groups.value].reshape(n, groups.value)
+
     def kat_sample(self, material, normals, dirs_out, rng_state, importance: bool = False):
         m = np.ascontiguousarray(material, np.uint32) | np.uint32(0x80000000 if importance else 0)
         nn, dd = _f32(normals).reshape(-1, 3), _f32(dirs_out).reshape(-1, 3)
diff --git a/amber_amd/csrc/hip/dev_scene.h b/amber_amd/csrc/hip/dev_scene.h
--- a/amber_amd/csrc/hip/dev_scene.h
+++ b/amber_amd/csrc/hip/dev_scene.h
@@ -78,7 +78,7 @@
   float ktol; uint32_t pad[3];
 };
 struct alignas(16) DevFilterGroup {
-  uint32_t plane_first, n_planes, n_simple_planes, tri_first;
+  uint32_t plane_first, n_planes, slab_ends, tri_first;
   uint32_t sphere_first, n_sphere_filters, always_mask, n_prog_tris;
   uint32_t n_objects, pad[3];
 };
@@ -137,7 +137,7 @@
   const DevTriFilter* __restrict__ tri_filters;
   const DevSphereFilter* __restrict__ sphere_filters;
   uint32_t n_planes, n_sphere_filters;
-  uint32_t n_simple_planes;
+  uint32_t slab_ends;
   uint32_t always_mask;
   uint32_t blade_mask;
   uint32_t n_prog_tris;
diff --git a/amber_amd/csrc/hip/dev_two_phase.h b/amber_amd/csrc/hip/dev_two_phase.h
--- a/amber_amd/csrc/hip/dev_two_phase.h
+++ b/amber_amd/csrc/hip/dev_two_phase.h
@@ -6,15 +6,26 @@
 #ifndef AMBER_SHARED_WEIGHT_QUOTIENT
 #define AMBER_SHARED_WEIGHT_QUOTIENT 1
 #endif
+#ifndef AMBER_AXIS_SLABS
+#define AMBER_AXIS_SLABS 1
+#endif
+#ifndef AMBER_AXIS_FIRST
+#define AMBER_AXIS_FIRST 1
+#endif
 struct FilterView {
   ConstWords planes, tris, spheres;
-  int n_planes, n_simple_planes, n_sphere_filters;
-  uint32_t always_mask, n_prog_tris, n_objects;
+  int n_planes, n_sphere_filters;
+  uint32_t slab_ends, always_mask, n_prog_tris, n_objects;
   int slot_base;
 };
 __device__ __forceinline__ FilterView SceneView(const DevScene& sc) {
-  return FilterView{(ConstWords)(sc.planes), (ConstWords)(sc.tri_filters), (ConstWords)(sc.sphere_filters), static_cast<int>(sc.n_planes), static_cast<int>(sc.n_simple_planes),
-                    static_cast<int>(sc.n_sphere_filters), sc.always_mask, sc.n_prog_tris, sc.n_objects, 0};
+  return FilterView{(ConstWords)(sc.planes), (ConstWords)(sc.tri_filters), (ConstWords)(sc.sphere_filters), static_cast<int>(sc.n_planes),
+                    static_cast<int>(sc.n_sphere_filters), sc.slab_ends, sc.always_mask, sc.n_prog_tris, sc.n_objects, 0};
+}
+__device__ __forceinline__ FilterView GroupView(const DevScene& sc, int g) {
+  ConstWords w = (ConstWords)(sc.groups) + g * 12;
+  return FilterView{(ConstWords)(sc.planes) + w[0] * 8u, (ConstWords)(sc.tri_filters) + w[3] * 8u, (ConstWords)(sc.sphere_filters) + w[4] * 8u,
+                    static_cast<int>(w[1]), static_cast<int>(w[5]), w[2], w[6], w[7], w[8], g * 32};
 }
 template <bool kMulti, bool kFirst, int kSqrt = SQRT_PLAIN>
 __device__ __forceinline__ void ClosestHitTwoPhaseView(const DevScene& sc, const FilterView fv, const DevObject* lds_objects, V3 o_world, V3 d, int origin_slot, HitRec& best AMBER_STAMP_PARAM,
@@ -29,15 +40,139 @@
                                                          const bool use_premask = false, const uint32_t premask = 0u) {
   ClosestHitTwoPhaseView<true, true, kSqrt>(sc, SceneView(sc), lds_objects, o_world, d, origin_slot < 32 ? origin_slot : -1, best AMBER_STAMP_ARG, use_premask, premask);
   const int n_groups = static_cast<int>(sc.n_groups);
-  ConstWords gw = (ConstWords)(sc.groups);
   for (int g = 1; g < n_groups; ++g) {
-    ConstWords w = gw + g * 12;
-    const FilterView fv{(ConstWords)(sc.planes) + w[0] * 8u, (ConstWords)(sc.tri_filters) + w[3] * 8u, (ConstWords)(sc.sphere_filters) + w[4] * 8u,
-                        static_cast<int>(w[1]), static_cast<int>(w[2]), static_cast<int>(w[5]), w[6], w[7], w[8], g * 32};
+    const FilterView fv = GroupView(sc, g);
     ClosestHitTwoPhaseView<true, false, kSqrt>(sc, fv, lds_objects, o_world, d, origin_slot, best AMBER_STAMP_ARG, false, 0u);
   }
 }
 template <bool kGrouped> constexpr uint32_t kLdsKindMask = kGrouped ? 0x7fu : 0xffu;
+template <int kC> __device__ __forceinline__ float Comp(const V3 v) { return kC == 0 ? v.x : (kC == 1 ? v.y : v.z); }
+template <bool kMulti, bool kAxis>
+__device__ __forceinline__ uint32_t PhaseA(const DevScene& sc, const FilterView& fv, const V3 o_world, const V3 d, uint32_t cand) {
+  const V3 o = v3(o_world.x - sc.fp_center[0], o_world.y - sc.fp_center[1], o_world.z - sc.fp_center[2]);
+  float t_upper = sc.fp_tmax * __builtin_amdgcn_rsqf(d.x * d.x + d.y * d.y + d.z * d.z);
+  if (!(t_upper == t_upper)) t_upper = 3.402823466e+38f;
+  ConstWords pl = kMulti ? fv.planes : (ConstWords)(sc.planes);
+  ConstWords tr = kMulti ? fv.tris : (ConstWords)(sc.tri_filters);
+  const int n_planes = kMulti ? fv.n_planes : static_cast<int>(sc.n_planes);
+  uint32_t bit = 1u;
+  float nd = 0.f, no = 0.f, rc = 0.f;
+#define AMBER_PLANE_NORMAL() \
+      nd = __builtin_fmaf(cw_f(pl, 0), d.x, __builtin_fmaf(cw_f(pl, 1), d.y, cw_f(pl, 2) * d.z)); \
+      no = __builtin_fmaf(cw_f(pl, 0), o.x, __builtin_fmaf(cw_f(pl, 1), o.y, cw_f(pl, 2) * o.z)); \
+      rc = __builtin_amdgcn_rcpf(nd);
+#define AMBER_PLANE_DISTANCE() \
+    const float tp = (cw_f(pl, 3) - no) * rc; \
+    const float rho = Abs(rc);
+#define AMBER_PLANE_SETUP() \
+    AMBER_PLANE_DISTANCE(); \
+    const float Px = __builtin_fmaf(tp, d.x, o.x), Py = __builtin_fmaf(tp, d.y, o.y), Pz = __builtin_fmaf(tp, d.z, o.z); \
+    AMBER_PLANE_TESTS();
+#define AMBER_PLANE_TESTS() \
+    const float kr = cw_f(pl, 4) * rho;                    \
+    const bool t_ok = (tp >= AMBER_KEPS - kr) && !(tp - kr > t_upper);                   \
+     \
+     \
+    const bool degenerate = !(Abs(nd) >= 1e-6f); \
+    const bool grazing = !(Abs(nd) >= AMBER_GRAZING); \
+    const bool t_sure = (tp - kr > AMBER_KEPS) && !grazing; \
+    const float ptol = cw_f(pl, 5) * rho; \
+    const float mtol = grazing ? -3.402823466e+38f : -ptol;                              \
+    bool plane_hit = false;
+#ifndef AMBER_NO_CERTAIN_HITS
+#define AMBER_PLANE_HIT(m_) plane_hit |= (m_) >= ptol
+#else
+#define AMBER_PLANE_HIT(m_)
+#endif
+#define AMBER_PAIR_RECORD() { \
+      const float b = __builtin_fmaf(cw_f(tr, 0), Px, __builtin_fmaf(cw_f(tr, 2), Py, __builtin_fmaf(cw_f(tr, 4), Pz, cw_f(tr, 6)))); \
+      const float a = __builtin_fmaf(cw_f(tr, 1), Px, __builtin_fmaf(cw_f(tr, 3), Py, __builtin_fmaf(cw_f(tr, 5), Pz, cw_f(tr, 7)))); \
+      AMBER_PAIR_TESTS(); }
+#define AMBER_PAIR_TESTS() \
+      const float ba = b + a;                              \
+      const float g = 1.0f - ba; \
+      const float m1 = __builtin_fminf(__builtin_fminf(b, a), g); \
+      const float m2 = __builtin_fminf(__builtin_fminf(-b, 1.0f - a), ba); \
+      const bool keep1 = (!(m1 < mtol) && t_ok) || degenerate;                           \
+      const bool keep2 = (!(m2 < mtol) && t_ok) || degenerate; \
+      cand |= keep1 ? bit : 0u; \
+      cand |= keep2 ? (bit << 1) : 0u; \
+      AMBER_PLANE_HIT(__builtin_fmaxf(m1, m2));
+#define AMBER_AXIS_SLAB_PLANE() { \
+      AMBER_PLANE_DISTANCE(); \
+      const float Pu = __builtin_fmaf(tp, du, ou), Pv = __builtin_fmaf(tp, dv, ov); \
+      AMBER_PLANE_TESTS(); \
+      { const float b = __builtin_fmaf(cw_f(tr, 2 * kU), Pu, __builtin_fmaf(cw_f(tr, 2 * kV), Pv, cw_f(tr, 6))); \
+        const float a = __builtin_fmaf(cw_f(tr, 2 * kU + 1), Pu, cw_f(tr, 7)); \
+        AMBER_PAIR_TESTS(); } \
+      if (plane_hit && t_sure) t_upper = __builtin_fminf(t_upper, tp + kr); } \
+    pl += 8; tr += 8; bit <<= 2;
+#define AMBER_AXIS_SLAB_LOOP(kC_, end_) { \
+    constexpr int kC = (kC_), kU = kC == 0 ? 1 : 0, kV = kC == 2 ? 1 : 2; \
+    const int end = static_cast<int>(end_); \
+    if (p < end) { \
+      const float du = Comp<kU>(d), dv = Comp<kV>(d), ou = Comp<kU>(o), ov = Comp<kV>(o); \
+      nd = Comp<kC>(d); no = Comp<kC>(o); rc = __builtin_amdgcn_rcpf(nd); \
+      for (; p < end; p += 2) { AMBER_AXIS_SLAB_PLANE(); AMBER_AXIS_SLAB_PLANE(); } } }
+  const uint32_t slab_ends = kMulti ? fv.slab_ends : sc.slab_ends;
+  int p = 0;
+  if (kAxis) {
+    AMBER_AXIS_SLAB_LOOP(AMBER_AXIS_FIRST % 3, slab_ends & 0xffu);
+    AMBER_AXIS_SLAB_LOOP((AMBER_AXIS_FIRST + 1) % 3, (slab_ends >> 8) & 0xffu);
+    AMBER_AXIS_SLAB_LOOP((AMBER_AXIS_FIRST + 2) % 3, (slab_ends >> 16) & 0xffu);
+  }
+  const int n_simple = static_cast<int>(slab_ends >> 24);
+  for (; p < n_simple; p += 2) {
+    AMBER_PLANE_NORMAL();
+    { AMBER_PLANE_SETUP(); AMBER_PAIR_RECORD(); if (plane_hit && t_sure) t_upper = __builtin_fminf(t_upper, tp + kr); }
+    pl += 8; tr += 8; bit <<= 2;
+    { AMBER_PLANE_SETUP(); AMBER_PAIR_RECORD(); if (plane_hit && t_sure) t_upper = __builtin_fminf(t_upper, tp + kr); }
+    pl += 8; tr += 8; bit <<= 2;
+  }
+  for (; p < n_planes; ++p, pl += 8) {
+    if (!(pl[6] & 0x80000000u)) { AMBER_PLANE_NORMAL(); }
+    AMBER_PLANE_SETUP();
+    const int nt = static_cast<int>(pl[6] & 0x7fffffffu), np = static_cast<int>(pl[7]);
+    for (int k = 0; k < np; ++k, tr += 8, bit <<= 2) {
+      AMBER_PAIR_RECORD();
+    }
+    for (int k = 0; k < nt; ++k, tr += 8, bit <<= 1) {
+      const float u = __builtin_fmaf(cw_f(tr, 0), Px, __builtin_fmaf(cw_f(tr, 2), Py, __builtin_fmaf(cw_f(tr, 4), Pz, cw_f(tr, 6))));
+      const float v = __builtin_fmaf(cw_f(tr, 1), Px, __builtin_fmaf(cw_f(tr, 3), Py, __builtin_fmaf(cw_f(tr, 5), Pz, cw_f(tr, 7))));
+      const float w = 1.0f - u - v;
+      const float m = __builtin_fminf(__builtin_fminf(u, v), w);
+      const bool keep = (!(m < mtol) && t_ok) || degenerate;
+      cand |= keep ? bit : 0u;
+      AMBER_PLANE_HIT(m);
+    }
+    if (plane_hit && t_sure) t_upper = __builtin_fminf(t_upper, tp + kr);
+  }
+#undef AMBER_AXIS_SLAB_LOOP
+#undef AMBER_AXIS_SLAB_PLANE
+#undef AMBER_PAIR_TESTS
+#undef AMBER_PLANE_TESTS
+#undef AMBER_PLANE_DISTANCE
+#undef AMBER_PLANE_SETUP
+#undef AMBER_PLANE_NORMAL
+#undef AMBER_PAIR_RECORD
+#undef AMBER_PLANE_HIT
+  ConstWords sp = kMulti ? fv.spheres : (ConstWords)(sc.sphere_filters);
+  const int ns = kMulti ? fv.n_sphere_filters : static_cast<int>(sc.n_sphere_filters);
+  for (int k = 0; k < ns; ++k, sp += 8, bit <<= 1) {
+    const float cx = cw_f(sp, 0) - o.x, cy = cw_f(sp, 1) - o.y, cz = cw_f(sp, 2) - o.z;
+    const float bb = __builtin_fmaf(cx, d.x, __builtin_fmaf(cy, d.y, cz * d.z));
+    const float c2 = __builtin_fmaf(cx, cx, __builtin_fmaf(cy, cy, cz * cz));
+    const float r2 = cw_f(sp, 3);
+    const float cc = c2 - r2;
+    const float tol = cw_f(sp, 4) * (c2 + r2);
+    const bool miss = (__builtin_fmaf(bb, bb, -cc) < -tol) || (bb < 0.0f && cc > tol);
+    cand |= miss ? 0u : bit;
+  }
+  const float ex = Abs(o_world.x - sc.fp_center[0]), ey = Abs(o_world.y - sc.fp_center[1]), ez = Abs(o_world.z - sc.fp_center[2]);
+  const bool in_model = __builtin_elementwise_maximum(__builtin_elementwise_maximum(ex, ey), ez) <= sc.fp_reach && (d.x * d.x + d.y * d.y + d.z * d.z) <= 4.0f;
+  if (!in_model) { const uint32_t n_here = kMulti ? fv.n_objects : sc.n_objects; cand = n_here >= 32u ? 0xffffffffu : ((1u << n_here) - 1u); }
+  return cand;
+}
 template <bool kMulti, bool kFirst, int kSqrt>
 __device__ __forceinline__ void ClosestHitTwoPhaseView(const DevScene& sc, const FilterView fv, const DevObject* lds_objects_all, V3 o_world, V3 d, int origin_slot_all, HitRec& best AMBER_STAMP_PARAM,
                                                        const bool use_premask, const uint32_t premask) {
@@ -48,99 +183,7 @@
   constexpr uint32_t kKindMask = kLdsKindMask<kMulti>;
   uint32_t cand = kMulti ? fv.always_mask : sc.always_mask;
   if (use_premask) cand |= premask;
-  else {
-    const V3 o = v3(o_world.x - sc.fp_center[0], o_world.y - sc.fp_center[1], o_world.z - sc.fp_center[2]);
-    float t_upper = sc.fp_tmax * __builtin_amdgcn_rsqf(d.x * d.x + d.y * d.y + d.z * d.z);
-    if (!(t_upper == t_upper)) t_upper = 3.402823466e+38f;
-    ConstWords pl = kMulti ? fv.planes : (ConstWords)(sc.planes);
-    ConstWords tr = kMulti ? fv.tris : (ConstWords)(sc.tri_filters);
-    const int n_planes = kMulti ? fv.n_planes : static_cast<int>(sc.n_planes);
-    uint32_t bit = 1u;
-    float nd = 0.f, no = 0.f, rc = 0.f;
-#define AMBER_PLANE_NORMAL() \
-        nd = __builtin_fmaf(cw_f(pl, 0), d.x, __builtin_fmaf(cw_f(pl, 1), d.y, cw_f(pl, 2) * d.z)); \
-        no = __builtin_fmaf(cw_f(pl, 0), o.x, __builtin_fmaf(cw_f(pl, 1), o.y, cw_f(pl, 2) * o.z)); \
-        rc = __builtin_amdgcn_rcpf(nd);
-#define AMBER_PLANE_SETUP() \
-      const float tp = (cw_f(pl, 3) - no) * rc; \
-      const float rho = Abs(rc); \
-      const float Px = __builtin_fmaf(tp, d.x, o.x), Py = __builtin_fmaf(tp, d.y, o.y), Pz = __builtin_fmaf(tp, d.z, o.z); \
-      const float kr = cw_f(pl, 4) * rho;                    \
-      const bool t_ok = (tp >= AMBER_KEPS - kr) && !(tp - kr > t_upper);                   \
-       \
-       \
-      const bool degenerate = !(Abs(nd) >= 1e-6f); \
-      const bool grazing = !(Abs(nd) >= AMBER_GRAZING); \
-      const bool t_sure = (tp - kr > AMBER_KEPS) && !grazing; \
-      const float ptol = cw_f(pl, 5) * rho; \
-      const float mtol = grazing ? -3.402823466e+38f : -ptol;                              \
-      bool plane_hit = false;
-#ifndef AMBER_NO_CERTAIN_HITS
-#define AMBER_PLANE_HIT(m_) plane_hit |= (m_) >= ptol
-#else
-#define AMBER_PLANE_HIT(m_)
-#endif
-#define AMBER_PAIR_RECORD() { \
-        const float b = __builtin_fmaf(cw_f(tr, 0), Px, __builtin_fmaf(cw_f(tr, 2), Py, __builtin_fmaf(cw_f(tr, 4), Pz, cw_f(tr, 6)))); \
-        const float a = __builtin_fmaf(cw_f(tr, 1), Px, __builtin_fmaf(cw_f(tr, 3), Py, __builtin_fmaf(cw_f(tr, 5), Pz, cw_f(tr, 7)))); \
-        const float ba = b + a;                              \
-        const float g = 1.0f - ba; \
-        const float m1 = __builtin_fminf(__builtin_fminf(b, a), g); \
-        const float m2 = __builtin_fminf(__builtin_fminf(-b, 1.0f - a), ba); \
-        const bool keep1 = (!(m1 < mtol) && t_ok) || degenerate;                           \
-        const bool keep2 = (!(m2 < mtol) && t_ok) || degenerate; \
-        cand |= keep1 ? bit : 0u; \
-        cand |= keep2 ? (bit << 1) : 0u; \
-        AMBER_PLANE_HIT(__builtin_fmaxf(m1, m2)); }
-    const int n_simple = kMulti ? fv.n_simple_planes : static_cast<int>(sc.n_simple_planes);
-    int p = 0;
-    for (; p < n_simple; p += 2) {
-      AMBER_PLANE_NORMAL();
-      { AMBER_PLANE_SETUP(); AMBER_PAIR_RECORD(); if (plane_hit && t_sure) t_upper = __builtin_fminf(t_upper, tp + kr); }
-      pl += 8; tr += 8; bit <<= 2;
-      { AMBER_PLANE_SETUP(); AMBER_PAIR_RECORD(); if (plane_hit && t_sure) t_upper = __builtin_fminf(t_upper, tp + kr); }
-      pl += 8; tr += 8; bit <<= 2;
-    }
-    for (; p < n_planes; ++p, pl += 8) {
-      if (!(pl[6] & 0x80000000u)) { AMBER_PLANE_NORMAL(); }
-      AMBER_PLANE_SETUP();
-      const int nt = static_cast<int>(pl[6] & 0x7fffffffu), np = static_cast<int>(pl[7]);
-      for (int k = 0; k < np; ++k, tr += 8, bit <<= 2) {
-        AMBER_PAIR_RECORD();
-      }
-      for (int k = 0; k < nt; ++k, tr += 8, bit <<= 1) {
-        const float u = __builtin_fmaf(cw_f(tr, 0), Px, __builtin_fmaf(cw_f(tr, 2), Py, __builtin_fmaf(cw_f(tr, 4), Pz, cw_f(tr, 6))));
-        const float v = __builtin_fmaf(cw_f(tr, 1), Px, __builtin_fmaf(cw_f(tr, 3), Py, __builtin_fmaf(cw_f(tr, 5), Pz, cw_f(tr, 7))));
-        const float w = 1.0f - u - v;
-        const float m = __builtin_fminf(__builtin_fminf(u, v), w);
-        const bool keep = (!(m < mtol) && t_ok) || degenerate;
-        cand |= keep ? bit : 0u;
-        AMBER_PLANE_HIT(m);
-      }
-      if (plane_hit && t_sure) t_upper = __builtin_fminf(t_upper, tp + kr);
-    }
-#undef AMBER_PLANE_SETUP
-#undef AMBER_PLANE_NORMAL
-#undef AMBER_PAIR_RECORD
-#undef AMBER_PLANE_HIT
-    ConstWords sp = kMulti ? fv.spheres : (ConstWords)(sc.sphere_filters);
-    const int ns = kMulti ? fv.n_sphere_filters : static_cast<int>(sc.n_sphere_filters);
-    for (int k = 0; k < ns; ++k, sp += 8, bit <<= 1) {
-      const float cx = cw_f(sp, 0) - o.x, cy = cw_f(sp, 1) - o.y, cz = cw_f(sp, 2) - o.z;
-      const float bb = __builtin_fmaf(cx, d.x, __builtin_fmaf(cy, d.y, cz * d.z));
-      const float c2 = __builtin_fmaf(cx, cx, __builtin_fmaf(cy, cy, cz * cz));
-      const float r2 = cw_f(sp, 3);
-      const float cc = c2 - r2;
-      const float tol = cw_f(sp, 4) * (c2 + r2);
-      const bool miss = (__builtin_fmaf(bb, bb, -cc) < -tol) || (bb < 0.0f && cc > tol);
-      cand |= miss ? 0u : bit;
-    }
-  }
-  if (!use_premask) {
-    const float ex = Abs(o_world.x - sc.fp_center[0]), ey = Abs(o_world.y - sc.fp_center[1]), ez = Abs(o_world.z - sc.fp_center[2]);
-    const bool in_model = __builtin_fmaxf(__builtin_fmaxf(ex, ey), ez) <= sc.fp_reach && (d.x * d.x + d.y * d.y + d.z * d.z) <= 4.0f;
-    if (!in_model) { const uint32_t n_here = kMulti ? fv.n_objects : sc.n_objects; cand = n_here >= 32u ? 0xffffffffu : ((1u << n_here) - 1u); }
-  }
+  else cand = PhaseA<kMulti, AMBER_AXIS_SLABS != 0>(sc, fv, o_world, d, cand);
   AMBER_STAMP(2);
   {
     const bool has_self = origin_slot >= 0 && ((cand >> (origin_slot & 31)) & 1u) != 0u;
diff --git a/amber_amd/csrc/hip/filter_build.h b/amber_amd/csrc/hip/filter_build.h
--- a/amber_amd/csrc/hip/filter_build.h
+++ b/amber_amd/csrc/hip/filter_build.h
@@ -23,7 +23,23 @@
   std::vector<uint32_t> order;
   uint32_t n_prog_tris = 0, always_mask = 0;
   uint32_t n_simple_planes = 0;
+  uint32_t n_axis_slabs[3] = {0, 0, 0};
 };
+inline int AxisSlabOrder(int k) { return (AMBER_AXIS_FIRST + k) % 3; }
+
+inline uint32_t SlabEnds(const FilterProgram& fp) {
+  const uint32_t e0 = 2u * fp.n_axis_slabs[AxisSlabOrder(0)], e1 = e0 + 2u * fp.n_axis_slabs[AxisSlabOrder(1)], e2 = e1 + 2u * fp.n_axis_slabs[AxisSlabOrder(2)];
+  return e0 | e1 << 8 | e2 << 16 | fp.n_simple_planes << 24;
+}
+inline void AxisSlabInPlane(int c, int& u, int& v) { u = c == 0 ? 1 : 0; v = c == 2 ? 1 : 2; }
+inline int AxisSlabClass(const DevPlane& p, const DevTriFilter& f) {
+  for (int c = 0; c < 3; c++) {
+    int u, v; AxisSlabInPlane(c, u, v);
+    if (std::fabs(p.n[c]) == 1.0f && p.n[u] == 0.0f && p.n[v] == 0.0f)
+      return (f.c[c][0] == 0.0f && f.c[c][1] == 0.0f && f.c[u][1] != 0.0f && f.c[v][1] == 0.0f) ? c : -1;
+  }
+  return -1;
+}
 
 inline void BuildFilterProgram(const std::vector<DevObject>& objs, const float center[3], FilterProgram& fp, const std::vector<uint32_t>* subset = nullptr) {
   double lo[3] = {1e300, 1e300, 1e300}, hi[3] = {-1e300, -1e300, -1e300}, e_max = 0;
@@ -160,6 +176,7 @@
     }
     groups.swap(sorted);
   }
+  std::vector<DevTriFilter> other_corner;
   for (const Group& g : groups) {
     const size_t nt = g.tris.size();
     std::vector<int> partner(nt, -1), unshared(nt, -1);
@@ -202,12 +219,14 @@
       if (partner[i] < 0 || static_cast<size_t>(partner[i]) < i) continue;
       const int bi = unshared[i], ai = (bi + 1) % 3;
       fp.tris.push_back(record(g.tris[i], bi, ai));
+      other_corner.push_back(record(g.tris[i], bi, (bi + 2) % 3));
       fp.order.push_back(g.tris[i].index); fp.order.push_back(g.tris[static_cast<size_t>(partner[i])].index);
       p.n_pairs++;
     }
     for (size_t i = 0; i < nt; i++) {
       if (partner[i] >= 0) continue;
       fp.tris.push_back(record(g.tris[i], 1, 2));
+      other_corner.push_back(fp.tris.back());
       fp.order.push_back(g.tris[i].index);
       p.n_tris++;
     }
@@ -224,13 +243,31 @@
         rec += np + nt; slot += 2 * np + nt;
       } }
     auto simple = [&](size_t i) { return fp.planes[i].n_pairs == 1 && (fp.planes[i].n_tris & 0x7fffffffu) == 0; };
-    std::vector<char> in_slab(fp.planes.size(), 0);
-    for (size_t i = 0; i + 1 < fp.planes.size(); i++)
-      if (!in_slab[i] && simple(i) && simple(i + 1) && std::memcmp(fp.planes[i].n, fp.planes[i + 1].n, sizeof fp.planes[i].n) == 0) { in_slab[i] = in_slab[i + 1] = 1; i++; }
+    enum { kSlabOther = 3, kGeneral = 4 };
+    std::vector<int> kind(fp.planes.size(), kGeneral);
+    for (size_t i = 0; i + 1 < fp.planes.size(); i++) {
+      if (!(simple(i) && simple(i + 1) && std::memcmp(fp.planes[i].n, fp.planes[i + 1].n, sizeof fp.planes[i].n) == 0)) continue;
+      int axis[2]; bool other[2];
+      for (size_t k = 0; k < 2; k++) {
+        axis[k] = AxisSlabClass(fp.planes[i + k], fp.tris[span[i + k].rec]);
+        other[k] = axis[k] < 0;
+        if (other[k]) axis[k] = AxisSlabClass(fp.planes[i + k], other_corner[span[i + k].rec]);
+      }
+      if (axis[0] >= 0 && axis[0] == axis[1]) {
+        for (size_t k = 0; k < 2; k++) {
+          DevPlane& q = fp.planes[i + k];
+          if (other[k]) fp.tris[span[i + k].rec] = other_corner[span[i + k].rec];
+          if (q.n[axis[0]] < 0.0f) q.d0 = -q.d0;
+          for (int c2 = 0; c2 < 3; c2++) q.n[c2] = c2 == axis[0] ? 1.0f : 0.0f;
+        }
+        kind[i] = kind[i + 1] = axis[0];
+      } else kind[i] = kind[i + 1] = kSlabOther;
+      i++;
+    }
     std::vector<DevPlane> planes; std::vector<DevTriFilter> tris; std::vector<uint32_t> order;
-    for (int pass = 0; pass < 2; pass++)
+    for (int pass = 0; pass <= kGeneral; pass++)
       for (size_t i = 0; i < fp.planes.size(); i++) {
-        if ((in_slab[i] != 0) != (pass == 0)) continue;
+        if (kind[i] != (pass < kSlabOther ? AxisSlabOrder(pass) : pass)) continue;
         DevPlane q = fp.planes[i];
         const uint32_t nt = q.n_tris & 0x7fffffffu, np = q.n_pairs;
         q.n_tris = nt;
@@ -238,7 +275,8 @@
         planes.push_back(q);
         for (uint32_t k = 0; k < np + nt; k++) tris.push_back(fp.tris[span[i].rec + k]);
         for (uint32_t k = 0; k < 2 * np + nt; k++) order.push_back(fp.order[span[i].slot + k]);
-        if (pass == 0) fp.n_simple_planes++;
+        if (pass < kGeneral) fp.n_simple_planes++;
+        if (pass < kSlabOther && (fp.n_simple_planes & 1u) == 0u) fp.n_axis_slabs[AxisSlabOrder(pass)]++;
       }
     fp.planes.swap(planes); fp.tris.swap(tris); fp.order.swap(order);
   }
diff --git a/amber_amd/csrc/hip/lab_api.inc b/amber_amd/csrc/hip/lab_api.inc
--- a/amber_amd/csrc/hip/lab_api.inc
+++ b/amber_amd/csrc/hip/lab_api.inc
@@ -109,6 +109,32 @@
   return AMBER_OK;
 }); }
 
+int amber_hip_kat_phase_a(amber_hip_pt* h, uint32_t n, const float* origins, const float* dirs, int axis_loops, uint32_t* out_mask, uint64_t mask_capacity, uint32_t* out_n_groups) { return Guarded("amber_hip_kat_phase_a", [&]() -> int {
+  if (!h || !origins || !dirs || !out_mask) return Fail(AMBER_EINVAL, "null argument");
+  if (!h->two_phase) return Fail(AMBER_EINVAL, "amber_hip_kat_phase_a: the handle's engine has no Phase A (two-phase engines only)");
+  const uint32_t n_groups = h->hit_engine == kHitTwoPhaseN ? h->scene.n_groups : 1u;
+  if (out_n_groups) *out_n_groups = n_groups;
+  if (static_cast<uint64_t>(n) * n_groups > mask_capacity) return Fail(AMBER_EINVAL, "amber_hip_kat_phase_a: out_mask holds fewer than n * n_groups words (at most four groups)");
+  if (n == 0) return AMBER_OK;
+  HIP_TRY(hipSetDevice(h->device));
+  DevBuf<float> d_o, d_d; DevBuf<uint32_t> d_m;
+  HIP_TRY(d_o.alloc(3ull * n)); HIP_TRY(d_d.alloc(3ull * n)); HIP_TRY(d_m.alloc(static_cast<size_t>(n) * n_groups));
+  HIP_TRY(hipMemcpy(d_o.p, origins, 12ull * n, hipMemcpyHostToDevice));
+  HIP_TRY(hipMemcpy(d_d.p, dirs, 12ull * n, hipMemcpyHostToDevice));
+  const dim3 grid((n + 255) / 256), block(256);
+  if (h->hit_engine == kHitTwoPhaseN) {
+    if (axis_loops) hipLaunchKernelGGL((kat_phase_a_kernel<true, true>), grid, block, 0, h->stream, h->scene, n, d_o.p, d_d.p, d_m.p);
+    else hipLaunchKernelGGL((kat_phase_a_kernel<true, false>), grid, block, 0, h->stream, h->scene, n, d_o.p, d_d.p, d_m.p);
+  } else {
+    if (axis_loops) hipLaunchKernelGGL((kat_phase_a_kernel<false, true>), grid, block, 0, h->stream, h->scene, n, d_o.p, d_d.p, d_m.p);
+    else hipLaunchKernelGGL((kat_phase_a_kernel<false, false>), grid, block, 0, h->stream, h->scene, n, d_o.p, d_d.p, d_m.p);
+  }
+  HIP_TRY(hipGetLastError());
+  HIP_TRY(hipStreamSynchronize(h->stream));
+  HIP_TRY(hipMemcpy(out_mask, d_m.p, 4ull * n * n_groups, hipMemcpyDeviceToHost));
+  return AMBER_OK;
+}); }
+
 int amber_hip_kat_sample(amber_hip_pt* h, uint32_t n, const uint32_t* material, const float* normals,
                          const float* dirs_out, uint64_t* rng_state, float* out_dir_in, float* out_weight) { return Guarded("amber_hip_kat_sample", [&]() -> int {
   if (!h || !material || !normals || !dirs_out || !rng_state || !out_dir_in || !out_weight) return Fail(AMBER_EINVAL, "null argument");
diff --git a/amber_amd/csrc/hip/lab_kernels.inc b/amber_amd/csrc/hip/lab_kernels.inc
--- a/amber_amd/csrc/hip/lab_kernels.inc
+++ b/amber_amd/csrc/hip/lab_kernels.inc
@@ -23,6 +23,19 @@
   out_t[i] = h.t;
   out_pos[3 * i] = pos.x; out_pos[3 * i + 1] = pos.y; out_pos[3 * i + 2] = pos.z;
   out_n[3 * i] = nrm.x; out_n[3 * i + 1] = nrm.y; out_n[3 * i + 2] = nrm.z;
+}
+
+template <bool kMulti, bool kAxis>
+__global__ void kat_phase_a_kernel(const DevScene sc, uint32_t n, const float* org, const float* dir, uint32_t* out) {
+  const uint32_t i = blockIdx.x * blockDim.x + threadIdx.x;
+  const uint32_t k = ClampToLastItem(i, n);
+  const V3 o = ld3(org + 3 * k), d = ld3(dir + 3 * k);
+  const uint32_t n_groups = kMulti ? sc.n_groups : 1u;
+  for (uint32_t g = 0; g < n_groups; ++g) {
+    const FilterView fv = g == 0u ? SceneView(sc) : GroupView(sc, static_cast<int>(g));
+    const uint32_t cand = PhaseA<kMulti, kAxis>(sc, fv, o, d, kMulti ? fv.always_mask : sc.always_mask);
+    if (i < n) out[static_cast<size_t>(i) * n_groups + g] = cand;
+  }
 }
 
 __global__ void kat_sample_kernel(const DevScene sc, uint32_t n, const uint32_t* material, const float* normals,
diff --git a/amber_amd/csrc/hip/scene_prep.h b/amber_amd/csrc/hip/scene_prep.h
--- a/amber_amd/csrc/hip/scene_prep.h
+++ b/amber_amd/csrc/hip/scene_prep.h
@@ -381,7 +381,7 @@
   if (!more_progs.empty()) {
     auto record = [&](const amber_filter::FilterProgram& fp, size_t plane_first, size_t tri_first, size_t sphere_first) {
       DevFilterGroup g{};
-      g.plane_first = static_cast<uint32_t>(plane_first); g.n_planes = static_cast<uint32_t>(fp.planes.size()); g.n_simple_planes = fp.n_simple_planes;
+      g.plane_first = static_cast<uint32_t>(plane_first); g.n_planes = static_cast<uint32_t>(fp.planes.size()); g.slab_ends = amber_filter::SlabEnds(fp);
       g.tri_first = static_cast<uint32_t>(tri_first); g.sphere_first = static_cast<uint32_t>(sphere_first); g.n_sphere_filters = static_cast<uint32_t>(fp.spheres.size());
       g.always_mask = fp.always_mask; g.n_prog_tris = fp.n_prog_tris; g.n_objects = static_cast<uint32_t>(fp.order.size());
       p.groups.push_back(g);
@@ -402,7 +402,7 @@
   p.ref_leaves = std::move(ref_tree.leaves);
 
   DevScene& sc = p.scene;
-  sc.n_planes = static_cast<uint32_t>(fprog.planes.size()); sc.n_simple_planes = fprog.n_simple_planes; sc.n_sphere_filters = static_cast<uint32_t>(fprog.spheres.size());
+  sc.n_planes = static_cast<uint32_t>(fprog.planes.size()); sc.slab_ends = amber_filter::SlabEnds(fprog); sc.n_sphere_filters = static_cast<uint32_t>(fprog.spheres.size());
   if (p.hit_engine == AMBER_ENGINE_REFERENCE_BVH) sc.bvh_root = ref_tree.root;
   for (int c = 0; c < 3; c++) sc.fp_center[c] = fp_center[c];
   sc.fp_reach = fp_reach;
diff --git a/include/amber_hip_lab.h b/include/amber_hip_lab.h
--- a/include/amber_hip_lab.h
+++ b/include/amber_hip_lab.h
@@ -10,6 +10,8 @@
 
 int amber_hip_kat_cast(amber_hip_pt*, uint32_t n, const float* origins , const float* dirs ,
                        int32_t* out_object, float* out_t, float* out_pos , float* out_normal );
+int amber_hip_kat_phase_a(amber_hip_pt*, uint32_t n, const float* origins , const float* dirs , int axis_loops,
+                          uint32_t* out_mask, uint64_t mask_capacity, uint32_t* out_n_groups);
 int amber_hip_kat_sample(amber_hip_pt*, uint32_t n, const uint32_t* material , const float* normals,
                          const float* dirs_out, uint64_t* rng_state , float* out_dir_in, float* out_weight);
 int amber_hip_kat_eye(amber_hip_pt*, uint32_t n, const uint32_t* pixel, const uint32_t* sample, float* out7);
```

New measurement: 48060 (median of 6 runs). +1.1%, better.
